# siyi-wind/MDViT

Hardware: AMD Instinct MI355X
Metric: 512x512 images/sec MDViT train step (fwd+bwd, two-sweep, AdamW) (higher is better)
Workload: dtype bf16x3 (fp32 storage; GEMM operands split hi+lo bf16, fp32 accumulate); 1 GPU; MDViT Sup+MLPFM train step, 4 domain(s) x bs=4 per GPU, 512x512, drop_rate=0.1 drop_path=0.1, bf16x3 GEMMs, data-parallel x1

## Files before the change

### include/mdvit_hip.h

```cpp
#ifndef MDVIT_HIP_H
#define MDVIT_HIP_H

#include <stddef.h>
#include <stdint.h>

#ifdef __cplusplus
extern "C" {
#endif

#define MDVIT_ABI_VERSION 1

enum {
    MDVIT_OK = 0,
    MDVIT_E_SHAPE = 1,
    MDVIT_E_DTYPE = 2,
    MDVIT_E_ALIGN = 3,
    MDVIT_E_WORKSPACE = 4,
    MDVIT_E_HIP = 5
};

enum { MDVIT_EPI_NONE = 0, MDVIT_EPI_GELU_DUAL = 1, MDVIT_EPI_DGELU = 2 };
enum { MDVIT_ACT_NONE = 0, MDVIT_ACT_HSWISH = 1, MDVIT_ACT_RELU = 2 };

const char* mdvit_last_error(void);
// ... 159 lines not shown
    int32_t ln_accumulate;
    float* e_out;
} MdvitBlockGrads;
typedef struct MdvitBlockStreams {
    void* main; void* side;
    void** events; int32_t n_events; int32_t* next_event;
} MdvitBlockStreams;
size_t mdvit_block_save_bytes(const MdvitBlockDesc* d);
size_t mdvit_block_fwd_ws_bytes(const MdvitBlockDesc* d);
int mdvit_block_fwd(const MdvitBlockDesc* d, const float* x, float* y, void* save, size_t save_bytes, void* ws, size_t ws_bytes, void* stream);
size_t mdvit_block_bwd_ws_bytes(const MdvitBlockDesc* d, const MdvitBlockGrads* g, int32_t with_side_stream, size_t* side_bytes);
int mdvit_block_bwd(const MdvitBlockDesc* d, const MdvitBlockGrads* g, const MdvitBlockStreams* st, const float* x, const void* save, size_t save_bytes,
                    const float* dy, float* dx , void* ws, size_t ws_bytes, void* ws_side, size_t ws_side_bytes);

int mdvit_rowdot_fwd(const float* x, int64_t ldx, const float* w, const float* b, float* y,
                     int32_t M, int32_t K, int32_t accumulate, void* stream);
int mdvit_rowdot_bwd(const float* x, int64_t ldx, const float* w, const float* dy, float* dx, int64_t lddx,
                     float* dw, float* db, void* ws , size_t ws_bytes, int32_t M, int32_t K, void* stream);

int mdvit_colsum_f32(const float* A, int64_t lda, float* out, float* masked, void* ws , size_t ws_bytes, int32_t M, int32_t N,
                     float drop_p, uint32_t key0, uint32_t key1, const float* rowscale, int32_t rows_per_scale,
                     int32_t accumulate, const uint32_t* drop_seed, void* stream);

int mdvit_layernorm_fwd(const float* x, const float* gamma, const float* beta, float* y, float* mean, float* rstd,
                        int32_t M, int32_t C, int32_t groups, float eps, void* stream);
int mdvit_layernorm_bwd(const float* dy, const float* x, const float* gamma, const float* mean, const float* rstd,
                        const float* add, float* dx, float* dgamma, float* dbeta, void* ws , size_t ws_bytes,
                        int32_t M, int32_t C, int32_t groups, void* stream);
int mdvit_layernorm_bwd_masked(const float* dy, const float* x, const float* gamma, const float* mean, const float* rstd, const float* add, float* dx,
                               float* dx_masked, float* dgamma, float* dbeta, void* ws, size_t ws_bytes, int32_t M, int32_t C, int32_t groups,
                               float drop_p, uint32_t key0, uint32_t key1, const float* rowscale, int32_t rows_per_scale, const uint32_t* seed, void* stream);

int mdvit_dwconv3x3_fwd(const float* x, const float* w, const float* bias, float* y,
                        int32_t B, int32_t Hi, int32_t Wi, int32_t C, int32_t stride, int32_t add_input, void* stream);
int mdvit_dwconv3x3_bwd(const float* dy, const float* x, const float* w, float* dx, float* dw, float* dbias,
                        void* ws , size_t ws_bytes,
                        int32_t B, int32_t Hi, int32_t Wi, int32_t C, int32_t stride, int32_t add_input,
                        int32_t accumulate , void* stream);
int mdvit_gconv2_3x3_fwd(const float* skip, const float* up, const float* w, float* y,
                         int32_t B, int32_t H, int32_t W, int32_t C, void* stream);
int mdvit_gconv2_3x3_bwd(const float* dy, const float* skip, const float* up, const float* w,
                         float* dskip, float* dup, float* dw, void* ws , size_t ws_bytes,
                         int32_t B, int32_t H, int32_t W, int32_t C, int32_t accumulate , void* stream);
int mdvit_im2col3x3(const float* x, float* col, int32_t B, int32_t Hi, int32_t Wi, int32_t Cin, int32_t stride, int32_t dilation, void* stream);
int mdvit_col2im3x3(const float* dcol, float* dx, int32_t B, int32_t Hi, int32_t Wi, int32_t Cin, int32_t stride, int32_t dilation, void* stream);
int mdvit_dropout_f32(const float* x, float* y, int64_t n, float p, uint32_t key0, uint32_t key1, const uint32_t* drop_seed, void* stream);
int mdvit_stemconv_fwd(const float* img, const float* w, float* y, int32_t B, int32_t H, int32_t W, int32_t Cin, int32_t Cout, void* stream);
int mdvit_stemconv_wgrad(const float* img, const float* dy, float* dw, void* ws , size_t ws_bytes,
                         int32_t B, int32_t H, int32_t W, int32_t Cin, int32_t Cout, int32_t accumulate , void* stream);

size_t mdvit_bn_ws_bytes(int32_t M, int32_t C, int32_t groups);
int mdvit_bn_stats(const float* y, void* ws, size_t ws_bytes, float* mean, float* rstd, float* running_mean, float* running_var,
                   int64_t* num_batches_tracked, int32_t M, int32_t C, int32_t groups, int32_t per_group_affine, float eps,
                   float momentum, void* stream);
int mdvit_bn_eval_prep(const float* running_mean, const float* running_var, float* mean, float* rstd, int32_t C, float eps, void* stream);
int mdvit_bn_apply(const float* y, const float* mean, const float* rstd, const float* gamma, const float* beta, float* z,
                   int32_t M, int32_t C, int32_t groups, int32_t per_group_affine, int32_t act, float drop2d_p, uint32_t key0,
                   uint32_t key1, const uint32_t* drop_seed, int32_t rows_per_sample, void* stream);
int mdvit_bn_bwd(const float* dz, const float* y, const float* mean, const float* rstd, const float* gamma, const float* beta,
                 float* dy, float* dgamma, float* dbeta, void* ws, size_t ws_bytes, int32_t M, int32_t C, int32_t groups,
                 int32_t per_group_affine, int32_t act, int32_t training, float drop2d_p, uint32_t key0, uint32_t key1, const uint32_t* drop_seed, int32_t rows_per_sample,
                 void* stream);

size_t mdvit_bn_rowdot_ws_bytes(int32_t M, int32_t C);
int mdvit_bn_rowdot_fwd(const float* y, const float* mean, const float* rstd, const float* gamma, const float* beta, const float* w, const float* b ,
                        float* low, int32_t M, int32_t C, int32_t act, float drop2d_p, uint32_t key0, uint32_t key1, const uint32_t* drop_seed,
                        int32_t rows_per_sample, void* stream);
int mdvit_bn_rowdot_bwd(const float* g, const float* y, const float* mean, const float* rstd, const float* gamma, const float* beta, const float* w,
                        float* dy, float* dgamma, float* dbeta, float* dw, float* db , void* ws, size_t ws_bytes, int32_t M, int32_t C, int32_t act,
                        int32_t training, float drop2d_p, uint32_t key0, uint32_t key1, const uint32_t* drop_seed, int32_t rows_per_sample, void* stream);

int mdvit_upsample_fwd(const float* x, const float* base , float* y,
                       int32_t B, int32_t Hi, int32_t Wi, int32_t Ho, int32_t Wo, int32_t C, void* stream);
size_t mdvit_upsample_bwd_ws_bytes(int32_t B, int32_t Hi, int32_t Wi, int32_t Ho, int32_t Wo, int32_t C);
int mdvit_upsample_bwd(const float* dy, float* dx, void* ws, size_t ws_bytes, int32_t B, int32_t Hi, int32_t Wi, int32_t Ho, int32_t Wo,
                       int32_t C, void* stream);

int mdvit_upsample_multi_fwd(const float* const* xs, const int32_t* Hi, const int32_t* Wi, int32_t n, const float* base, float* y, int32_t B, int32_t Ho,
                             int32_t Wo, int32_t C, void* stream);
size_t mdvit_upsample_multi_bwd_ws_bytes(const int32_t* Wi, int32_t n, int32_t B, int32_t Ho, int32_t C);
int mdvit_upsample_multi_bwd(const float* dy, float* const* dxs, const int32_t* Hi, const int32_t* Wi, int32_t n, void* ws, size_t ws_bytes, int32_t B,
                             int32_t Ho, int32_t Wo, int32_t C, void* stream);

int mdvit_da_fwd(const float* label, const float* W1, const float* b1, const float* W2, const float* b2, float* a,
                 int32_t B, int32_t D, int32_t hid, int32_t C, int32_t heads, void* stream);
#define MDVIT_DA_MANY_MAX 32
typedef struct MdvitDaMany {
    int32_t n;
    int32_t hid[MDVIT_DA_MANY_MAX], C[MDVIT_DA_MANY_MAX], heads[MDVIT_DA_MANY_MAX];
    const float* W1[MDVIT_DA_MANY_MAX]; const float* b1[MDVIT_DA_MANY_MAX]; const float* W2[MDVIT_DA_MANY_MAX]; const float* b2[MDVIT_DA_MANY_MAX];
    float* a[MDVIT_DA_MANY_MAX];
} MdvitDaMany;
int mdvit_da_fwd_many(const MdvitDaMany* m, const float* label, int32_t B, int32_t D, void* stream);
typedef struct MdvitDaManyGrads {
    const float* e[MDVIT_DA_MANY_MAX];
    float* dW1[MDVIT_DA_MANY_MAX]; float* db1[MDVIT_DA_MANY_MAX]; float* dW2[MDVIT_DA_MANY_MAX]; float* db2[MDVIT_DA_MANY_MAX];
} MdvitDaManyGrads;
size_t mdvit_da_many_ws_bytes(const MdvitDaMany* m, int32_t B);
int mdvit_da_bwd_many(const MdvitDaMany* m, const MdvitDaManyGrads* g, const float* label, float scale, void* ws, size_t ws_bytes, int32_t B, int32_t D, void* stream);
size_t mdvit_da_ws_bytes(int32_t B, int32_t hid, int32_t C);
int mdvit_da_bwd(const float* label, const float* W1, const float* b1, const float* W2, const float* b2, const float* a,
                 const float* e, float scale, float* dW1, float* db1, float* dW2, float* db2, void* ws, size_t ws_bytes,
                 int32_t B, int32_t D, int32_t hid, int32_t C, int32_t heads, void* stream);

size_t mdvit_factoratt_ws_bytes(int32_t B, int32_t N, int32_t C, int32_t heads);
int mdvit_factoratt_fwd(const float* qkv, const float* w3, const float* b3, const float* w5, const float* b5,
                        const float* w7, const float* b7, const float* a, float* out, float* U, float* kmax, float* ksum, float* Mmat,
                        void* ws, size_t ws_bytes, int32_t B, int32_t H, int32_t W, int32_t C, int32_t heads,
                        int32_t s3, int32_t s5, int32_t s7, void* stream);
int mdvit_factoratt_bwd(const float* dout, const float* qkv, const float* out, const float* U,
                        const float* w3, const float* b3, const float* w5, const float* b5, const float* w7, const float* b7,
                        const float* a, const float* kmax, const float* ksum, const float* Mmat,
                        float* dqkv, float* e, float* dw3, float* db3, float* dw5, float* db5, float* dw7, float* db7,
                        void* ws, size_t ws_bytes, int32_t B, int32_t H, int32_t W, int32_t C, int32_t heads,
                        int32_t s3, int32_t s5, int32_t s7, void* stream);
int mdvit_factoratt_wgrad(const float* qkv, void* ws, size_t ws_bytes, float* dw3, float* db3, float* dw5, float* db5,
                          float* dw7, float* db7, int32_t B, int32_t H, int32_t W, int32_t C, int32_t heads,
                          int32_t s3, int32_t s5, int32_t s7, int32_t accumulate, void* stream);

int mdvit_seg_losses_fwd(const float* out, const float* aux, const float* label, double* sums, float* losses, int64_t n, void* stream);
int mdvit_seg_losses_sums(const float* out, const float* aux, const float* label, double* sums, int64_t n, void* stream);
int mdvit_seg_losses_final(const double* sums, float* losses, int64_t n_total, int32_t has_aux, void* stream);
int mdvit_seg_losses_bwd(const float* out, const float* aux, const float* label, const double* sums, const float* g,
                         float* dout, float* daux, int64_t n, float dice_gain, void* stream);
int mdvit_seg_losses_bwd3(const float* out, const float* aux, const float* label, const double* sums, const float* g0, const float* g1, const float* g2,
                          float* dout, float* daux, int64_t n, float dice_gain, void* stream);
int mdvit_seg_losses_groups_sums(const float* out, const float* aux, const float* label, double* sums, int64_t n, int32_t G, void* stream);
int mdvit_seg_losses_groups_final(const double* sums, float* losses, float* per_group, int64_t n_total, int32_t has_aux, int32_t G, void* stream);
int mdvit_seg_losses_groups_bwd(const float* out, const float* aux, const float* label, const double* sums, const float* g0, const float* g1, const float* g2,
                                float* dout, float* daux, int64_t n, int32_t G, float dice_gain, void* stream);

int mdvit_seg_metrics(const float* out, const float* aux, const float* label, uint64_t* counts, float* metrics, int64_t n, void* stream);
int mdvit_image_normalize_u8(const uint8_t* img_nhwc, float* out_nchw, int32_t B, int32_t H, int32_t W, void* stream);
int mdvit_augment_normalize_u8(const uint8_t* img_nhwc, const uint8_t* mask, const float* params, const uint32_t* keys, float* out_nchw, float* label,
                               int32_t B, int32_t H, int32_t W, void* stream);
int mdvit_augment_probe_taps(float xs, float ys, int32_t H, int32_t W, int32_t* idx5, float* w4);

int mdvit_adamw_step(const void* table_dev, int32_t n_tensors, int32_t blocks_per_tensor, const float* lr_dev, float* step_dev,
                     float beta1, float beta2, float eps, float weight_decay, int32_t zero_grad, void* stream);

int mdvit_imgconv_fwd(const float* img, const float* w, float* y, int32_t B, int32_t H, int32_t W, int32_t in_chans, int32_t Cout, int32_t ksize, void* stream);
int mdvit_imgconv_wgrad(const float* img, const float* dy, float* dw, void* ws, size_t ws_bytes, int32_t B, int32_t H, int32_t W, int32_t in_chans,
                        int32_t Cout, int32_t ksize, int32_t accumulate, void* stream);
int mdvit_imgconv_im2col(const float* img, float* col, int32_t B, int32_t H, int32_t W, int32_t in_chans, int32_t ksize, int32_t ldc, void* stream);
int mdvit_maxpool3x3s2_fwd(const float* x, float* y, void* idx, int32_t B, int32_t H, int32_t W, int32_t C, void* stream);
int mdvit_maxpool3x3s2_bwd(const float* dy, const void* idx, float* dx, int32_t B, int32_t H, int32_t W, int32_t C, void* stream);
int mdvit_resize_ac_fwd(const float* x, float* y, int32_t B, int32_t Hi, int32_t Wi, int32_t Ho, int32_t Wo, int32_t C, void* stream);
int mdvit_resize_ac_bwd(const float* dy, float* dx, int32_t B, int32_t Hi, int32_t Wi, int32_t Ho, int32_t Wo, int32_t C, void* stream);
int mdvit_ew(const float* a, const float* b, float* y, int64_t n, int32_t mode, void* stream);
int mdvit_add3(const float* a, const float* b, const float* c, float* y, int64_t n, void* stream);
int mdvit_add_parts(const float* a, const float* b, const void* const* parts, int32_t G, int64_t part_elems, float* y, void* stream);
int mdvit_add_bcast(const float* x, const float* pe, float* y, int32_t B, int64_t R, void* stream);
int mdvit_sum_batch(const float* g, float* out, int32_t B, int64_t R, void* stream);
int mdvit_gate_fwd(const float* x, const float* s, float* y, int32_t B, int64_t P, int32_t C, int32_t mode, void* stream);
size_t mdvit_gate_bwd_ws_bytes(int32_t B, int64_t P, int32_t C, int32_t mode);
int mdvit_gate_bwd(const float* g, const float* x, const float* s, float* dx, float* ds, void* ws, size_t ws_bytes, int32_t B, int64_t P, int32_t C, int32_t mode,
                   void* stream);
int mdvit_chanpool_fwd(const float* x, float* y, int32_t* idx, int64_t M, int32_t C, void* stream);
int mdvit_chanpool_bwd(const float* dy, const int32_t* idx, float* dx, int64_t M, int32_t C, void* stream);
int mdvit_conv7x7_2to1_fwd(const float* x, const float* w, float* y, int32_t B, int32_t H, int32_t W, void* stream);
int mdvit_conv7x7_2to1_bwd(const float* dy, const float* x, const float* w, float* dx , float* dw , int32_t B, int32_t H,
                           int32_t W, void* stream);
int mdvit_bn1_fwd(const float* x, const float* gamma, const float* beta, float* running_mean, float* running_var, void* num_batches_tracked, float* y,
                  float* stat, int64_t M, int32_t groups, int32_t training, float eps, float momentum, void* stream);
int mdvit_bn1_bwd(const float* g, const float* x, const float* gamma, const float* stat, float* dx, float* dgamma_dbeta, int64_t M, int32_t groups, int32_t training,
                  void* stream);
// ... 32 lines not shown
```

### mdvit_amd/_lib.py

```python
from __future__ import annotations

import ctypes as C
import os
import re
from typing import List

_HERE = os.path.dirname(os.path.abspath(__file__))
LIB_PATH = os.environ.get("MDVIT_HIP_LIB") or os.path.join(_HERE, "lib", "libmdvit_hip.so")
HEADER_PATH = os.path.join(_HERE, "..", "include", "mdvit_hip.h")

EPI_NONE, EPI_GELU_DUAL, EPI_DGELU = 0, 1, 2
ACT_NONE, ACT_HSWISH, ACT_RELU = 0, 1, 2

f32p = C.c_void_p
vp = C.c_void_p
i32 = C.c_int32
i64 = C.c_int64
u32 = C.c_uint32
f32 = C.c_float


class GemmDesc(C.Structure):
    _fields_ = [
        ("A", vp), ("B", vp), ("C", vp), ("C2", vp),
# ... 113 lines not shown
    "mdvit_linear_rc": [vp, i64, vp, i64, vp, vp, i64, i32, i32, i32, f32, u32, u32, vp, i32, vp, i64, vp, vp],
    "mdvit_linear_rc_ln": [vp, vp, vp, i32, f32, vp, vp, vp, vp, i64, vp, vp, i64, i32, i32, i32, vp],
    "mdvit_mlp_rc_fwd_ln": [vp, vp, vp, i32, f32, vp, vp, vp, vp, vp, vp, vp, vp, i32, vp, vp, i32, i32, i32, f32, u32, u32, u32, u32, vp, vp],
    "mdvit_mlp_rc16_fwd": [vp, vp, vp, vp, vp, vp, vp, i32, vp, vp, i32, i32, i32, f32, u32, u32, u32, u32, vp, vp],
    "mdvit_mlp_rc_dgrad": [vp, vp, vp, vp, vp, vp, vp, i32, i32, i32, f32, u32, u32, vp, vp],
    "mdvit_mlp_rc16_dgrad": [vp, vp, vp, vp, vp, vp, vp, vp, i32, i32, i32, f32, u32, u32, vp, vp],
    "mdvit_mlp_rc_fwd_ln_hbf16": [vp, vp, vp, i32, f32, vp, vp, vp, vp, vp, vp, vp, vp, i32, vp, vp, i32, i32, i32, f32, u32, u32, u32, u32, vp, vp],
    "mdvit_mlp_rc16_fwd_hbf16": [vp, vp, vp, vp, vp, vp, vp, i32, vp, vp, i32, i32, i32, f32, u32, u32, u32, u32, vp, vp],
    "mdvit_mlp_rc16_dgrad_hbf16": [vp, vp, vp, vp, vp, vp, vp, vp, i32, i32, i32, f32, u32, u32, vp, vp],
    "mdvit_mlp_rc_wgrad": [vp, vp, vp, vp, vp, vp, vp, vp, vp, C.c_size_t, i32, i32, i32, f32, u32, u32, vp, i32, vp],
    "mdvit_mlp_rc_bwd": [vp, vp, vp, vp, vp, vp, vp, vp, vp, vp, vp, C.c_size_t, i32, i32, i32, f32, u32, u32, vp, i32, vp],
    "mdvit_imgconv_fwd": [vp, vp, vp, i32, i32, i32, i32, i32, i32, vp],
    "mdvit_imgconv_wgrad": [vp, vp, vp, vp, C.c_size_t, i32, i32, i32, i32, i32, i32, i32, vp],
    "mdvit_maxpool3x3s2_fwd": [vp, vp, vp, i32, i32, i32, i32, vp],
    "mdvit_maxpool3x3s2_bwd": [vp, vp, vp, i32, i32, i32, i32, vp],
    "mdvit_resize_ac_fwd": [vp, vp, i32, i32, i32, i32, i32, i32, vp],
    "mdvit_resize_ac_bwd": [vp, vp, i32, i32, i32, i32, i32, i32, vp],
    "mdvit_ew": [vp, vp, vp, i64, i32, vp],
    "mdvit_add3": [vp, vp, vp, vp, i64, vp],
    "mdvit_add_parts": [vp, vp, C.POINTER(vp), i32, i64, vp, vp],
    "mdvit_add_bcast": [vp, vp, vp, i32, i64, vp],
    "mdvit_sum_batch": [vp, vp, i32, i64, vp],
    "mdvit_gate_fwd": [vp, vp, vp, i32, i64, i32, i32, vp],
    "mdvit_gate_bwd": [vp, vp, vp, vp, vp, vp, C.c_size_t, i32, i64, i32, i32, vp],
    "mdvit_imgconv_im2col": [vp, vp, i32, i32, i32, i32, i32, i32, vp],
    "mdvit_chanpool_fwd": [vp, vp, vp, i64, i32, vp],
    "mdvit_chanpool_bwd": [vp, vp, vp, i64, i32, vp],
    "mdvit_conv7x7_2to1_fwd": [vp, vp, vp, i32, i32, i32, vp],
    "mdvit_conv7x7_2to1_bwd": [vp, vp, vp, vp, vp, i32, i32, i32, vp],
    "mdvit_bn1_fwd": [vp, vp, vp, vp, vp, vp, vp, vp, i64, i32, i32, f32, f32, vp],
    "mdvit_bn1_bwd": [vp, vp, vp, vp, vp, vp, i64, i32, i32, vp],
    "mdvit_subsample2": [vp, vp, i32, i32, i32, i32, i32, vp],
    "mdvit_patchify": [vp, vp, i32, i32, i32, i32, i32, vp],
    "mdvit_dropout2d": [vp, vp, i32, i64, i32, f32, u32, u32, vp, vp],
    "mdvit_sdpa_fwd": [vp, vp, vp, vp, i32, i32, i32, i32, vp],
    "mdvit_sdpa_bwd": [vp, vp, vp, vp, vp, vp, vp, vp, i32, i32, i32, i32, vp],
    "mdvit_sdpa_mfma_fwd": [vp, vp, vp, vp, i32, i32, i32, i32, vp],
    "mdvit_sdpa_mfma_bwd": [vp, vp, vp, vp, vp, vp, vp, vp, i32, i32, i32, i32, vp],
    "mdvit_structure_weight": [vp, vp, vp, i32, i32, i32, vp],
    "mdvit_structure_loss_fwd": [vp, vp, vp, vp, vp, i32, i64, vp],
    "mdvit_structure_loss_bwd": [vp, vp, vp, vp, vp, vp, i32, i64, vp],
    "mdvit_split_planes": [vp, i64, vp, i64, i64, i64, i32, i32, vp],
    "mdvit_split_planes_many": [vp, i32, i32, i32, vp],
    "mdvit_split_planes_t": [vp, i64, vp, i64, i64, i32, i32, i32, i32, vp],
    "mdvit_event_create": [C.POINTER(vp)],
    "mdvit_event_destroy": [vp],
    "mdvit_event_elapsed_ms": [vp, vp, C.POINTER(f32)],
    "mdvit_timing_arm": [vp, vp],
    "mdvit_gemm_f32": [C.POINTER(GemmDesc), vp],
    "mdvit_gemm_plan": [C.POINTER(GemmDesc), C.POINTER(i32), C.POINTER(i32), C.POINTER(i32)],
    "mdvit_gemm_force_plan": [i32, i32],
    "mdvit_conv_weight_relayout": [vp, vp, i32, i32, i32, vp],
    "mdvit_conv_weight_relayout_many": [vp, i32, i32, vp],
    "mdvit_gemm_kernel_name": [vp, C.c_char_p, i32],
    "mdvit_gemm_tn_config": [i32, i32, i32],
    "mdvit_gemm_tn_grid_order": [i32],
    "mdvit_transpose_f32": [vp, i64, vp, i32, i32, vp],
    "mdvit_mlp_bwd_dgrad_f32": [vp, vp, vp, vp, vp, vp, vp, vp, i32, i32, i32, f32, u32, u32, vp, vp],
    "mdvit_mlp_fwd_f32": [vp, vp, vp, vp, vp, vp, vp, i32, vp, vp, i32, i32, i32, f32, u32, u32, u32, u32, vp, vp],
    "mdvit_transpose_many": [vp, i32, i32, vp],
    "mdvit_rowdot_fwd": [vp, i64, vp, vp, vp, i32, i32, i32, vp],
    "mdvit_rowdot_bwd": [vp, i64, vp, vp, vp, i64, vp, vp, vp, C.c_size_t, i32, i32, vp],
    "mdvit_colsum_f32": [vp, i64, vp, vp, vp, C.c_size_t, i32, i32, f32, u32, u32, vp, i32, i32, vp, vp],
    "mdvit_layernorm_fwd": [vp, vp, vp, vp, vp, vp, i32, i32, i32, f32, vp],
    "mdvit_layernorm_bwd": [vp, vp, vp, vp, vp, vp, vp, vp, vp, vp, C.c_size_t, i32, i32, i32, vp],
    "mdvit_layernorm_bwd_masked": [vp, vp, vp, vp, vp, vp, vp, vp, vp, vp, vp, C.c_size_t, i32, i32, i32, f32, u32, u32, vp, i32, vp, vp],
    "mdvit_dwconv3x3_fwd": [vp, vp, vp, vp, i32, i32, i32, i32, i32, i32, vp],
    "mdvit_dwconv3x3_bwd": [vp, vp, vp, vp, vp, vp, vp, C.c_size_t, i32, i32, i32, i32, i32, i32, i32, vp],
    "mdvit_gconv2_3x3_fwd": [vp, vp, vp, vp, i32, i32, i32, i32, vp],
    "mdvit_gconv2_3x3_bwd": [vp, vp, vp, vp, vp, vp, vp, vp, C.c_size_t, i32, i32, i32, i32, i32, vp],
    "mdvit_im2col3x3": [vp, vp, i32, i32, i32, i32, i32, i32, vp],
    "mdvit_col2im3x3": [vp, vp, i32, i32, i32, i32, i32, i32, vp],
    "mdvit_dropout_f32": [vp, vp, i64, f32, u32, u32, vp, vp],
    "mdvit_stemconv_fwd": [vp, vp, vp, i32, i32, i32, i32, i32, vp],
    "mdvit_stemconv_wgrad": [vp, vp, vp, vp, C.c_size_t, i32, i32, i32, i32, i32, i32, vp],
    "mdvit_bn_rowdot_fwd": [vp, vp, vp, vp, vp, vp, vp, vp, i32, i32, i32, f32, u32, u32, vp, i32, vp],
    "mdvit_bn_rowdot_bwd": [vp, vp, vp, vp, vp, vp, vp, vp, vp, vp, vp, vp, vp, C.c_size_t, i32, i32, i32, i32, f32, u32, u32, vp, i32, vp],
    "mdvit_bn_stats": [vp, vp, C.c_size_t, vp, vp, vp, vp, vp, i32, i32, i32, i32, f32, f32, vp],
    "mdvit_bn_eval_prep": [vp, vp, vp, vp, i32, f32, vp],
    "mdvit_bn_apply": [vp, vp, vp, vp, vp, vp, i32, i32, i32, i32, i32, f32, u32, u32, vp, i32, vp],
    "mdvit_bn_bwd": [vp, vp, vp, vp, vp, vp, vp, vp, vp, vp, C.c_size_t, i32, i32, i32, i32, i32, i32, f32, u32, u32, vp, i32, vp],
    "mdvit_upsample_multi_fwd": [vp, vp, vp, i32, vp, vp, i32, i32, i32, i32, vp],
    "mdvit_upsample_multi_bwd": [vp, vp, vp, vp, i32, vp, C.c_size_t, i32, i32, i32, i32, vp],
    "mdvit_upsample_fwd": [vp, vp, vp, i32, i32, i32, i32, i32, i32, vp],
    "mdvit_upsample_bwd": [vp, vp, vp, C.c_size_t, i32, i32, i32, i32, i32, i32, vp],
    "mdvit_da_fwd": [vp, vp, vp, vp, vp, vp, i32, i32, i32, i32, i32, vp],
    "mdvit_da_bwd": [vp] * 7 + [f32] + [vp] * 4 + [vp, C.c_size_t] + [i32] * 5 + [vp],
    "mdvit_factoratt_fwd": [vp] * 13 + [vp, C.c_size_t] + [i32] * 8 + [vp],
    "mdvit_factoratt_wgrad": [vp, vp, C.c_size_t] + [vp] * 6 + [i32] * 9 + [vp],
    "mdvit_factoratt_bwd": [vp] * 22 + [vp, C.c_size_t] + [i32] * 8 + [vp],
    "mdvit_seg_losses_fwd": [vp, vp, vp, vp, vp, i64, vp],
    "mdvit_adamw_step": [vp, i32, i32, vp, vp, f32, f32, f32, f32, i32, vp],
    "mdvit_seg_metrics": [vp, vp, vp, vp, vp, i64, vp],
    "mdvit_image_normalize_u8": [vp, vp, i32, i32, i32, vp],
    "mdvit_augment_normalize_u8": [vp, vp, vp, vp, vp, vp, i32, i32, i32, vp],
    "mdvit_augment_probe_taps": [f32, f32, i32, i32, C.POINTER(i32), C.POINTER(f32)],
    "mdvit_seg_losses_sums": [vp, vp, vp, vp, i64, vp],
    "mdvit_seg_losses_final": [vp, vp, i64, i32, vp],
    "mdvit_seg_losses_bwd": [vp, vp, vp, vp, vp, vp, vp, i64, f32, vp],
    "mdvit_seg_losses_bwd3": [vp, vp, vp, vp, vp, vp, vp, vp, vp, i64, f32, vp],
    "mdvit_seg_losses_groups_sums": [vp, vp, vp, vp, i64, i32, vp],
    "mdvit_seg_losses_groups_final": [vp, vp, vp, i64, i32, i32, vp],
    "mdvit_seg_losses_groups_bwd": [vp, vp, vp, vp, vp, vp, vp, vp, vp, i64, i32, f32, vp],
    "mdvit_se_adapter_fwd": [C.POINTER(SeAdapterDesc), vp, vp, vp, vp, C.c_size_t, vp],
    "mdvit_se_adapter_bwd": [C.POINTER(SeAdapterDesc)] + [vp] * 10 + [vp, C.c_size_t, vp],
}

_lib = None


class MdvitHipError(RuntimeError):
    pass


def declared_symbols() -> List[str]:
    with open(HEADER_PATH) as f:
        text = f.read()
    text = re.sub(r"/\*.*?\*/", "", text, flags=re.S)
    return sorted(set(re.findall(r"\b(mdvit_[a-z0-9_]+)\s*\(", text)))


_on_load = []


def on_load(fn):
    if _lib is not None:
        fn(_lib)
    else:
        _on_load.append(fn)


def load():
    global _lib
    if _lib is not None:
        return _lib
    if not os.path.exists(LIB_PATH):
        raise MdvitHipError(
            f"{LIB_PATH} is missing: build it with `python -m mdvit_amd.build` (hipcc, gfx950). "
            "mdvit_amd has no CPU or PyTorch fallback.")
    lib = C.CDLL(LIB_PATH)
    try:
        _attach_prototypes(lib)
    except AttributeError as e:
        raise MdvitHipError(f"{LIB_PATH} is stale ({e}): rebuild it with `python -m mdvit_amd.build`.") from None
    _lib = lib
    while _on_load:
        _on_load.pop(0)(lib)
    return lib


def _attach_prototypes(lib):
    lib.mdvit_last_error.restype = C.c_char_p
    lib.mdvit_last_error.argtypes = []
    lib.mdvit_version.restype = C.c_int
    lib.mdvit_version.argtypes = []
    lib.mdvit_factoratt_ws_bytes.restype = C.c_size_t
    lib.mdvit_factoratt_ws_bytes.argtypes = [i32, i32, i32, i32]
    lib.mdvit_gemm_ws_bytes.restype = C.c_size_t
    lib.mdvit_gemm_ws_bytes.argtypes = [C.POINTER(GemmDesc)]
    lib.mdvit_gate_bwd_ws_bytes.restype = C.c_size_t
    lib.mdvit_gate_bwd_ws_bytes.argtypes = [i32, i64, i32, i32]
    lib.mdvit_gemm_planes_ws_bytes.restype = C.c_size_t
    lib.mdvit_gemm_planes_ws_bytes.argtypes = [C.POINTER(PlaneGemmDesc)]
    lib.mdvit_bn_rowdot_ws_bytes.restype = C.c_size_t
    lib.mdvit_bn_rowdot_ws_bytes.argtypes = [i32, i32]
    lib.mdvit_bn_ws_bytes.restype = C.c_size_t
    lib.mdvit_bn_ws_bytes.argtypes = [i32, i32, i32]
    lib.mdvit_upsample_multi_bwd_ws_bytes.restype = C.c_size_t
    lib.mdvit_upsample_multi_bwd_ws_bytes.argtypes = [vp, i32, i32, i32, i32]
    lib.mdvit_upsample_bwd_ws_bytes.restype = C.c_size_t
    lib.mdvit_upsample_bwd_ws_bytes.argtypes = [i32] * 6
    lib.mdvit_partials_ws_bytes.restype = C.c_size_t
    lib.mdvit_partials_ws_bytes.argtypes = [i32]
    lib.mdvit_mlp_rc_wgrad_ws_bytes.restype = C.c_size_t
    lib.mdvit_mlp_rc_wgrad_ws_bytes.argtypes = [i32, i32, i32]
    lib.mdvit_block_save_bytes.restype = C.c_size_t
    lib.mdvit_block_save_bytes.argtypes = [C.POINTER(BlockDesc)]
    lib.mdvit_block_fwd_ws_bytes.restype = C.c_size_t
    lib.mdvit_block_fwd_ws_bytes.argtypes = [C.POINTER(BlockDesc)]
    lib.mdvit_block_bwd_ws_bytes.restype = C.c_size_t
    lib.mdvit_block_bwd_ws_bytes.argtypes = [C.POINTER(BlockDesc), C.POINTER(BlockGrads), i32, C.POINTER(C.c_size_t)]
    lib.mdvit_da_ws_bytes.restype = C.c_size_t
    lib.mdvit_da_ws_bytes.argtypes = [i32, i32, i32]
    lib.mdvit_da_many_ws_bytes.restype = C.c_size_t
    lib.mdvit_da_many_ws_bytes.argtypes = [C.POINTER(DaMany), i32]
    lib.mdvit_se_adapter_save_bytes.restype = C.c_size_t
    lib.mdvit_se_adapter_save_bytes.argtypes = [C.POINTER(SeAdapterDesc)]
    lib.mdvit_se_adapter_ws_bytes.restype = C.c_size_t
    lib.mdvit_se_adapter_ws_bytes.argtypes = [C.POINTER(SeAdapterDesc)]
    for name, sig in _SIGS.items():
        try:
            fn = getattr(lib, name)
        except AttributeError:
            raise MdvitHipError(f"{LIB_PATH} is stale: it does not export `{name}` (built from an earlier tree). "
                                "Rebuild it with `python -m mdvit_amd.build`.") from None
        fn.restype = C.c_int
        fn.argtypes = sig


def check(code: int, what: str):
    if code != 0:
        msg = load().mdvit_last_error().decode(errors="replace")
        raise MdvitHipError(f"{what} failed (code {code}): {msg}")


def call(name: str, *args):
    lib = load()
    check(getattr(lib, name)(*args), name)
```

### mdvit_amd/build.py

```python
from __future__ import annotations

import concurrent.futures as cf
import hashlib
import os
import subprocess
import sys

HERE = os.path.dirname(os.path.abspath(__file__))
CSRC = os.path.join(HERE, "csrc")
OBJ = os.path.join(HERE, "build")
LIB_DIR = os.path.join(HERE, "lib")
LIB = os.path.join(LIB_DIR, "libmdvit_hip.so")
SOURCES = ["abi.hip", "gemm.hip", "gemm_tn.hip", "gemm_bp.hip", "gemm_ph.hip", "gemm_pm.hip", "mlp.hip", "mlp_rc.hip", "block.hip", "norm.hip", "conv.hip", "attn.hip", "loss.hip", "optim.hip", "transfuse.hip", "sdpa.hip", "se_adapter.hip", "augment.hip"]
FLAGS = ["--offload-arch=gfx950", "-O3", "-std=c++17", "-fPIC", "-Wno-unused-result"]
EXTRA_FLAGS = {"mlp_rc.hip": ["-fno-slp-vectorize"], "gemm.hip": ["-fno-slp-vectorize"], "gemm_tn.hip": ["-fno-slp-vectorize"], "gemm_bp.hip": ["-fno-slp-vectorize"], "gemm_ph.hip": ["-fno-slp-vectorize"], "gemm_pm.hip": ["-fno-slp-vectorize"]}


def _hipcc() -> str:
    for c in (os.environ.get("HIPCC"), "/opt/rocm/bin/hipcc", "hipcc"):
        if c and (os.path.isabs(c) and os.path.exists(c) or not os.path.isabs(c)):
            return c
    raise RuntimeError("hipcc not found")


def _digest(paths) -> str:
    h = hashlib.sha256()
    for p in paths:
        with open(p, "rb") as f:
            h.update(f.read())
    h.update(" ".join(FLAGS).encode())
    return h.hexdigest()


def _compile(src: str) -> str:
    obj = os.path.join(OBJ, os.path.splitext(src)[0] + ".o")
    stamp = obj + ".sha"
    deps = [os.path.join(CSRC, src), os.path.join(CSRC, "common.h"), os.path.join(CSRC, "conv_tile.h"), os.path.join(CSRC, "gemm_body.inc"), os.path.join(CSRC, "gemm_bp.h"), os.path.join(CSRC, "augment_taps.h"),
            os.path.join(HERE, "..", "include", "mdvit_hip.h")]
    extra = EXTRA_FLAGS.get(src, [])
    dig = _digest(deps) + " ".join(extra)
    if os.path.exists(obj) and os.path.exists(stamp) and open(stamp).read() == dig:
        return obj
    cmd = [_hipcc(), *FLAGS, *extra, "-c", os.path.join(CSRC, src), "-o", obj]
    r = subprocess.run(cmd, capture_output=True, text=True)
    if r.returncode != 0:
        raise RuntimeError(f"hipcc failed on {src}:\n{r.stderr}")
    with open(stamp, "w") as f:
        f.write(dig)
    return obj


def build(verbose: bool = True) -> str:
    os.makedirs(OBJ, exist_ok=True)
    os.makedirs(LIB_DIR, exist_ok=True)
    with cf.ThreadPoolExecutor(max_workers=min(6, os.cpu_count() or 2)) as ex:
        objs = list(ex.map(_compile, SOURCES))
    newest = max(os.path.getmtime(o) for o in objs)
    if not os.path.exists(LIB) or os.path.getmtime(LIB) < newest:
        cmd = [_hipcc(), "--offload-arch=gfx950", "-shared", "-fPIC", *objs, "-o", LIB]
        r = subprocess.run(cmd, capture_output=True, text=True)
        if r.returncode != 0:
            raise RuntimeError(f"link failed:\n{r.stderr}")
    if verbose:
        print(f"built {LIB} ({os.path.getsize(LIB) / 1e6:.1f} MB)")
    return LIB


if __name__ == "__main__":
    build()
    sys.exit(0)
```

### mdvit_amd/csrc/conv.hip

```cpp
#include "common.h"
#include "conv_tile.h"

namespace {

__device__ __forceinline__ float4 f4_fma(float4 a, float4 w, float4 acc) {
    acc.x = fmaf(a.x, w.x, acc.x); acc.y = fmaf(a.y, w.y, acc.y); acc.z = fmaf(a.z, w.z, acc.z); acc.w = fmaf(a.w, w.w, acc.w);
    return acc;
}
__device__ __forceinline__ float4 f4_add(float4 a, float4 b) { return make_float4(a.x + b.x, a.y + b.y, a.z + b.z, a.w + b.w); }

__global__ __launch_bounds__(256) void dwconv3x3_fwd_kernel(const float* __restrict__ x, const float* __restrict__ w,
                                                            const float* __restrict__ bias, float* __restrict__ y,
                                                            int B, int Hi, int Wi, int C, int stride, int add_input) {
    extern __shared__ float s_w[];
    for (int i = threadIdx.x; i < 9 * C; i += blockDim.x) { const int c = i / 9, t = i % 9; s_w[t * C + c] = w[i]; }
    __syncthreads();
    const int Ho = (Hi - 1) / stride + 1, Wo = (Wi - 1) / stride + 1, QC = C >> 2;
    const long total = (long)B * Ho * Wo * QC;
    for (long e = (long)blockIdx.x * blockDim.x + threadIdx.x; e < total; e += (long)gridDim.x * blockDim.x) {
        const int c = (int)(e % QC) * 4;
        long tkn = e / QC;
        const int wo = (int)(tkn % Wo); tkn /= Wo;
        const int ho = (int)(tkn % Ho);
        const int b = (int)(tkn / Ho);
        float4 acc = bias ? *reinterpret_cast<const float4*>(bias + c) : make_float4(0.f, 0.f, 0.f, 0.f);
#pragma unroll
        for (int kh = 0; kh < 3; ++kh) {
            const int hi = ho * stride + kh - 1, hc = min(max(hi, 0), Hi - 1);
#pragma unroll
            for (int kw = 0; kw < 3; ++kw) {
                const int wi = wo * stride + kw - 1, wc = min(max(wi, 0), Wi - 1);
                const float m = (hi == hc && wi == wc) ? 1.f : 0.f;
                const float4 xv = *reinterpret_cast<const float4*>(x + (((long)b * Hi + hc) * Wi + wc) * C + c);
                const float4 wv = *reinterpret_cast<const float4*>(&s_w[(kh * 3 + kw) * C + c]);
                acc = f4_fma(xv, make_float4(wv.x * m, wv.y * m, wv.z * m, wv.w * m), acc);
            }
        }
        if (add_input) acc = f4_add(acc, *reinterpret_cast<const float4*>(x + (((long)b * Hi + ho) * Wi + wo) * C + c));
        *reinterpret_cast<float4*>(y + (((long)b * Ho + ho) * Wo + wo) * C + c) = acc;
    }
}

__global__ __launch_bounds__(256) void dwconv3x3_dgrad_kernel(const float* __restrict__ dy, const float* __restrict__ w,
                                                              float* __restrict__ dx, int B, int Hi, int Wi, int C, int stride, int add_input) {
    extern __shared__ float s_w[];
    for (int i = threadIdx.x; i < 9 * C; i += blockDim.x) { const int c = i / 9, t = i % 9; s_w[t * C + c] = w[i]; }
    __syncthreads();
    const int Ho = (Hi - 1) / stride + 1, Wo = (Wi - 1) / stride + 1, QC = C >> 2;
    const long total = (long)B * Hi * Wi * QC;
    for (long e = (long)blockIdx.x * blockDim.x + threadIdx.x; e < total; e += (long)gridDim.x * blockDim.x) {
        const int c = (int)(e % QC) * 4;
        long tkn = e / QC;
        const int wi = (int)(tkn % Wi); tkn /= Wi;
        const int hi = (int)(tkn % Hi);
        const int b = (int)(tkn / Hi);
        float4 acc = make_float4(0.f, 0.f, 0.f, 0.f);
#pragma unroll
        for (int kh = 0; kh < 3; ++kh) {
            const int hn = hi - kh + 1;
            if (hn < 0 || (hn % stride) != 0) continue;
            const int ho = hn / stride;
            if (ho >= Ho) continue;
#pragma unroll
            for (int kw = 0; kw < 3; ++kw) {
                const int wn = wi - kw + 1;
                if (wn < 0 || (wn % stride) != 0) continue;
                const int wo = wn / stride;
                if (wo >= Wo) continue;
                const float4 g = *reinterpret_cast<const float4*>(dy + (((long)b * Ho + ho) * Wo + wo) * C + c);
                const float4 wv = *reinterpret_cast<const float4*>(&s_w[(kh * 3 + kw) * C + c]);
                acc = f4_fma(g, wv, acc);
            }
        }
        if (add_input) acc = f4_add(acc, *reinterpret_cast<const float4*>(dy + (((long)b * Hi + hi) * Wi + wi) * C + c));
        *reinterpret_cast<float4*>(dx + (((long)b * Hi + hi) * Wi + wi) * C + c) = acc;
    }
}

__global__ __launch_bounds__(256) void dwconv3x3_wgrad_kernel(const float* __restrict__ dy, const float* __restrict__ x,
                                                              float* __restrict__ part,
                                                              int B, int Hi, int Wi, int C, int stride, int tokens_per_block) {
    extern __shared__ float s_acc[];
    for (int i = threadIdx.x; i < C * 10; i += blockDim.x) s_acc[i] = 0.f;
    __syncthreads();
// ... 334 lines not shown
    for (int co = threadIdx.x % nco; co < Cout; co += nco) {
        float acc[KK];
#pragma unroll
        for (int k = 0; k < KK; ++k) acc[k] = 0.f;
        if (pl < npl) {
            for (long px = p_beg + pl; px < p_end; px += npl) {
                long r = px;
                const int wo = (int)(r % Wo); r /= Wo;
                const int ho = (int)(r % Ho);
                const int b = (int)(r / Ho);
                const float g = dy[px * Cout + co];
#pragma unroll
                for (int ci = 0; ci < CIN; ++ci)
#pragma unroll
                    for (int kh = 0; kh < 3; ++kh) {
                        const int hi = 2 * ho + kh - 1;
#pragma unroll
                        for (int kw = 0; kw < 3; ++kw) {
                            const int wi = 2 * wo + kw - 1;
                            const bool ok = hi >= 0 && hi < H && wi >= 0 && wi < W;
                            const float xv = ok ? img[(((long)b * CIN + ci) * H + hi) * W + wi] : 0.f;
                            acc[ci * 9 + kh * 3 + kw] = fmaf(g, xv, acc[ci * 9 + kh * 3 + kw]);
                        }
                    }
            }
        }
#pragma unroll
        for (int k = 0; k < KK; ++k) atomicAdd(&s_acc[co * KK + k], acc[k]);
    }
    __syncthreads();
    for (int i = threadIdx.x; i < Cout * KK; i += blockDim.x) part[(long)blockIdx.x * Cout * KK + i] = s_acc[i];
}

template <int CIN>
__global__ __launch_bounds__(256) void stemconv_wgrad_mfma_kernel(const float* __restrict__ img, const float* __restrict__ dy,
                                                                  float* __restrict__ part, int B, int H, int W, int Cout, int pix_per_block) {
    typedef float f32x16 __attribute__((ext_vector_type(16)));
    constexpr int KK = CIN * 9;
    static_assert(KK <= 32, "one 32-wide tap block");
    __shared__ float s_acc[4][32 * 33];
    const int Ho = (H - 1) / 2 + 1, Wo = (W - 1) / 2 + 1;
    const long npix = (long)B * Ho * Wo;
    const long p_beg = (long)blockIdx.x * pix_per_block, p_end = min(npix, p_beg + pix_per_block);
    const int lane = threadIdx.x & 63, wave = threadIdx.x >> 6, l31 = lane & 31, lhi = lane >> 5;
    const int tap = min(l31, KK - 1), ci = tap / 9, kh = (tap % 9) / 3, kw = tap % 3;
    const bool tap_ok = l31 < KK;
    constexpr int UN = 8;
    for (int cb = 0; cb < Cout; cb += 32) {
        f32x16 acc;
#pragma unroll
        for (int r = 0; r < 16; ++r) acc[r] = 0.f;
        for (long p0 = p_beg + wave * 2 * UN; p0 < p_end; p0 += 4 * 2 * UN) {
            float a[UN], x[UN];
            const long p0s = ((long)__builtin_amdgcn_readfirstlane((int)(p0 >> 32)) << 32) | (unsigned)__builtin_amdgcn_readfirstlane((int)p0);
            const int wo0 = (int)(p0s % Wo), ho0 = (int)((p0s / Wo) % Ho), b0 = (int)(p0s / Wo / Ho);
#pragma unroll
            for (int u = 0; u < UN; ++u) {
                const long px = p0 + 2 * u + lhi;
                const bool pok = px < p_end;
                const long pc = pok ? px : p_end - 1;
                int wo = wo0 + 2 * u + lhi - (int)(px - pc), ho = ho0, b = b0;
                while (wo >= Wo) { wo -= Wo; ++ho; }
                while (ho >= Ho) { ho -= Ho; ++b; }
                const int hi = 2 * ho + kh - 1, wi = 2 * wo + kw - 1;
                const bool ok = pok && tap_ok && hi >= 0 && hi < H && wi >= 0 && wi < W;
                const float g = dy[pc * Cout + cb + l31];
                const float v = img[(((long)b * CIN + ci) * H + min(max(hi, 0), H - 1)) * W + min(max(wi, 0), W - 1)];
                a[u] = pok ? g : 0.f;
                x[u] = ok ? v : 0.f;
            }
#pragma unroll
            for (int u = 0; u < UN; ++u) acc = __builtin_amdgcn_mfma_f32_32x32x2f32(a[u], x[u], acc, 0, 0, 0);
        }
        __syncthreads();
#pragma unroll
        for (int r = 0; r < 16; ++r) s_acc[wave][((r & 3) + 8 * (r >> 2) + 4 * lhi) * 33 + l31] = acc[r];
        __syncthreads();
        for (int i = threadIdx.x; i < 32 * KK; i += 256) {
            const int co = i / KK, k = i % KK;
            const float t = ((s_acc[0][co * 33 + k] + s_acc[1][co * 33 + k]) + s_acc[2][co * 33 + k]) + s_acc[3][co * 33 + k];
            part[(long)blockIdx.x * Cout * KK + (cb + co) * KK + k] = t;
        }
    }
}

__device__ __forceinline__ void bilin_src(int o, int in_size, float scale, int& i0, int& i1, float& l1) {
    float src = scale * ((float)o + 0.5f) - 0.5f;
    if (src < 0.f) src = 0.f;
    i0 = (int)src;
    if (i0 > in_size - 1) i0 = in_size - 1;
    i1 = i0 + (i0 < in_size - 1 ? 1 : 0);
    l1 = src - (float)i0;
}

__global__ __launch_bounds__(256) void upsample_fwd_kernel(const float* __restrict__ x, const float* base_, float* y,
                                                           int B, int Hi, int Wi, int Ho, int Wo, int C) {
    const float sh = (float)Hi / (float)Ho, sw = (float)Wi / (float)Wo;
    const bool vec = (C & 3) == 0;
    const int QC = vec ? C >> 2 : C;
    const long total = (long)B * Ho * Wo * QC;
    for (long e = (long)mdvit_xcd_logical_block() * blockDim.x + threadIdx.x; e < total; e += (long)gridDim.x * blockDim.x) {
        const int q = (int)(e % QC);
        long r = e / QC;
        const int wo = (int)(r % Wo); r /= Wo;
        const int ho = (int)(r % Ho);
        const int b = (int)(r / Ho);
        int h0, h1, w0, w1; float lh, lw;
        bilin_src(ho, Hi, sh, h0, h1, lh);
        bilin_src(wo, Wi, sw, w0, w1, lw);
        const float c00 = (1.f - lh) * (1.f - lw), c01 = (1.f - lh) * lw, c10 = lh * (1.f - lw), c11 = lh * lw;
        const long base = (long)b * Hi * Wi;
        if (vec) {
            const int c = q * 4;
            const float4 v00 = *reinterpret_cast<const float4*>(x + (base + (long)h0 * Wi + w0) * C + c);
            const float4 v01 = *reinterpret_cast<const float4*>(x + (base + (long)h0 * Wi + w1) * C + c);
            const float4 v10 = *reinterpret_cast<const float4*>(x + (base + (long)h1 * Wi + w0) * C + c);
            const float4 v11 = *reinterpret_cast<const float4*>(x + (base + (long)h1 * Wi + w1) * C + c);
            float4 o;
            o.x = c00 * v00.x + c01 * v01.x + c10 * v10.x + c11 * v11.x;
            o.y = c00 * v00.y + c01 * v01.y + c10 * v10.y + c11 * v11.y;
            o.z = c00 * v00.z + c01 * v01.z + c10 * v10.z + c11 * v11.z;
            o.w = c00 * v00.w + c01 * v01.w + c10 * v10.w + c11 * v11.w;
            const long oi = (((long)b * Ho + ho) * Wo + wo) * C + c;
            if (base_) o = f4_add(o, *reinterpret_cast<const float4*>(base_ + oi));
            *reinterpret_cast<float4*>(y + oi) = o;
        } else {
            const float v = c00 * x[(base + (long)h0 * Wi + w0) * C + q] + c01 * x[(base + (long)h0 * Wi + w1) * C + q] +
                            c10 * x[(base + (long)h1 * Wi + w0) * C + q] + c11 * x[(base + (long)h1 * Wi + w1) * C + q];
            const long oi = (((long)b * Ho + ho) * Wo + wo) * C + q;
            y[oi] = base_ ? base_[oi] + v : v;
        }
    }
}

__device__ __forceinline__ void out_range(int i, int in_size, int out_size, int& lo, int& hi) {
    if (out_size % in_size == 0 && ((out_size / in_size) & 1) == 0) {
        const int s = out_size / in_size;
        lo = s * i - s / 2; hi = s * i + 3 * s / 2;
        if (lo < 0) lo = 0;
        if (hi > out_size) hi = out_size;
        return;
    }
    const float inv = (float)out_size / (float)in_size;
    lo = (int)floorf(((float)i - 1.0f) * inv) - 1;
    hi = (int)ceilf(((float)i + 2.0f) * inv) + 1;
    if (lo < 0) lo = 0;
    if (hi > out_size) hi = out_size;
}

template <bool ALONG_W>
__global__ __launch_bounds__(256) void upsample_bwd_pass_kernel(const float* __restrict__ src, float* __restrict__ dst,
                                                                long outer, int n_in, int n_out, long inner_q, int vec) {
    const float sc = (float)n_in / (float)n_out;
    const long total = outer * n_in * inner_q;
    for (long e = (long)blockIdx.x * blockDim.x + threadIdx.x; e < total; e += (long)gridDim.x * blockDim.x) {
        const long q = e % inner_q;
        long r = e / inner_q;
        const int i = (int)(r % n_in);
        const long o = r / n_in;
        int lo, hi;
        out_range(i, n_in, n_out, lo, hi);
        float4 acc = make_float4(0.f, 0.f, 0.f, 0.f);
        const long inner = vec ? inner_q * 4 : inner_q;
        const float* base = src + o * n_out * inner + (vec ? q * 4 : q);
#pragma unroll 4
        for (int t = lo; t < hi; ++t) {
            int i0, i1; float l;
            bilin_src(t, n_in, sc, i0, i1, l);
            const float wgt = (i0 == i ? 1.f - l : 0.f) + (i1 == i ? l : 0.f);
            if (vec) {
                const float4 g = *reinterpret_cast<const float4*>(base + (long)t * inner);
                acc.x = fmaf(wgt, g.x, acc.x); acc.y = fmaf(wgt, g.y, acc.y); acc.z = fmaf(wgt, g.z, acc.z); acc.w = fmaf(wgt, g.w, acc.w);
            } else {
                acc.x = fmaf(wgt, base[(long)t * inner], acc.x);
            }
        }
        float* d = dst + (o * n_in + i) * inner + (vec ? q * 4 : q);
        if (vec) *reinterpret_cast<float4*>(d) = acc;
        else *d = acc.x;
    }
}

struct UpMulti {
    const float* x[3]; float* d[3];
    int Hi[3], Wi[3];
    int n;
};

__global__ __launch_bounds__(256) void upsample_multi_fwd_kernel(UpMulti p, const float* base_, float* __restrict__ y, int B, int Ho, int Wo, int C) {
    const int QC = C >> 2;
    const int row_items = Wo * QC;
    const int cpr = (row_items + 1023) >> 10;
    const long nunits = (long)B * Ho * cpr;
    for (long u = mdvit_xcd_logical_block(); u < nunits; u += gridDim.x) {
        const long row = u / cpr;
        const int k = (int)(u - row * cpr);
        const int ho = (int)(row % Ho), b = (int)(row / Ho);
        int h0[3], h1[3]; float lh[3];
#pragma unroll
        for (int i = 0; i < 3; ++i) {
            h0[i] = h1[i] = 0; lh[i] = 0.f;
            if (i < p.n) bilin_src(ho, p.Hi[i], (float)p.Hi[i] / (float)Ho, h0[i], h1[i], lh[i]);
        }
#pragma unroll
        for (int it = 0; it < 4; ++it) {
            const int e = (k << 10) + it * 256 + (int)threadIdx.x;
            if (e >= row_items) break;
            const int wo = e / QC, c = (e - wo * QC) * 4;
            const long oi = ((row * Wo) + wo) * C + c;
            float4 o = base_ ? *reinterpret_cast<const float4*>(base_ + oi) : make_float4(0.f, 0.f, 0.f, 0.f);
#pragma unroll
            for (int i = 0; i < 3; ++i) {
                if (i >= p.n) break;
                const int Hi = p.Hi[i], Wi = p.Wi[i];
                int w0, w1; float lw;
                bilin_src(wo, Wi, (float)Wi / (float)Wo, w0, w1, lw);
                const float c00 = (1.f - lh[i]) * (1.f - lw), c01 = (1.f - lh[i]) * lw, c10 = lh[i] * (1.f - lw), c11 = lh[i] * lw;
                const float* x = p.x[i] + (long)b * Hi * Wi * C + c;
                const float4 v00 = *reinterpret_cast<const float4*>(x + ((long)h0[i] * Wi + w0) * C), v01 = *reinterpret_cast<const float4*>(x + ((long)h0[i] * Wi + w1) * C);
                const float4 v10 = *reinterpret_cast<const float4*>(x + ((long)h1[i] * Wi + w0) * C), v11 = *reinterpret_cast<const float4*>(x + ((long)h1[i] * Wi + w1) * C);
                float4 uu;
                uu.x = c00 * v00.x + c01 * v01.x + c10 * v10.x + c11 * v11.x;
                uu.y = c00 * v00.y + c01 * v01.y + c10 * v10.y + c11 * v11.y;
                uu.z = c00 * v00.z + c01 * v01.z + c10 * v10.z + c11 * v11.z;
                uu.w = c00 * v00.w + c01 * v01.w + c10 * v10.w + c11 * v11.w;
                o = (i == 0 && !base_) ? uu : f4_add(uu, o);
            }
            *reinterpret_cast<float4*>(y + oi) = o;
        }
    }
}

constexpr int UT_H = 8, UT_W = 16, UT_C = 128, UT_POOL = 96;
__global__ __launch_bounds__(256) void upsample_multi_tile_kernel(UpMulti p, const float* __restrict__ base_, float* __restrict__ y, int Ho, int Wo, int C) {
    __shared__ __attribute__((aligned(16))) float s_src[UT_POOL * UT_C];
    const int tiles_w = Wo / UT_W;
    const int ty = blockIdx.x / tiles_w, tx = blockIdx.x - ty * tiles_w;
    const int ho0 = ty * UT_H, wo0 = tx * UT_W, c0 = blockIdx.y * UT_C, b = blockIdx.z;
    int r0[3], q0[3], pw[3], off[3];
    {
        int used = 0;
#pragma unroll
        for (int i = 0; i < 3; ++i) {
            r0[i] = q0[i] = pw[i] = off[i] = 0;
            if (i >= p.n) continue;
            const int Hi = p.Hi[i], Wi = p.Wi[i];
            int a0, a1, b0, b1; float l;
            bilin_src(ho0, Hi, (float)Hi / (float)Ho, a0, b0, l);
            bilin_src(ho0 + UT_H - 1, Hi, (float)Hi / (float)Ho, a1, b1, l);
            const int ph = b1 - a0 + 1;
            r0[i] = a0;
            bilin_src(wo0, Wi, (float)Wi / (float)Wo, a0, b0, l);
            bilin_src(wo0 + UT_W - 1, Wi, (float)Wi / (float)Wo, a1, b1, l);
            pw[i] = b1 - a0 + 1;
            q0[i] = a0;
            off[i] = used * UT_C;
            const float* x = p.x[i] + (long)b * Hi * Wi * C + c0;
            const int items = ph * pw[i] * (UT_C / 4);
            for (int e = threadIdx.x; e < items; e += 256) {
                const int cq = e & (UT_C / 4 - 1), px = e >> 5, pr = px / pw[i], pc = px - pr * pw[i];
                *reinterpret_cast<float4*>(s_src + off[i] + px * UT_C + 4 * cq) =
                    *reinterpret_cast<const float4*>(x + ((long)(r0[i] + pr) * Wi + (q0[i] + pc)) * C + 4 * cq);
            }
            used += ph * pw[i];
        }
    }
    __syncthreads();
    const int cq = threadIdx.x & 31, colh = threadIdx.x >> 5;
#pragma unroll 2
    for (int it = 0; it < UT_H * 2; ++it) {
        const int ho = ho0 + (it >> 1), wo = wo0 + (it & 1) * 8 + colh;
        const long oi = ((((long)b * Ho + ho) * Wo) + wo) * C + c0 + 4 * cq;
        float4 o = base_ ? *reinterpret_cast<const float4*>(base_ + oi) : make_float4(0.f, 0.f, 0.f, 0.f);
#pragma unroll
        for (int i = 0; i < 3; ++i) {
            if (i >= p.n) break;
            const int Hi = p.Hi[i], Wi = p.Wi[i];
            int h0, h1, w0, w1; float lh, lw;
            bilin_src(ho, Hi, (float)Hi / (float)Ho, h0, h1, lh);
            bilin_src(wo, Wi, (float)Wi / (float)Wo, w0, w1, lw);
            const float c00 = (1.f - lh) * (1.f - lw), c01 = (1.f - lh) * lw, c10 = lh * (1.f - lw), c11 = lh * lw;
            const float* sp = s_src + off[i] + 4 * cq;
            const float4 v00 = *reinterpret_cast<const float4*>(sp + ((h0 - r0[i]) * pw[i] + (w0 - q0[i])) * UT_C), v01 = *reinterpret_cast<const float4*>(sp + ((h0 - r0[i]) * pw[i] + (w1 - q0[i])) * UT_C);
            const float4 v10 = *reinterpret_cast<const float4*>(sp + ((h1 - r0[i]) * pw[i] + (w0 - q0[i])) * UT_C), v11 = *reinterpret_cast<const float4*>(sp + ((h1 - r0[i]) * pw[i] + (w1 - q0[i])) * UT_C);
            float4 uu;
            uu.x = c00 * v00.x + c01 * v01.x + c10 * v10.x + c11 * v11.x;
            uu.y = c00 * v00.y + c01 * v01.y + c10 * v10.y + c11 * v11.y;
            uu.z = c00 * v00.z + c01 * v01.z + c10 * v10.z + c11 * v11.z;
            uu.w = c00 * v00.w + c01 * v01.w + c10 * v10.w + c11 * v11.w;
            o = (i == 0 && !base_) ? uu : f4_add(uu, o);
        }
        *reinterpret_cast<float4*>(y + oi) = o;
    }
}

__global__ __launch_bounds__(256) void upsample_multi_bwd_w_kernel(UpMulti p, const float* __restrict__ dy, long outer, int Wo, int C, int bpr) {
    const int QC = C >> 2;
    const int Wsum = p.Wi[0] + (p.n > 1 ? p.Wi[1] : 0) + (p.n > 2 ? p.Wi[2] : 0);
    const int nwg = (int)gridDim.x, qx = nwg >> 3, rx = nwg & 7, xcd = blockIdx.x & 7, ix = blockIdx.x >> 3;
    const int lb = (xcd < rx ? xcd * (qx + 1) : rx * (qx + 1) + (xcd - rx) * qx) + ix;
    const long o = lb / bpr;
    {
        const long e = (long)(lb % bpr) * blockDim.x + threadIdx.x;
        if (e >= (long)Wsum * QC) return;
        const int c = (int)(e % QC) * 4;
        int j = (int)(e / QC);
        int src = 0;
        if (j >= p.Wi[0]) { j -= p.Wi[0]; src = 1; if (j >= p.Wi[1]) { j -= p.Wi[1]; src = 2; } }
        const int Wi = p.Wi[src];
        const float sc = (float)Wi / (float)Wo;
        int lo, hi;
        out_range(j, Wi, Wo, lo, hi);
        float4 acc = make_float4(0.f, 0.f, 0.f, 0.f);
        const float* base = dy + o * Wo * C + c;
#pragma unroll 4
        for (int t = lo; t < hi; ++t) {
            int i0, i1; float l;
            bilin_src(t, Wi, sc, i0, i1, l);
            const float wgt = (i0 == j ? 1.f - l : 0.f) + (i1 == j ? l : 0.f);
            const float4 g = *reinterpret_cast<const float4*>(base + (long)t * C);
            acc.x = fmaf(wgt, g.x, acc.x); acc.y = fmaf(wgt, g.y, acc.y); acc.z = fmaf(wgt, g.z, acc.z); acc.w = fmaf(wgt, g.w, acc.w);
        }
        float* dsts[3] = {p.d[0], p.d[1], p.d[2]};
        *reinterpret_cast<float4*>(dsts[src] + (o * Wi + j) * C + c) = acc;
    }
}

__global__ __launch_bounds__(256) void upsample_multi_bwd_w_lds_kernel(UpMulti p, const float* __restrict__ dy, int Wo, int C) {
    extern __shared__ __attribute__((aligned(16))) float s_row[];
    const long o = blockIdx.x;
    const int c0 = blockIdx.y * 32;
    const float* src = dy + o * Wo * C + c0;
    for (int e = threadIdx.x; e < Wo * 8; e += 256) {
        const int t = e >> 3, q = e & 7;
        *reinterpret_cast<float4*>(s_row + t * 32 + 4 * q) = *reinterpret_cast<const float4*>(src + (long)t * C + 4 * q);
    }
    __syncthreads();
    const int Wsum = p.Wi[0] + (p.n > 1 ? p.Wi[1] : 0) + (p.n > 2 ? p.Wi[2] : 0);
    float* dsts[3] = {p.d[0], p.d[1], p.d[2]};
    for (int e = threadIdx.x; e < Wsum * 8; e += 256) {
        const int q = e & 7;
        int j = e >> 3, sidx = 0;
        if (j >= p.Wi[0]) { j -= p.Wi[0]; sidx = 1; if (j >= p.Wi[1]) { j -= p.Wi[1]; sidx = 2; } }
        const int Wi = p.Wi[sidx];
        const float sc = (float)Wi / (float)Wo;
        int lo, hi;
        out_range(j, Wi, Wo, lo, hi);
        float4 acc = make_float4(0.f, 0.f, 0.f, 0.f);
#pragma unroll 4
        for (int t = lo; t < hi; ++t) {
            int i0, i1; float l;
            bilin_src(t, Wi, sc, i0, i1, l);
            const float wgt = (i0 == j ? 1.f - l : 0.f) + (i1 == j ? l : 0.f);
            const float4 g = *reinterpret_cast<const float4*>(s_row + t * 32 + 4 * q);
            acc.x = fmaf(wgt, g.x, acc.x); acc.y = fmaf(wgt, g.y, acc.y); acc.z = fmaf(wgt, g.z, acc.z); acc.w = fmaf(wgt, g.w, acc.w);
        }
        *reinterpret_cast<float4*>(dsts[sidx] + (o * Wi + j) * C + c0 + 4 * q) = acc;
    }
}

__global__ __launch_bounds__(256) void dropout_kernel(const float* __restrict__ x, float* __restrict__ y, long n4, uint32_t k0, uint32_t k1,
                                                      const uint32_t* __restrict__ seed, uint32_t thresh, float inv_keep) {
    const uint32_t k0e = k0 ^ (seed ? seed[0] : 0u), k1e = k1 + (seed ? seed[1] : 0u);
    for (long i = (long)blockIdx.x * blockDim.x + threadIdx.x; i < n4; i += (long)gridDim.x * blockDim.x) {
        const float4 v = *reinterpret_cast<const float4*>(x + 4 * i);
        const float4 d = mdvit_drop_scale4(k0e, k1e, (uint32_t)(4 * i), thresh, inv_keep);
        *reinterpret_cast<float4*>(y + 4 * i) = make_float4(v.x * d.x, v.y * d.y, v.z * d.z, v.w * d.w);
    }
}

inline int ew_grid(long total) { return (int)min((total + 255) / 256, 16384L); }

}

extern "C" int mdvit_dwconv3x3_fwd(const float* x, const float* w, const float* bias, float* y, int32_t B, int32_t Hi, int32_t Wi,
                                   int32_t C, int32_t stride, int32_t add_input, void* stream) {
    MDVIT_CHECK_ARG(B > 0 && Hi > 0 && Wi > 0 && C > 0 && C % 4 == 0 && C <= 4096, MDVIT_E_SHAPE, "dwconv3x3_fwd: bad shape B=%d H=%d W=%d C=%d", B, Hi, Wi, C);
    MDVIT_CHECK_ARG(stride == 1 || stride == 2, MDVIT_E_SHAPE, "dwconv3x3_fwd: stride must be 1 or 2");
    MDVIT_CHECK_ARG(!(add_input && stride != 1), MDVIT_E_SHAPE, "dwconv3x3_fwd: add_input needs stride 1");
    const int Ho = (Hi - 1) / stride + 1, Wo = (Wi - 1) / stride + 1;
    if (stride == 1) {
        launch_conv_tile<3, false>(x, (long)C, 0, w, bias, y, (long)C, 0, CtGeom{B, Hi, Wi}, C, (hipStream_t)stream, add_input);
        MDVIT_LAUNCH_CHECK();
        return MDVIT_OK;
    }
    const long total = (long)B * Ho * Wo * C / 4;
    hipLaunchKernelGGL(dwconv3x3_fwd_kernel, dim3(ew_grid(total)), dim3(256), sizeof(float) * 9 * C, (hipStream_t)stream,
                       x, w, bias, y, B, Hi, Wi, C, stride, add_input);
    MDVIT_LAUNCH_CHECK();
    return MDVIT_OK;
}

extern "C" int mdvit_dwconv3x3_bwd(const float* dy, const float* x, const float* w, float* dx, float* dw, float* dbias, void* ws, size_t ws_bytes,
                                   int32_t B, int32_t Hi, int32_t Wi, int32_t C, int32_t stride, int32_t add_input, int32_t accumulate,
                                   void* stream) {
    hipStream_t s = (hipStream_t)stream;
    MDVIT_CHECK_ARG(B > 0 && Hi > 0 && Wi > 0 && C > 0 && C % 4 == 0 && C <= 1024, MDVIT_E_SHAPE, "dwconv3x3_bwd: bad shape B=%d H=%d W=%d C=%d", B, Hi, Wi, C);
    MDVIT_CHECK_ARG(stride == 1 || stride == 2, MDVIT_E_SHAPE, "dwconv3x3_bwd: stride must be 1 or 2");
    const int Ho = (Hi - 1) / stride + 1, Wo = (Wi - 1) / stride + 1;
    if (stride == 1) {
        const CtGeom cg{B, Hi, Wi};
        if (dx) launch_conv_tile<3, true>(dy, (long)C, 0, w, nullptr, dx, (long)C, 0, cg, C, s, add_input);
        if (dw) {
            int tpb; long nblk;
            conv_wgrad_plan(cg, C, tpb, nblk);
            MDVIT_CHECK_PARTIALS_WS(ws, ws_bytes, nblk, CT_CL * 10, "dwconv3x3_bwd");
            const int rc = launch_conv_tile_wgrad<3>(dy, (long)C, 0, x, (long)C, 0, dw, dbias, (float*)ws, cg, C, s, accumulate);
            if (rc != MDVIT_OK) return rc;
        }
        MDVIT_LAUNCH_CHECK();
        return MDVIT_OK;
    }
    if (dx) {
        const long total = (long)B * Hi * Wi * C / 4;
        hipLaunchKernelGGL(dwconv3x3_dgrad_kernel, dim3(ew_grid(total)), dim3(256), sizeof(float) * 9 * C, s, dy, w, dx, B, Hi, Wi, C, stride, add_input);
    }
    if (dw) {
        const long ntok = (long)B * Ho * Wo;
        int tpb = (int)max(64L, (ntok + 1023) / 1024);
        const int nblk = cdiv(ntok, tpb);
        MDVIT_CHECK_PARTIALS_WS(ws, ws_bytes, nblk, 10 * C, "dwconv3x3_bwd");
        hipLaunchKernelGGL(dwconv3x3_wgrad_kernel, dim3(nblk), dim3(256), sizeof(float) * 10 * C, s, dy, x, (float*)ws, B, Hi, Wi, C, stride, tpb);
        const int rc = mdvit_reduce_partials((const float*)ws, nblk, 10L * C, 9 * C, dw, C, dbias, accumulate, s);
        if (rc != MDVIT_OK) return rc;
    }
    MDVIT_LAUNCH_CHECK();
    return MDVIT_OK;
}

extern "C" int mdvit_gconv2_3x3_fwd(const float* skip, const float* up, const float* w, float* y, int32_t B, int32_t H, int32_t W, int32_t C, void* stream) {
    MDVIT_CHECK_ARG(B > 0 && H > 0 && W > 0 && C > 0 && C % 4 == 0 && C <= 2048, MDVIT_E_SHAPE, "gconv2_fwd: bad shape B=%d H=%d W=%d C=%d", B, H, W, C);
    const long total = (long)B * H * W * C / 2;
    const int tiles_w = cdiv(W, CT_TW), tiles = tiles_w * cdiv(H, CT_TH);
    if (C % 32 == 0 && aligned16(skip) && aligned16(up) && B <= 65535)
        hipLaunchKernelGGL((gconv2_tile_kernel<false>), dim3(tiles, 2 * C / CT_CL, B), dim3(256), 0, (hipStream_t)stream, skip, up, w, y, (float*)nullptr, H, W, C, tiles_w);
    else
        hipLaunchKernelGGL(gconv2_fwd_kernel, dim3(ew_grid(total)), dim3(256), sizeof(float) * 18 * C, (hipStream_t)stream, skip, up, w, y, B, H, W, C);
    MDVIT_LAUNCH_CHECK();
    return MDVIT_OK;
}

// ... 46 lines not shown
    return MDVIT_OK;
}

extern "C" int mdvit_dropout_f32(const float* x, float* y, int64_t n, float p, uint32_t key0, uint32_t key1, const uint32_t* drop_seed, void* stream) {
    MDVIT_CHECK_ARG(n > 0 && n % 4 == 0 && n < (1L << 32) && p >= 0.f && p < 1.f, MDVIT_E_SHAPE, "dropout: need 0 < n < 2^32, n %% 4 == 0, 0 <= p < 1 (n=%ld p=%g)", (long)n, p);
    MDVIT_CHECK_ARG(aligned16(x) && aligned16(y), MDVIT_E_ALIGN, "dropout: 16-byte aligned buffers");
    hipLaunchKernelGGL(dropout_kernel, dim3(ew_grid(n / 4)), dim3(256), 0, (hipStream_t)stream, x, y, (long)(n / 4), key0, key1, drop_seed,
                       mdvit_drop_thresh(p), 1.f / (1.f - p));
    MDVIT_LAUNCH_CHECK();
    return MDVIT_OK;
}

extern "C" int mdvit_stemconv_fwd(const float* img, const float* w, float* y, int32_t B, int32_t H, int32_t W, int32_t Cin, int32_t Cout, void* stream) {
    MDVIT_CHECK_ARG(Cin == 3, MDVIT_E_SHAPE, "stemconv_fwd: only in_chans == 3 is built (got %d)", Cin);
    MDVIT_CHECK_ARG(B > 0 && H > 0 && W > 0 && Cout > 0 && Cout % 4 == 0 && Cout <= 256, MDVIT_E_SHAPE, "stemconv_fwd: bad shape");
    const int Ho = (H - 1) / 2 + 1, Wo = (W - 1) / 2 + 1;
    static const bool px32 = [] { const char* e = getenv("MDVIT_STEM_FWD32"); return !(e && e[0] == '0'); }();
    if (px32 && Cout == 32)
        hipLaunchKernelGGL((stemconv_fwd32_kernel<3>), dim3((int)min(((long)B * Ho * Wo + 127) / 128, 8192L)), dim3(256), 0, (hipStream_t)stream, img, w, y, B, H, W);
    else
        hipLaunchKernelGGL((stemconv_fwd_kernel<3>), dim3(ew_grid((long)B * Ho * Wo * Cout / 4)), dim3(256), sizeof(float) * 27 * Cout, (hipStream_t)stream,
                           img, w, y, B, H, W, Cout);
    MDVIT_LAUNCH_CHECK();
    return MDVIT_OK;
}

extern "C" int mdvit_stemconv_wgrad(const float* img, const float* dy, float* dw, void* ws, size_t ws_bytes, int32_t B, int32_t H, int32_t W,
                                    int32_t Cin, int32_t Cout, int32_t accumulate, void* stream) {
    hipStream_t s = (hipStream_t)stream;
    MDVIT_CHECK_ARG(Cin == 3, MDVIT_E_SHAPE, "stemconv_wgrad: only in_chans == 3 is built (got %d)", Cin);
    MDVIT_CHECK_ARG(B > 0 && H > 0 && W > 0 && Cout > 0 && Cout <= 256, MDVIT_E_SHAPE, "stemconv_wgrad: bad shape");
    const int Ho = (H - 1) / 2 + 1, Wo = (W - 1) / 2 + 1;
    const long npix = (long)B * Ho * Wo;
    int ppb = (int)max(64L, (npix + 2047) / 2048);
    const int nblk = cdiv(npix, ppb);
    MDVIT_CHECK_PARTIALS_WS(ws, ws_bytes, nblk, 27 * Cout, "stemconv_wgrad");
    static const bool mfma = [] { const char* e = getenv("MDVIT_STEM_WGRAD_MFMA"); return !(e && e[0] == '0'); }();
    if (mfma && Cout % 32 == 0) {
        ppb = (int)max(128L, (npix + 1023) / 1024);
        const int nb2 = cdiv(npix, ppb);
        hipLaunchKernelGGL((stemconv_wgrad_mfma_kernel<3>), dim3(nb2), dim3(256), 0, s, img, dy, (float*)ws, B, H, W, Cout, ppb);
        MDVIT_LAUNCH_CHECK();
        return mdvit_reduce_partials((const float*)ws, nb2, 27L * Cout, 27 * Cout, dw, 0, nullptr, accumulate, s);
    }
    hipLaunchKernelGGL((stemconv_wgrad_kernel<3>), dim3(nblk), dim3(256), sizeof(float) * 27 * Cout, s, img, dy, (float*)ws, B, H, W, Cout, ppb);
    MDVIT_LAUNCH_CHECK();
    return mdvit_reduce_partials((const float*)ws, nblk, 27L * Cout, 27 * Cout, dw, 0, nullptr, accumulate, s);
}

extern "C" int mdvit_upsample_fwd(const float* x, const float* base, float* y, int32_t B, int32_t Hi, int32_t Wi, int32_t Ho, int32_t Wo, int32_t C, void* stream) {
    MDVIT_CHECK_ARG(B > 0 && Hi > 0 && Wi > 0 && Ho > 0 && Wo > 0 && C > 0, MDVIT_E_SHAPE, "upsample_fwd: bad shape");
    const long total = (long)B * Ho * Wo * ((C & 3) == 0 ? C / 4 : C);
    hipLaunchKernelGGL(upsample_fwd_kernel, dim3(ew_grid(total)), dim3(256), 0, (hipStream_t)stream, x, base, y, B, Hi, Wi, Ho, Wo, C);
    MDVIT_LAUNCH_CHECK();
    return MDVIT_OK;
}

extern "C" size_t mdvit_upsample_bwd_ws_bytes(int32_t B, int32_t Hi, int32_t Wi, int32_t Ho, int32_t Wo, int32_t C) {
    if (B <= 0 || Hi <= 0 || Wi <= 0 || Ho <= 0 || Wo <= 0 || C <= 0) return 0;
    return sizeof(float) * (size_t)B * Ho * Wi * C;
}

extern "C" int mdvit_upsample_bwd(const float* dy, float* dx, void* ws, size_t ws_bytes, int32_t B, int32_t Hi, int32_t Wi, int32_t Ho, int32_t Wo,
                                  int32_t C, void* stream) {
    hipStream_t s = (hipStream_t)stream;
    MDVIT_CHECK_ARG(B > 0 && Hi > 0 && Wi > 0 && Ho > 0 && Wo > 0 && C > 0, MDVIT_E_SHAPE, "upsample_bwd: bad shape");
    MDVIT_CHECK_ARG(ws != nullptr && ws_bytes >= mdvit_upsample_bwd_ws_bytes(B, Hi, Wi, Ho, Wo, C), MDVIT_E_WORKSPACE,
                    "upsample_bwd: workspace too small (mdvit_upsample_bwd_ws_bytes)");
    float* tmp = (float*)ws;
    const int vec = (C & 3) == 0 && aligned16(dy) && aligned16(dx) && aligned16(tmp);
    const long cq = vec ? C / 4 : C;
    {
        const long total = (long)B * Ho * Wi * cq;
        hipLaunchKernelGGL((upsample_bwd_pass_kernel<true>), dim3(ew_grid(total)), dim3(256), 0, s, dy, tmp, (long)B * Ho, Wi, Wo, cq, vec);
    }
    {
        const long total = (long)B * Hi * Wi * cq;
        hipLaunchKernelGGL((upsample_bwd_pass_kernel<false>), dim3(ew_grid(total)), dim3(256), 0, s, tmp, dx, (long)B, Hi, Ho, (long)Wi * cq, vec);
    }
    MDVIT_LAUNCH_CHECK();
    return MDVIT_OK;
}

extern "C" int mdvit_upsample_multi_fwd(const float* const* xs, const int32_t* Hi, const int32_t* Wi, int32_t n, const float* base, float* y, int32_t B, int32_t Ho,
                                        int32_t Wo, int32_t C, void* stream) {
    MDVIT_CHECK_ARG(n >= 1 && n <= 3 && B > 0 && Ho > 0 && Wo > 0 && C > 0 && C % 4 == 0, MDVIT_E_SHAPE, "upsample_multi_fwd: 1..3 sources, C %% 4 == 0 (n=%d C=%d)", n, C);
    UpMulti p; memset(&p, 0, sizeof(p));
    p.n = n;
    for (int i = 0; i < n; ++i) {
        MDVIT_CHECK_ARG(xs[i] && Hi[i] > 0 && Wi[i] > 0 && aligned16(xs[i]), MDVIT_E_SHAPE, "upsample_multi_fwd: bad source %d", i);
        p.x[i] = xs[i]; p.Hi[i] = Hi[i]; p.Wi[i] = Wi[i];
    }
    MDVIT_CHECK_ARG(aligned16(y) && (!base || aligned16(base)), MDVIT_E_ALIGN, "upsample_multi_fwd: y / base must be 16-byte aligned");
    {
        bool ok = Ho % UT_H == 0 && Wo % UT_W == 0 && C % UT_C == 0 && (long)(Ho / UT_H) * (Wo / UT_W) < (1L << 30) && C / UT_C < 65536 && B < 65536;
        int pool = 0;
        for (int i = 0; i < n && ok; ++i) {
            const int fh = Ho / Hi[i], fw = Wo / Wi[i];
            ok = Ho % Hi[i] == 0 && Wo % Wi[i] == 0 && fh >= 2 && fw >= 2 && fh <= 16 && fw <= 16 && (fh & (fh - 1)) == 0 && (fw & (fw - 1)) == 0;
            if (ok) pool += (UT_H / fh + 2) * (UT_W / fw + 2);
        }
        if (ok && pool <= UT_POOL) {
            hipLaunchKernelGGL(upsample_multi_tile_kernel, dim3((Ho / UT_H) * (Wo / UT_W), C / UT_C, B), dim3(256), 0, (hipStream_t)stream, p, base, y, Ho, Wo, C);
            MDVIT_LAUNCH_CHECK();
            return MDVIT_OK;
        }
    }
    MDVIT_CHECK_ARG((long)Wo * (C / 4) < (1L << 30), MDVIT_E_SHAPE, "upsample_multi_fwd: output row too long");
    const long nunits = (long)B * Ho * (((long)Wo * (C / 4) + 1023) >> 10);
    hipLaunchKernelGGL(upsample_multi_fwd_kernel, dim3((unsigned)min(nunits, 16384L)), dim3(256), 0, (hipStream_t)stream, p, base, y, B, Ho, Wo, C);
    MDVIT_LAUNCH_CHECK();
    return MDVIT_OK;
}

extern "C" size_t mdvit_upsample_multi_bwd_ws_bytes(const int32_t* Wi, int32_t n, int32_t B, int32_t Ho, int32_t C) {
    size_t t = 0;
    for (int i = 0; i < n && i < 3; ++i) t += (size_t)B * Ho * Wi[i] * C;
    return sizeof(float) * t;
}

extern "C" int mdvit_upsample_multi_bwd(const float* dy, float* const* dxs, const int32_t* Hi, const int32_t* Wi, int32_t n, void* ws, size_t ws_bytes, int32_t B,
                                        int32_t Ho, int32_t Wo, int32_t C, void* stream) {
    hipStream_t s = (hipStream_t)stream;
    MDVIT_CHECK_ARG(n >= 1 && n <= 3 && B > 0 && Ho > 0 && Wo > 0 && C > 0 && C % 4 == 0, MDVIT_E_SHAPE, "upsample_multi_bwd: 1..3 sources, C %% 4 == 0 (n=%d C=%d)", n, C);
    MDVIT_CHECK_ARG(ws && ws_bytes >= mdvit_upsample_multi_bwd_ws_bytes(Wi, n, B, Ho, C) && aligned16(ws) && aligned16(dy), MDVIT_E_WORKSPACE,
                    "upsample_multi_bwd: workspace too small (mdvit_upsample_multi_bwd_ws_bytes)");
    UpMulti p; memset(&p, 0, sizeof(p));
    p.n = n;
    float* t = (float*)ws;
    int wsum = 0;
    for (int i = 0; i < n; ++i) {
        MDVIT_CHECK_ARG(dxs[i] && Hi[i] > 0 && Wi[i] > 0 && aligned16(dxs[i]), MDVIT_E_SHAPE, "upsample_multi_bwd: bad source %d", i);
        p.Hi[i] = Hi[i]; p.Wi[i] = Wi[i]; p.d[i] = t;
        t += (size_t)B * Ho * Wi[i] * C;
        wsum += Wi[i];
    }
    const long cq = C / 4;
    const int bpr = (int)cdiv((long)wsum * cq, 256L);
    MDVIT_CHECK_ARG((long)B * Ho * bpr < (1L << 31), MDVIT_E_SHAPE, "upsample_multi_bwd: too many workgroups");
    if (C % 32 == 0 && Wo <= 384 && (long)B * Ho < (1L << 31) && C / 32 <= 65535)
        hipLaunchKernelGGL(upsample_multi_bwd_w_lds_kernel, dim3((unsigned)((long)B * Ho), C / 32), dim3(256), sizeof(float) * Wo * 32, s, p, dy, Wo, C);
    else
        hipLaunchKernelGGL(upsample_multi_bwd_w_kernel, dim3((unsigned)((long)B * Ho * bpr)), dim3(256), 0, s, p, dy, (long)B * Ho, Wo, C, bpr);
    for (int i = 0; i < n; ++i)
        hipLaunchKernelGGL((upsample_bwd_pass_kernel<false>), dim3(ew_grid((long)B * Hi[i] * Wi[i] * cq)), dim3(256), 0, s, p.d[i], dxs[i], (long)B, Hi[i], Ho,
                           (long)Wi[i] * cq, 1);
    MDVIT_LAUNCH_CHECK();
    return MDVIT_OK;
}
```

### mdvit_amd/csrc/norm.hip

```cpp
#include "common.h"

namespace {

#define LN_GROUP_FWD(C_)                                                                                   \
    { const long g_ = blockIdx.y; x += g_ * M * (C_); y += g_ * M * (C_); mean += g_ * M; rstd += g_ * M;   \
      gamma += g_ * (C_); beta += g_ * (C_); }
#define LN_GROUP_BWD(C_)                                                                                   \
    { const long g_ = blockIdx.y; dy += g_ * M * (C_); x += g_ * M * (C_); dx += g_ * M * (C_);             \
      if (add) add += g_ * M * (C_);                                                                       \
      mean += g_ * M; rstd += g_ * M; gamma += g_ * (C_); part += g_ * gridDim.x * 2 * (C_); }

template <int VPT>
__global__ __launch_bounds__(256) void ln_fwd_kernel(const float* __restrict__ x, const float* __restrict__ gamma,
                                                     const float* __restrict__ beta, float* __restrict__ y,
                                                     float* __restrict__ mean, float* __restrict__ rstd, int M, int C, float eps) {
    LN_GROUP_FWD(C);
    const int lane = threadIdx.x & 63;
    const int nw = (gridDim.x * blockDim.x) >> 6;
    for (int row = (blockIdx.x * blockDim.x + threadIdx.x) >> 6; row < M; row += nw) {
        const float* xr = x + (long)row * C;
        float v[VPT];
        float s = 0.f;
#pragma unroll
        for (int j = 0; j < VPT; ++j) {
            const int c = lane + 64 * j;
            v[j] = c < C ? xr[c] : 0.f;
            s += v[j];
        }
        const float mu = wave_sum(s) / (float)C;
        float q = 0.f;
#pragma unroll
        for (int j = 0; j < VPT; ++j) {
            const int c = lane + 64 * j;
            const float d = c < C ? v[j] - mu : 0.f;
            q += d * d;
        }
        const float rs = 1.0f / sqrtf(wave_sum(q) / (float)C + eps);
        float* yr = y + (long)row * C;
#pragma unroll
        for (int j = 0; j < VPT; ++j) {
            const int c = lane + 64 * j;
            if (c < C) yr[c] = (v[j] - mu) * rs * gamma[c] + beta[c];
        }
        if (lane == 0) { mean[row] = mu; rstd[row] = rs; }
    }
}

template <int VPT>
__global__ __launch_bounds__(256) void ln_bwd_kernel(const float* __restrict__ dy, const float* __restrict__ x,
                                                     const float* __restrict__ gamma, const float* __restrict__ mean,
                                                     const float* __restrict__ rstd, const float* __restrict__ add, float* __restrict__ dx,
                                                     float* __restrict__ part, int M, int C) {
    LN_GROUP_BWD(C);
    __shared__ float s_dg[4][64 * VPT];
    __shared__ float s_db[4][64 * VPT];
    const int lane = threadIdx.x & 63, wave = threadIdx.x >> 6;
    const int nw = (gridDim.x * blockDim.x) >> 6;
    float adg[VPT], adb[VPT], g[VPT];
#pragma unroll
    for (int j = 0; j < VPT; ++j) {
        adg[j] = 0.f; adb[j] = 0.f;
        const int c = lane + 64 * j;
        g[j] = c < C ? gamma[c] : 0.f;
    }
    for (int row = (blockIdx.x * blockDim.x + threadIdx.x) >> 6; row < M; row += nw) {
        const float mu = mean[row], rs = rstd[row];
        float xh[VPT], d[VPT];
        float c1 = 0.f, c2 = 0.f;
#pragma unroll
        for (int j = 0; j < VPT; ++j) {
            const int c = lane + 64 * j;
            const bool ok = c < C;
            const float dv = ok ? dy[(long)row * C + c] : 0.f;
            xh[j] = ok ? (x[(long)row * C + c] - mu) * rs : 0.f;
            d[j] = dv * g[j];
            c1 += d[j];
            c2 += d[j] * xh[j];
            adg[j] += dv * xh[j];
            adb[j] += dv;
        }
        c1 = wave_sum(c1) / (float)C;
        c2 = wave_sum(c2) / (float)C;
#pragma unroll
// ... 492 lines not shown
            const int c = (lane + 64 * v) * 4 + j;
            const float rs = p.rstd[c] * p.gamma[c];
            sc[v][j] = rs; sh[v][j] = p.beta[c] - p.mean[c] * rs; wv[v][j] = w[c];
        }
    const float b0 = bias ? bias[0] : 0.f;
    for (long row = ((long)blockIdx.x * blockDim.x + threadIdx.x) >> 6; row < p.M; row += nw) {
        float4 yv[VPL];
#pragma unroll
        for (int v = 0; v < VPL; ++v) yv[v] = *reinterpret_cast<const float4*>(p.a + row * p.C + (lane + 64 * v) * 4);
        float s = 0.f;
#pragma unroll
        for (int v = 0; v < VPL; ++v) {
            const float y4[4] = {yv[v].x, yv[v].y, yv[v].z, yv[v].w};
            float ds[4] = {1.f, 1.f, 1.f, 1.f};
            if (p.drop_p > 0.f) {
                const float4 d4 = mdvit_drop_scale4(k0e, k1e, (uint32_t)((row / p.rows_per_sample) * p.C + (lane + 64 * v) * 4), p.thresh, p.inv_keep);
                ds[0] = d4.x; ds[1] = d4.y; ds[2] = d4.z; ds[3] = d4.w;
            }
#pragma unroll
            for (int j = 0; j < 4; ++j) s += wv[v][j] * (act_fwd(p.act, fmaf(y4[j], sc[v][j], sh[v][j])) * ds[j]);
        }
        s = wave_sum(s);
        if (lane == 0) low[row] = s + b0;
    }
}

__global__ __launch_bounds__(256) void bn_rowdot_reduce_kernel(ChanArgs p, const float* __restrict__ g, const float* __restrict__ w, int want_w) {
    extern __shared__ float s_part[];
    const uint32_t k0e = p.k0 ^ (p.seed ? p.seed[0] : 0u), k1e = p.k1 + (p.seed ? p.seed[1] : 0u);
    const int QC = p.C >> 2;
    const long T = (long)gridDim.x * blockDim.x, t0 = (long)blockIdx.x * blockDim.x + threadIdx.x;
    const int q = (int)(t0 % QC), c = q * 4;
    const long total = (long)p.M * QC;
    float mu[4], rs[4], ga[4], be[4], wv[4];
#pragma unroll
    for (int j = 0; j < 4; ++j) { mu[j] = p.mean[c + j]; rs[j] = p.rstd[c + j]; ga[j] = p.gamma[c + j]; be[j] = p.beta[c + j]; wv[j] = w[c + j]; }
    float s1[4] = {0.f, 0.f, 0.f, 0.f}, s2[4] = {0.f, 0.f, 0.f, 0.f}, s3[4] = {0.f, 0.f, 0.f, 0.f}, s4 = 0.f;
    (void)total;
    const long rstep = T / QC;
    auto one_row = [&](long row, const float gr, const float4 yv) __attribute__((always_inline)) {
        const float y4[4] = {yv.x, yv.y, yv.z, yv.w};
        float ds[4] = {1.f, 1.f, 1.f, 1.f};
        if (p.drop_p > 0.f) {
            const float4 d4 = mdvit_drop_scale4(k0e, k1e, (uint32_t)((row / p.rows_per_sample) * p.C + c), p.thresh, p.inv_keep);
            ds[0] = d4.x; ds[1] = d4.y; ds[2] = d4.z; ds[3] = d4.w;
        }
        if (q == 0) s4 += gr;
#pragma unroll
        for (int j = 0; j < 4; ++j) {
            const float xh = (y4[j] - mu[j]) * rs[j], pre = xh * ga[j] + be[j];
            const float G = gr * wv[j] * act_grad(p.act, pre) * ds[j];
            s1[j] += G; s2[j] += G * xh;
            if (want_w) s3[j] += gr * (act_fwd(p.act, pre) * ds[j]);
        }
    };
    long r = t0 / QC;
    for (; r + 3 * rstep < p.M; r += 4 * rstep) {
        float gr[4]; float4 yv[4];
#pragma unroll
        for (int k = 0; k < 4; ++k) { gr[k] = g[r + k * rstep]; yv[k] = *reinterpret_cast<const float4*>(p.a + (r + k * rstep) * p.C + c); }
#pragma unroll
        for (int k = 0; k < 4; ++k) one_row(r + k * rstep, gr[k], yv[k]);
    }
    for (; r < p.M; r += rstep) one_row(r, g[r], *reinterpret_cast<const float4*>(p.a + r * p.C + c));
#pragma unroll
    for (int j = 0; j < 4; ++j) { s_part[threadIdx.x * 13 + j] = s1[j]; s_part[threadIdx.x * 13 + 4 + j] = s2[j]; s_part[threadIdx.x * 13 + 8 + j] = s3[j]; }
    s_part[threadIdx.x * 13 + 12] = s4;
    __syncthreads();
    const int blk_q0 = (int)(((long)blockIdx.x * blockDim.x) % QC);
    float* dst = p.part + (long)blockIdx.x * (3 * p.C + 4);
    for (int qq = threadIdx.x; qq < QC; qq += blockDim.x) {
        float a1[4] = {0.f, 0.f, 0.f, 0.f}, a2[4] = {0.f, 0.f, 0.f, 0.f}, a3[4] = {0.f, 0.f, 0.f, 0.f}, a4 = 0.f;
        for (int tt = (qq - blk_q0 + QC) % QC; tt < (int)blockDim.x; tt += QC) {
#pragma unroll
            for (int j = 0; j < 4; ++j) { a1[j] += s_part[tt * 13 + j]; a2[j] += s_part[tt * 13 + 4 + j]; a3[j] += s_part[tt * 13 + 8 + j]; }
            a4 += s_part[tt * 13 + 12];
        }
#pragma unroll
        for (int j = 0; j < 4; ++j) { dst[qq * 4 + j] = a1[j]; dst[p.C + qq * 4 + j] = a2[j]; dst[2 * p.C + qq * 4 + j] = a3[j]; }
        if (qq == 0) { dst[3 * p.C] = a4; dst[3 * p.C + 1] = 0.f; dst[3 * p.C + 2] = 0.f; dst[3 * p.C + 3] = 0.f; }
    }
}

__global__ __launch_bounds__(256) void bn_rowdot_bwd_apply_kernel(ChanArgs p, const float* __restrict__ g, const float* __restrict__ w, float* __restrict__ dy,
                                                                 float* dgamma, float* dbeta, float* dw, float* db, int training) {
    const uint32_t k0e = p.k0 ^ (p.seed ? p.seed[0] : 0u), k1e = p.k1 + (p.seed ? p.seed[1] : 0u);
    const int QC = p.C >> 2;
    const long T = (long)gridDim.x * blockDim.x, t0 = (long)blockIdx.x * blockDim.x + threadIdx.x;
    const int c = (int)(t0 % QC) * 4;
    const long rstep = T / QC;
    const double invM = 1.0 / (double)p.M;
    float mu[4], rs[4], ga[4], be[4], wv[4], sg[4], sgx[4];
#pragma unroll
    for (int j = 0; j < 4; ++j) {
        mu[j] = p.mean[c + j]; rs[j] = p.rstd[c + j]; ga[j] = p.gamma[c + j]; be[j] = p.beta[c + j]; wv[j] = w[c + j];
        sg[j] = training ? (float)(p.ws[c + j] * invM) : 0.f;
        sgx[j] = training ? (float)(p.ws[p.C + c + j] * invM) : 0.f;
    }
    for (long row = t0 / QC; row < p.M; row += rstep) {
        const float gr = g[row];
        const float4 yv = *reinterpret_cast<const float4*>(p.a + row * p.C + c);
        const float y4[4] = {yv.x, yv.y, yv.z, yv.w};
        float ds[4] = {1.f, 1.f, 1.f, 1.f};
        if (p.drop_p > 0.f) {
            const float4 q4 = mdvit_drop_scale4(k0e, k1e, (uint32_t)((row / p.rows_per_sample) * p.C + c), p.thresh, p.inv_keep);
            ds[0] = q4.x; ds[1] = q4.y; ds[2] = q4.z; ds[3] = q4.w;
        }
        float o[4];
#pragma unroll
        for (int j = 0; j < 4; ++j) {
            const float xh = (y4[j] - mu[j]) * rs[j];
            const float G = gr * wv[j] * act_grad(p.act, xh * ga[j] + be[j]) * ds[j];
            o[j] = ga[j] * rs[j] * (G - sg[j] - xh * sgx[j]);
        }
        *reinterpret_cast<float4*>(dy + row * p.C + c) = make_float4(o[0], o[1], o[2], o[3]);
    }
    if (blockIdx.x == 0 && dgamma) {
        for (int cc = threadIdx.x; cc < p.C; cc += blockDim.x) { dbeta[cc] = (float)p.ws[cc]; dgamma[cc] = (float)p.ws[p.C + cc]; dw[cc] = (float)p.ws[2 * p.C + cc]; }
        if (threadIdx.x == 0 && db) db[0] = (float)p.ws[3 * p.C];
    }
}

int chan_grid(long M, int C, int max_blocks) {
    const int QC = C / 4;
    int g = 1;
    {
        int a = QC, b = 256;
        while (b) { int t = a % b; a = b; b = t; }
        g = QC / a;
    }
    long want = ((long)M * QC + 256L * 8 - 1) / (256L * 8);
    if (want > max_blocks) want = max_blocks;
    if (want < 1) want = 1;
    long grid = (want + g - 1) / g * g;
    return (int)grid;
}

void fill_drop(ChanArgs& a, float p, uint32_t k0, uint32_t k1, int rows_per_sample) {
    a.drop_p = p; a.k0 = k0; a.k1 = k1;
    a.thresh = mdvit_drop_thresh(p);
    a.inv_keep = p > 0.f ? 1.f / (1.f - p) : 1.f;
    a.rows_per_sample = rows_per_sample > 0 ? rows_per_sample : 1;
}

}

#define LN_DISPATCH(KERN, C, ...)                                                                    \
    do {                                                                                             \
        if (C <= 64) hipLaunchKernelGGL((KERN<1>), grid, dim3(256), 0, s, __VA_ARGS__);              \
        else if (C <= 128) hipLaunchKernelGGL((KERN<2>), grid, dim3(256), 0, s, __VA_ARGS__);        \
        else if (C <= 256) hipLaunchKernelGGL((KERN<4>), grid, dim3(256), 0, s, __VA_ARGS__);        \
        else if (C <= 512) hipLaunchKernelGGL((KERN<8>), grid, dim3(256), 0, s, __VA_ARGS__);        \
        else hipLaunchKernelGGL((KERN<16>), grid, dim3(256), 0, s, __VA_ARGS__);                     \
    } while (0)

extern "C" int mdvit_layernorm_fwd(const float* x, const float* gamma, const float* beta, float* y, float* mean, float* rstd,
                                   int32_t M, int32_t C, int32_t groups, float eps, void* stream) {
    hipStream_t s = (hipStream_t)stream;
    MDVIT_CHECK_ARG(M > 0 && C > 0 && C <= 1024, MDVIT_E_SHAPE, "layernorm_fwd: need 0 < C <= 1024 (M=%d C=%d)", M, C);
    MDVIT_CHECK_ARG(groups > 0 && M % groups == 0, MDVIT_E_SHAPE, "layernorm_fwd: M=%d is not a multiple of groups=%d", M, groups);
    const int Mg = M / groups;
    if (C == 64 || C == 128 || C == 320 || C == 512) {
        dim3 grid16(min(cdiv(Mg, 16), max(1, 4096 / groups)), groups);
        if (C == 64) hipLaunchKernelGGL((ln_fwd16_kernel<1>), grid16, dim3(256), 0, s, x, gamma, beta, y, mean, rstd, Mg, eps);
        else if (C == 128) hipLaunchKernelGGL((ln_fwd16_kernel<2>), grid16, dim3(256), 0, s, x, gamma, beta, y, mean, rstd, Mg, eps);
        else if (C == 320) hipLaunchKernelGGL((ln_fwd16_kernel<5>), grid16, dim3(256), 0, s, x, gamma, beta, y, mean, rstd, Mg, eps);
        else hipLaunchKernelGGL((ln_fwd16_kernel<8>), grid16, dim3(256), 0, s, x, gamma, beta, y, mean, rstd, Mg, eps);
        MDVIT_LAUNCH_CHECK();
        return MDVIT_OK;
    }
    dim3 grid(min(cdiv(Mg, 4), max(1, 4096 / groups)), groups);
    LN_DISPATCH(ln_fwd_kernel, C, x, gamma, beta, y, mean, rstd, Mg, C, eps);
    MDVIT_LAUNCH_CHECK();
    return MDVIT_OK;
}

static thread_local const float* g_ln_dy2 = nullptr;
void mdvit_layernorm_bwd_next_dy2(const float* dy2) { g_ln_dy2 = dy2; }
static inline const float* ln_take_dy2() { const float* p = g_ln_dy2; g_ln_dy2 = nullptr; return p; }

static int layernorm_bwd_impl(const float* dy, const float* dy2, const float* x, const float* gamma, const float* mean, const float* rstd,
                              const float* add, float* dx, float* dgamma, float* dbeta, void* ws, size_t ws_bytes,
                              int32_t M, int32_t C, int32_t groups, const LnMasked& mk, void* stream, int* defer_nblk = nullptr);

extern "C" int mdvit_layernorm_bwd(const float* dy, const float* x, const float* gamma, const float* mean, const float* rstd,
                                   const float* add, float* dx, float* dgamma, float* dbeta, void* ws, size_t ws_bytes,
                                   int32_t M, int32_t C, int32_t groups, void* stream) {
    const float* dy2 = ln_take_dy2();
    LnMasked mk; memset(&mk, 0, sizeof(mk));
    return layernorm_bwd_impl(dy, dy2, x, gamma, mean, rstd, add, dx, dgamma, dbeta, ws, ws_bytes, M, C, groups, mk, stream);
}

extern "C" int mdvit_layernorm_bwd_masked(const float* dy, const float* x, const float* gamma, const float* mean, const float* rstd,
                                          const float* add, float* dx, float* dx_masked, float* dgamma, float* dbeta, void* ws, size_t ws_bytes,
                                          int32_t M, int32_t C, int32_t groups, float drop_p, uint32_t key0, uint32_t key1, const float* rowscale,
                                          int32_t rows_per_scale, const uint32_t* seed, void* stream) {
    const float* dy2 = ln_take_dy2();
    MDVIT_CHECK_ARG(C == 64 || C == 128 || C == 320 || C == 512, MDVIT_E_SHAPE, "layernorm_bwd_masked: C=%d not built (64/128/320/512)", C);
    MDVIT_CHECK_ARG(dx_masked != nullptr && drop_p >= 0.f && drop_p < 1.f && (rowscale == nullptr || rows_per_scale > 0), MDVIT_E_SHAPE,
                    "layernorm_bwd_masked: bad mask arguments");
    MDVIT_CHECK_ARG((long)M * C < (1L << 32), MDVIT_E_SHAPE, "layernorm_bwd_masked: dropout index space exceeds 2^32");
    LnMasked mk; memset(&mk, 0, sizeof(mk));
    mk.out = dx_masked; mk.drop_p = drop_p; mk.k0 = key0; mk.k1 = key1; mk.thresh = mdvit_drop_thresh(drop_p);
// ... 2 lines not shown
}

int mdvit_layernorm_bwd_parts(const float* dy, const float* x, const float* gamma, const float* mean, const float* rstd, const float* add, float* dx,
                              float* dx_masked, void* ws, size_t ws_bytes, int M, int C, int groups, float drop_p, uint32_t key0, uint32_t key1,
                              const float* rowscale, int rows_per_scale, const uint32_t* seed, hipStream_t stream, int* nblk) {
    const float* dy2 = ln_take_dy2();
    MDVIT_CHECK_ARG(C == 64 || C == 128 || C == 320 || C == 512, MDVIT_E_SHAPE, "layernorm_bwd_parts: C=%d not built (64/128/320/512)", C);
    MDVIT_CHECK_ARG(nblk != nullptr && ws != nullptr, MDVIT_E_SHAPE, "layernorm_bwd_parts: null argument");
    LnMasked mk; memset(&mk, 0, sizeof(mk));
    if (dx_masked) {
        MDVIT_CHECK_ARG((long)M * C < (1L << 32), MDVIT_E_SHAPE, "layernorm_bwd_parts: dropout index space exceeds 2^32");
        mk.out = dx_masked; mk.drop_p = drop_p; mk.k0 = key0; mk.k1 = key1; mk.thresh = mdvit_drop_thresh(drop_p);
        mk.inv_keep = drop_p > 0.f ? 1.f / (1.f - drop_p) : 1.f; mk.rowscale = rowscale; mk.rows_per_scale = rows_per_scale > 0 ? rows_per_scale : 1; mk.seed = seed;
    }
    float dummy;
    return layernorm_bwd_impl(dy, dy2, x, gamma, mean, rstd, add, dx, &dummy, &dummy, ws, ws_bytes, M, C, groups, mk, stream, nblk);
}

static int layernorm_bwd_impl(const float* dy, const float* dy2, const float* x, const float* gamma, const float* mean, const float* rstd,
                              const float* add, float* dx, float* dgamma, float* dbeta, void* ws, size_t ws_bytes,
                              int32_t M, int32_t C, int32_t groups, const LnMasked& mk_in, void* stream, int* defer_nblk) {
    hipStream_t s = (hipStream_t)stream;
    LnMasked mk = mk_in;
    mk.dy2 = dy2;
    MDVIT_CHECK_ARG(mk.dy2 == nullptr || ((C == 64 || C == 128 || C == 320 || C == 512) && aligned16(mk.dy2)), MDVIT_E_SHAPE, "layernorm_bwd: a second dy partial needs C in 64/128/320/512");
    MDVIT_CHECK_ARG(M > 0 && C > 0 && C <= 1024, MDVIT_E_SHAPE, "layernorm_bwd: need 0 < C <= 1024 (M=%d C=%d)", M, C);
    MDVIT_CHECK_ARG(groups > 0 && groups <= 64 && M % groups == 0, MDVIT_E_SHAPE, "layernorm_bwd: M=%d is not a multiple of groups=%d", M, groups);
    const int Mg = M / groups;
    const bool want_params = dgamma != nullptr || dbeta != nullptr;
    float* part = want_params ? (float*)ws : nullptr;
    int nblk;
    if (C == 64 || C == 128 || C == 320 || C == 512) {
        static const int rows_env = [] { const char* e = getenv("MDVIT_LN_BWD_ROWS"); return e ? atoi(e) : 0; }();
        const int rows_wg = rows_env > 0 ? rows_env : ((C >= 320 && (long)M * C <= (16384L * 512)) ? 16 : 64);
        nblk = min(cdiv(Mg, rows_wg), 1024 / groups);
        if (want_params) MDVIT_CHECK_PARTIALS_WS(ws, ws_bytes, nblk * groups, 2 * C, "layernorm_bwd");
        dim3 grid16(nblk, groups);
        if (C == 64) hipLaunchKernelGGL((ln_bwd16_kernel<1>), grid16, dim3(256), 0, s, dy, x, gamma, mean, rstd, add, dx, part, Mg, mk);
        else if (C == 128) hipLaunchKernelGGL((ln_bwd16_kernel<2>), grid16, dim3(256), 0, s, dy, x, gamma, mean, rstd, add, dx, part, Mg, mk);
        else if (C == 320) hipLaunchKernelGGL((ln_bwd16_kernel<5>), grid16, dim3(256), 0, s, dy, x, gamma, mean, rstd, add, dx, part, Mg, mk);
        else hipLaunchKernelGGL((ln_bwd16_kernel<8>), grid16, dim3(256), 0, s, dy, x, gamma, mean, rstd, add, dx, part, Mg, mk);
    } else {
        nblk = min(cdiv(Mg, 16), 1024 / groups);
        MDVIT_CHECK_PARTIALS_WS(ws, ws_bytes, nblk * groups, 2 * C, "layernorm_bwd");
        part = (float*)ws;
        dim3 grid(nblk, groups);
        LN_DISPATCH(ln_bwd_kernel, C, dy, x, gamma, mean, rstd, add, dx, part, Mg, C);
    }
    MDVIT_LAUNCH_CHECK();
    if (!want_params) return MDVIT_OK;
    if (defer_nblk) { *defer_nblk = nblk; return MDVIT_OK; }
    return mdvit_reduce_partials_batched2(part, groups, nblk, C, dgamma, C, dbeta, s);
}

constexpr int CHAN_MAX_BLOCKS = 512;

static size_t bn_ws_bytes(int M, int C, int groups) {
    return (size_t)groups * (sizeof(double) * 2 * (size_t)C + sizeof(float) * 2 * (size_t)C * (size_t)chan_grid(M, C, CHAN_MAX_BLOCKS));
}

extern "C" size_t mdvit_bn_ws_bytes(int32_t M, int32_t C, int32_t groups) {
    if (M <= 0 || C <= 0 || C % 4 || groups <= 0 || M % groups) return 0;
    return bn_ws_bytes(M / groups, C, groups);
}

extern "C" int mdvit_bn_stats(const float* y, void* ws, size_t ws_bytes, float* mean, float* rstd, float* running_mean, float* running_var,
                              int64_t* nbt, int32_t M, int32_t C, int32_t groups, int32_t per_group_affine, float eps, float momentum, void* stream) {
    hipStream_t s = (hipStream_t)stream;
    MDVIT_CHECK_ARG(M > 0 && C > 0 && C % 4 == 0 && C <= 4096, MDVIT_E_SHAPE, "bn_stats: need C %% 4 == 0, C <= 4096 (M=%d C=%d)", M, C);
    MDVIT_CHECK_ARG(groups > 0 && M % groups == 0, MDVIT_E_SHAPE, "bn_stats: M=%d is not a multiple of groups=%d", M, groups);
    const int Mg = M / groups;
    MDVIT_CHECK_ARG(ws_bytes >= bn_ws_bytes(Mg, C, groups), MDVIT_E_WORKSPACE, "bn_stats: workspace too small");
    ChanArgs a; memset(&a, 0, sizeof(a));
    a.a = y; a.lda = C; a.M = Mg; a.C = C; a.groups = groups; a.rows_per_group = Mg;
    a.ws = (double*)ws; a.part = (float*)((double*)ws + 2 * (size_t)C * groups);
    const int grid = chan_grid(Mg, C, CHAN_MAX_BLOCKS);
    hipLaunchKernelGGL((chan_reduce_kernel<0>), dim3(grid, groups), dim3(256), sizeof(float) * (2 * C + 256 * 8), s, a);
    hipLaunchKernelGGL(bn_stats_finalize_kernel, dim3(cdiv(C, 16)), dim3(1024), 0, s, a.part, a.ws, grid, mean, rstd, running_mean, running_var, nbt, Mg, C, eps, momentum,
                       groups, per_group_affine);
    MDVIT_LAUNCH_CHECK();
    return MDVIT_OK;
}

extern "C" int mdvit_bn_eval_prep(const float* rm, const float* rv, float* mean, float* rstd, int32_t C, float eps, void* stream) {
    hipLaunchKernelGGL(bn_eval_prep_kernel, dim3(cdiv(C, 256)), dim3(256), 0, (hipStream_t)stream, rm, rv, mean, rstd, C, eps);
    MDVIT_LAUNCH_CHECK();
    return MDVIT_OK;
}

extern "C" int mdvit_bn_apply(const float* y, const float* mean, const float* rstd, const float* gamma, const float* beta, float* z,
                              int32_t M, int32_t C, int32_t groups, int32_t per_group_affine, int32_t act, float drop2d_p, uint32_t key0, uint32_t key1,
                              const uint32_t* seed, int32_t rows_per_sample, void* stream) {
    MDVIT_CHECK_ARG(M > 0 && C > 0 && C % 4 == 0, MDVIT_E_SHAPE, "bn_apply: need C %% 4 == 0 (M=%d C=%d)", M, C);
    MDVIT_CHECK_ARG(groups > 0 && M % groups == 0, MDVIT_E_SHAPE, "bn_apply: M=%d is not a multiple of groups=%d", M, groups);
    ChanArgs a; memset(&a, 0, sizeof(a));
    a.a = y; a.mean = mean; a.rstd = rstd; a.gamma = gamma; a.beta = beta; a.M = M; a.C = C; a.act = act;
    a.groups = groups; a.rows_per_group = M / groups; a.affine_stride = per_group_affine ? C : 0;
    a.M = M / groups;
    fill_drop(a, drop2d_p, key0, key1, rows_per_sample);
    a.seed = seed;
    hipLaunchKernelGGL(bn_apply_kernel, dim3(chan_grid(a.M, C, max(1, 4096 / groups)), groups), dim3(256), 0, (hipStream_t)stream, a, z);
    MDVIT_LAUNCH_CHECK();
    return MDVIT_OK;
}

extern "C" int mdvit_bn_bwd(const float* dz, const float* y, const float* mean, const float* rstd, const float* gamma, const float* beta,
                            float* dy, float* dgamma, float* dbeta, void* ws, size_t ws_bytes, int32_t M, int32_t C, int32_t groups,
                            int32_t per_group_affine, int32_t act, int32_t training, float drop2d_p, uint32_t key0, uint32_t key1, const uint32_t* seed, int32_t rows_per_sample,
                            void* stream) {
    hipStream_t s = (hipStream_t)stream;
    MDVIT_CHECK_ARG(M > 0 && C > 0 && C % 4 == 0 && C <= 4096, MDVIT_E_SHAPE, "bn_bwd: need C %% 4 == 0, C <= 4096 (M=%d C=%d)", M, C);
    MDVIT_CHECK_ARG(groups > 0 && M % groups == 0, MDVIT_E_SHAPE, "bn_bwd: M=%d is not a multiple of groups=%d", M, groups);
    const int Mg = M / groups;
    MDVIT_CHECK_ARG(ws_bytes >= bn_ws_bytes(Mg, C, groups), MDVIT_E_WORKSPACE, "bn_bwd: workspace too small");
    ChanArgs a; memset(&a, 0, sizeof(a));
    a.a = dz; a.b = y; a.lda = C; a.mean = mean; a.rstd = rstd; a.gamma = gamma; a.beta = beta; a.M = Mg; a.C = C; a.act = act;
    a.groups = groups; a.rows_per_group = Mg; a.affine_stride = per_group_affine ? C : 0;
    a.ws = (double*)ws; a.part = (float*)((double*)ws + 2 * (size_t)C * groups);
    fill_drop(a, drop2d_p, key0, key1, rows_per_sample);
    a.seed = seed;
    const int grid = chan_grid(Mg, C, CHAN_MAX_BLOCKS);
    hipLaunchKernelGGL((chan_reduce_kernel<1>), dim3(grid, groups), dim3(256), sizeof(float) * (2 * C + 256 * 8), s, a);
    hipLaunchKernelGGL(chan_finalize_kernel, dim3(cdiv(2 * C, 32), groups), dim3(256), 0, s, a.part, a.ws, grid, 2 * C);
    hipLaunchKernelGGL(bn_bwd_apply_kernel, dim3(chan_grid(Mg, C, max(1, 4096 / groups)), groups), dim3(256), 0, s, a, dy, dgamma, dbeta, training);
    MDVIT_LAUNCH_CHECK();
    return MDVIT_OK;
}

extern "C" size_t mdvit_bn_rowdot_ws_bytes(int32_t M, int32_t C) {
    if (M <= 0 || C <= 0 || C % 4) return 0;
    return sizeof(double) * (3 * (size_t)C + 4) + sizeof(float) * (3 * (size_t)C + 4) * (size_t)chan_grid(M, C, CHAN_MAX_BLOCKS);
}

extern "C" int mdvit_bn_rowdot_fwd(const float* y, const float* mean, const float* rstd, const float* gamma, const float* beta, const float* w, const float* b,
                                   float* low, int32_t M, int32_t C, int32_t act, float drop2d_p, uint32_t key0, uint32_t key1, const uint32_t* seed,
                                   int32_t rows_per_sample, void* stream) {
    MDVIT_CHECK_ARG(M > 0 && (C == 256 || C == 512 || C == 1024), MDVIT_E_SHAPE, "bn_rowdot_fwd: built for C = 256 / 512 / 1024 (M=%d C=%d)", M, C);
    MDVIT_CHECK_ARG(y && mean && rstd && gamma && beta && w && low && aligned16(y), MDVIT_E_SHAPE, "bn_rowdot_fwd: null or misaligned operand");
    ChanArgs a; memset(&a, 0, sizeof(a));
    a.a = y; a.mean = mean; a.rstd = rstd; a.gamma = gamma; a.beta = beta; a.M = M; a.C = C; a.act = act;
    fill_drop(a, drop2d_p, key0, key1, rows_per_sample);
    a.seed = seed;
    const dim3 grid(min(cdiv(M, 4), 8192));
    if (C == 256) hipLaunchKernelGGL((bn_rowdot_fwd_kernel<1>), grid, dim3(256), 0, (hipStream_t)stream, a, w, b, low);
    else if (C == 512) hipLaunchKernelGGL((bn_rowdot_fwd_kernel<2>), grid, dim3(256), 0, (hipStream_t)stream, a, w, b, low);
    else hipLaunchKernelGGL((bn_rowdot_fwd_kernel<4>), grid, dim3(256), 0, (hipStream_t)stream, a, w, b, low);
    MDVIT_LAUNCH_CHECK();
    return MDVIT_OK;
}

extern "C" int mdvit_bn_rowdot_bwd(const float* g, const float* y, const float* mean, const float* rstd, const float* gamma, const float* beta, const float* w,
                                   float* dy, float* dgamma, float* dbeta, float* dw, float* db, void* ws, size_t ws_bytes, int32_t M, int32_t C, int32_t act,
                                   int32_t training, float drop2d_p, uint32_t key0, uint32_t key1, const uint32_t* seed, int32_t rows_per_sample, void* stream) {
    hipStream_t s = (hipStream_t)stream;
    MDVIT_CHECK_ARG(M > 0 && C > 0 && C % 4 == 0 && C <= 4096, MDVIT_E_SHAPE, "bn_rowdot_bwd: need C %% 4 == 0, C <= 4096 (M=%d C=%d)", M, C);
    MDVIT_CHECK_ARG(g && y && mean && rstd && gamma && beta && w && dy && aligned16(y) && aligned16(dy), MDVIT_E_SHAPE, "bn_rowdot_bwd: null or misaligned operand");
    MDVIT_CHECK_ARG((dgamma == nullptr) == (dbeta == nullptr) && (dgamma == nullptr) == (dw == nullptr), MDVIT_E_SHAPE,
                    "bn_rowdot_bwd: dgamma, dbeta and dw must be all given or all NULL (data gradient only)");
    MDVIT_CHECK_ARG(ws && ws_bytes >= mdvit_bn_rowdot_ws_bytes(M, C), MDVIT_E_WORKSPACE, "bn_rowdot_bwd: workspace too small (mdvit_bn_rowdot_ws_bytes)");
    ChanArgs a; memset(&a, 0, sizeof(a));
    a.a = y; a.mean = mean; a.rstd = rstd; a.gamma = gamma; a.beta = beta; a.M = M; a.C = C; a.act = act;
    a.ws = (double*)ws; a.part = (float*)((double*)ws + 3 * (size_t)C + 4);
    fill_drop(a, drop2d_p, key0, key1, rows_per_sample);
    a.seed = seed;
    const int C2 = 3 * C + 4;
    if (training || dgamma) {
        const int grid = chan_grid(M, C, CHAN_MAX_BLOCKS);
        hipLaunchKernelGGL(bn_rowdot_reduce_kernel, dim3(grid), dim3(256), sizeof(float) * 256 * 13, s, a, g, w, dgamma != nullptr);
        hipLaunchKernelGGL(chan_finalize_kernel, dim3(cdiv(C2, 32), 1), dim3(256), 0, s, a.part, a.ws, grid, C2);
    }
    hipLaunchKernelGGL(bn_rowdot_bwd_apply_kernel, dim3(chan_grid(M, C, 4096)), dim3(256), 0, s, a, g, w, dy, dgamma, dbeta, dw, db, training);
    MDVIT_LAUNCH_CHECK();
    return MDVIT_OK;
}

static int colsum_impl(const float* A, int64_t lda, float* out, float* masked, void* ws, size_t ws_bytes, int32_t M, int32_t N, float drop_p,
                       uint32_t key0, uint32_t key1, const float* rowscale, int32_t rows_per_scale, int32_t accumulate, const uint32_t* seed, void* stream, int* defer_nblk);

int mdvit_colsum_parts(const float* A, long lda, float* masked, void* ws, size_t ws_bytes, int M, int N, float drop_p, uint32_t key0, uint32_t key1,
                       const float* rowscale, int rows_per_scale, const uint32_t* seed, hipStream_t stream, int* nblk) {
    float dummy;
    return colsum_impl(A, lda, &dummy, masked, ws, ws_bytes, M, N, drop_p, key0, key1, rowscale, rows_per_scale, 0, seed, stream, nblk);
}

extern "C" int mdvit_colsum_f32(const float* A, int64_t lda, float* out, float* masked, void* ws, size_t ws_bytes, int32_t M, int32_t N, float drop_p,
                                uint32_t key0, uint32_t key1, const float* rowscale, int32_t rows_per_scale, int32_t accumulate,
                                const uint32_t* seed, void* stream) {
    return colsum_impl(A, lda, out, masked, ws, ws_bytes, M, N, drop_p, key0, key1, rowscale, rows_per_scale, accumulate, seed, stream, nullptr);
}

static int colsum_impl(const float* A, int64_t lda, float* out, float* masked, void* ws, size_t ws_bytes, int32_t M, int32_t N, float drop_p,
                       uint32_t key0, uint32_t key1, const float* rowscale, int32_t rows_per_scale, int32_t accumulate, const uint32_t* seed, void* stream,
                       int* defer_nblk) {
    hipStream_t s = (hipStream_t)stream;
    MDVIT_CHECK_ARG(M > 0 && N > 0 && N % 4 == 0 && N <= 8192 && lda % 4 == 0, MDVIT_E_SHAPE, "colsum: need N %% 4 == 0 (M=%d N=%d)", M, N);
    MDVIT_CHECK_ARG(out || masked, MDVIT_E_SHAPE, "colsum: nothing to produce (out and masked are both NULL)");
    MDVIT_CHECK_ARG((long)M * N < (1L << 32), MDVIT_E_SHAPE, "colsum: dropout index space exceeds 2^32");
    const int nblk = chan_grid(M, N, out ? 1024 : 4096);
    if (out) MDVIT_CHECK_PARTIALS_WS(ws, ws_bytes, nblk, N, "colsum");
    ChanArgs a; memset(&a, 0, sizeof(a));
    a.a = A; a.lda = lda; a.M = M; a.C = N; a.out = out; a.masked = masked; a.part = (float*)ws;
    fill_drop(a, drop_p, key0, key1, 1);
    a.seed = seed;
    a.rowscale = rowscale; a.rows_per_scale = rows_per_scale > 0 ? rows_per_scale : 1;
    hipLaunchKernelGGL((chan_reduce_kernel<2>), dim3(nblk), dim3(256), sizeof(float) * (2 * N + 256 * 4), s, a);
    MDVIT_LAUNCH_CHECK();
    if (defer_nblk) { *defer_nblk = nblk; return MDVIT_OK; }
    return out ? mdvit_reduce_partials((const float*)ws, nblk, (long)N, N, out, 0, nullptr, accumulate, s) : MDVIT_OK;
}

extern "C" int mdvit_rowdot_fwd(const float* x, int64_t ldx, const float* w, const float* b, float* y, int32_t M, int32_t K,
                                int32_t accumulate, void* stream) {
    MDVIT_CHECK_ARG(M > 0 && K > 0, MDVIT_E_SHAPE, "rowdot_fwd: bad shape M=%d K=%d", M, K);
    hipLaunchKernelGGL(rowdot_fwd_kernel, dim3(min(cdiv(M, 4), 8192)), dim3(256), 0, (hipStream_t)stream, x, (long)ldx, w, b, y, M, K, accumulate);
    MDVIT_LAUNCH_CHECK();
    return MDVIT_OK;
}

extern "C" int mdvit_rowdot_bwd(const float* x, int64_t ldx, const float* w, const float* dy, float* dx, int64_t lddx, float* dw, float* db,
                                void* ws, size_t ws_bytes, int32_t M, int32_t K, void* stream) {
    hipStream_t s = (hipStream_t)stream;
    MDVIT_CHECK_ARG(M > 0 && K > 0 && K <= 1024, MDVIT_E_SHAPE, "rowdot_bwd: need K <= 1024 (M=%d K=%d)", M, K);
    const int nblk = min(cdiv(M, 4), 1024);
    const bool want_w = dw != nullptr || db != nullptr;
    MDVIT_CHECK_ARG(want_w || dx != nullptr, MDVIT_E_SHAPE, "rowdot_bwd: nothing to produce");
    if (want_w) MDVIT_CHECK_PARTIALS_WS(ws, ws_bytes, nblk, K + 1, "rowdot_bwd");
    dim3 grid(nblk);
    const int C = K;
    float* part = want_w ? (float*)ws : nullptr;
    LN_DISPATCH(rowdot_bwd_kernel, C, x, (long)ldx, w, dy, dx, (long)lddx, part, db != nullptr, M, K);
    MDVIT_LAUNCH_CHECK();
    if (!want_w) return MDVIT_OK;
    return mdvit_reduce_partials(part, nblk, (long)K + 1, K, dw, 1, db, 0, s);
}
```

### mdvit_amd/decode.py

```python
from __future__ import annotations

import os

import torch
from torch import nn

from . import ops
from ._lib import ACT_RELU
from .blocks import BatchNormAct, ConvParams, DecoderDWConv2d_BN, _NoParams, _check_norm


class UnetDecodingBlockTransformer(nn.Module):
    def __init__(self, in_channel, out_channel, mhsa_block, use_res=False, conv_norm=nn.BatchNorm2d, dsn=0):
        super().__init__()
        if use_res:
            raise NotImplementedError("use_res=True is never used by the reference's models")
        self.use_res = use_res
        self.conv_before = ConvParams(out_channel, in_channel, 1, 1, bias=True)
        self.conv_after = DecoderDWConv2d_BN(out_channel * 2, out_channel, norm_layer=conv_norm, dsn=dsn)
        self.mhsa_block = mhsa_block

    def forward(self, input, skip, domain_label=None):
        B, H, W, Cout = skip.shape
        low = ops.linear(input, self.conv_before.weight, self.conv_before.bias)
        up = ops.upsample_bilinear(low, H, W)
        z = self.conv_after(skip, up)
        t = self.mhsa_block(z.view(B, H * W, Cout), H, W, domain_label)
        return t.view(B, H, W, Cout)


_COMPOSE_GROUPED = os.environ.get("MDVIT_COMPOSE_GROUPED", "1") != "0"
_LOWS_GROUPED = os.environ.get("MDVIT_LOWS_GROUPED", "1") != "0"
_WT_BATCH = os.environ.get("MDVIT_WT_BATCH", "1") != "0"
_HEAD_CAT = os.environ.get("MDVIT_HEAD_CAT", "1") != "0"


class MLPDecoderFM(nn.Module):
    def __init__(self, in_channels, out_channel, hidden_channel=256, outfeature_channel=64, dropout_ratio=0.1, conv_norm=nn.BatchNorm2d):
        super().__init__()
        _check_norm(conv_norm)
        assert out_channel == 1
        self.linear1 = ConvParams(hidden_channel, in_channels[0], 1, 1)
        self.linear2 = ConvParams(hidden_channel, in_channels[1], 1, 1)
        self.linear3 = ConvParams(hidden_channel, in_channels[2], 1, 1)
        self.linear4 = ConvParams(hidden_channel, in_channels[3], 1, 1)
        self.linear_fuse = nn.Sequential(ConvParams(hidden_channel, hidden_channel * 4 + outfeature_channel, 1, 1),
                                         BatchNormAct(hidden_channel, ACT_RELU), _NoParams())
        self.dropout = nn.Dropout2d(dropout_ratio)
        self.linear_out = ConvParams(out_channel, hidden_channel, 1, 1)
        self.hidden = hidden_channel
        self.with_fm = outfeature_channel > 0

    def fuse_blocks(self):
        hid = self.hidden
        Wf = self.linear_fuse[0].weight.view(hid, -1)
        if not self.with_fm:
            return Wf, None
        return ops.split_cols(Wf, [4 * hid, Wf.shape[1] - 4 * hid])

    @staticmethod
    def compose_many(heads):
        blocks = [h.fuse_blocks() for h in heads]
        lins = [(h.linear1, h.linear2, h.linear3, h.linear4) for h in heads]
        if not _COMPOSE_GROUPED:
            hid = heads[0].hidden
            return [(blocks[g][1], [(ops.matmul(blocks[g][0][:, q * hid:(q + 1) * hid], l.weight.view(hid, -1)), ops.rowdot(blocks[g][0][:, q * hid:(q + 1) * hid], l.bias))
                                    for q, l in enumerate(lins[g])]) for g in range(len(heads))]
        comp = ops.compose_heads([b[0] for b in blocks], [[l.weight for l in ls] for ls in lins], [[l.bias for l in ls] for ls in lins])
        cat = _HEAD_CAT and all(h.with_fm for h in heads)
        if cat:
            for g, h in enumerate(heads):
                comp[g].append((torch.cat([comp[g][0][0], blocks[g][1]], 1), comp[g][0][1] + h.linear_fuse[0].bias))
        if _WT_BATCH and ops._gemm_precision >= 1 and torch.is_grad_enabled():
            ops.transpose_weights_batch([w for g in range(len(heads)) for (w, _) in (comp[g][1:] if cat else comp[g])] + ([] if cat else [blocks[g][1] for g in range(len(heads))]))
        return [(blocks[g][1], comp[g]) for g in range(len(heads))]

    @staticmethod
    def grouped_lows(composed, feats_per_head):
        G = len(composed)
        if G < 2 or not _LOWS_GROUPED or any(c is None for c in composed):
            return composed
        h, w = feats_per_head[0][0].shape[1:3]
        out = [dict() for _ in range(G)]
        for q in range(4):
            f0 = feats_per_head[0][q]
            if (f0.shape[1] == h and f0.shape[2] == w) or f0.shape[-1] in (64, 128) or not f0.is_cuda:
                continue
            ys = ops.linear_grouped([feats_per_head[g][q] for g in range(G)], [composed[g][1][q][0] for g in range(G)], [composed[g][1][q][1] for g in range(G)])
            for g in range(G):
                out[g][q] = ys[g]
        return [(composed[g][0], composed[g][1], out[g]) for g in range(G)]

    def forward(self, features, img_size, out_feat=False, composed=None):
        if out_feat:
            raise NotImplementedError("out_feat=True of the aux head is unused by the train path")
        x1 = features[0]
        B, h, w, _ = x1.shape
        hid = self.hidden
        bias = self.linear_fuse[0].bias
        W5, comp = (composed if composed is not None else MLPDecoderFM.compose_many([self])[0])[:2]
        pre = composed[2] if (composed is not None and len(composed) > 2) else {}
        lows = []
        q0 = 0
        if self.with_fm and len(comp) > 4 and features[0].shape[1:3] == features[4].shape[1:3]:
            Wcat, bcat = comp[4]
            acc = ops.linear(ops.cat_channels(features[0], features[4]), Wcat, bcat)
            q0 = 1
        else:
            acc = ops.linear(features[4], W5, bias) if self.with_fm else None
        for q in range(q0, 4):
            Wc, bc = comp[q]
            fq = features[q]
            if acc is None:
                assert fq.shape[1] == h and fq.shape[2] == w
                acc = ops.linear(fq, Wc, bc + bias)
            elif fq.shape[1] == h and fq.shape[2] == w:
                acc = ops.linear(fq, Wc, bc, residual=acc)
            elif q in pre:
                lows.append(pre[q])
            else:
                lows.append(ops.linear(fq, Wc, bc))
        if lows:
            acc = ops.upsample_sum(acc, lows, h, w)
        p = self.dropout.p if self.training else 0.0
        bn = self.linear_fuse[1]
        low = ops.bn_act_rowdot(acc, bn.weight, bn.bias, bn.running_mean, bn.running_var, bn.num_batches_tracked, bn.training, bn.act,
                                self.linear_out.weight, self.linear_out.bias, bn.eps, bn.momentum, p)
        out = ops.upsample_bilinear(low.view(B, h, w, 1), int(img_size[0]), int(img_size[1]))
        return out.view(B, 1, int(img_size[0]), int(img_size[1]))


class MLPDecoder(MLPDecoderFM):

    def __init__(self, in_channels, out_channel, hidden_channel=256, dropout_ratio=0.1, conv_norm=nn.BatchNorm2d):
        super().__init__(in_channels, out_channel, hidden_channel, outfeature_channel=0, dropout_ratio=dropout_ratio, conv_norm=conv_norm)


class _ASPP(nn.Module):

    def __init__(self, in_channels, atrous_rates, out_channels=256):
        super().__init__()
        mods = [nn.Sequential(ConvParams(out_channels, in_channels, 1, 1, bias=False), BatchNormAct(out_channels, ACT_RELU), _NoParams())]
        for _ in atrous_rates:
            mods.append(nn.Sequential(ConvParams(out_channels, in_channels, 3, 3, bias=False), BatchNormAct(out_channels, ACT_RELU), _NoParams()))
        mods.append(nn.Sequential(_NoParams(), ConvParams(out_channels, in_channels, 1, 1, bias=False), BatchNormAct(out_channels, ACT_RELU), _NoParams()))
        self.convs = nn.ModuleList(mods)
        self.project = nn.Sequential(ConvParams(out_channels, (len(atrous_rates) + 2) * out_channels, 1, 1, bias=False),
                                     BatchNormAct(out_channels, ACT_RELU), _NoParams(), nn.Dropout(0.1))
        self.rates = tuple(atrous_rates)
        self.out_channels = out_channels

    def forward(self, x):
        B, h, w, _ = x.shape
        oc = self.out_channels
        xs = ops.fork(x, len(self.rates) + 2)
        res = [self.convs[0][1](ops.linear(xs[0], self.convs[0][0].weight.view(oc, -1)))]
        for i, r in enumerate(self.rates, start=1):
            res.append(self.convs[i][1](ops.conv3x3_dense(xs[i], self.convs[i][0].weight, None, 1, dilation=r)))
        pool = self.convs[-1]
        pooled = ops.linear(ops.global_avg_pool(xs[-1]), pool[1].weight.view(oc, -1)).view(B, 1, 1, oc)
        res.append(ops.upsample_bilinear(pool[2](pooled), h, w))
        y = self.project[1](ops.linear(torch.cat(res, dim=-1), self.project[0].weight.view(oc, -1)))
        return ops.dropout(y, self.project[3].p, self.training)


class DeepLabV3Decoder(nn.Module):

    def __init__(self, in_channel, out_channel, aspp_dilate=(6, 12, 18), conv_norm=nn.BatchNorm2d):
        super().__init__()
        _check_norm(conv_norm)
        assert out_channel == 1
        self.classifier = nn.Sequential(_ASPP(in_channel, aspp_dilate), ConvParams(256, 256, 3, 3, bias=False), BatchNormAct(256, ACT_RELU),
                                        _NoParams(), ConvParams(out_channel, 256, 1, 1))

    def forward(self, features, img_size, out_feat=False):
        x = features[3] if isinstance(features, (list, tuple)) else features
        c = self.classifier
        y = ops.conv3x3_dense(c[0](x), c[1].weight, None, 1)
        B, h, w, _ = y.shape
        bn = c[2]
        low = ops.bn_act_rowdot(y, bn.weight, bn.bias, bn.running_mean, bn.running_var, bn.num_batches_tracked, bn.training, bn.act, c[4].weight, c[4].bias,
                                bn.eps, bn.momentum, 0.0)
        out = ops.upsample_bilinear(low.view(B, h, w, 1), int(img_size[0]), int(img_size[1]))
        return out.view(B, 1, int(img_size[0]), int(img_size[1]))
```

### mdvit_amd/ops.py

```python
from __future__ import annotations

import ctypes as C
import itertools
import os
import weakref
from typing import Optional, Tuple

import torch

from . import _lib
from ._lib import GemmDesc, call

_key_counter = itertools.count(1)
_POISON = os.environ.get("MDVIT_POISON", "0") == "1"


def _empty(*a, **k):
    t = torch.empty(*a, **k)
    if _POISON and t.is_floating_point():
        t.fill_(float("nan"))
    return t


def _empty_like(x):
# ... 1977 lines not shown
    groups = _bn_groups if (training or gamma.dim() == 2) else 1
    if groups > 1 and y.shape[0] % groups:
        raise ValueError(f"bn_groups({groups}) needs a batch that is a multiple of it, got {y.shape[0]}")
    return _BNAct.apply(_c(y), _c(gamma), _c(beta), running_mean, running_var, nbt, bool(training), float(eps), float(momentum),
                        int(act), float(drop2d_p), int(rows_per_sample), int(groups))


class _Upsample(torch.autograd.Function):
    @staticmethod
    def forward(ctx, x, Ho, Wo, base):
        ctx.set_materialize_grads(False)
        _chk(x, base)
        B, H, W_, Cn = x.shape
        y = _empty((B, Ho, Wo, Cn), device=x.device, dtype=torch.float32)
        call("mdvit_upsample_fwd", _p(x), _p(base), _p(y), B, H, W_, Ho, Wo, Cn, _stream())
        ctx.meta = (B, H, W_, Ho, Wo, Cn, base is not None)
        return y

    @staticmethod
    def backward(ctx, g):
        if g is None:
            return (None,) * 4
        B, H, W_, Ho, Wo, Cn, has_base = ctx.meta
        g = _c(g)
        dx = _empty((B, H, W_, Cn), device=g.device, dtype=torch.float32)
        wsb = _lib.load().mdvit_upsample_bwd_ws_bytes(B, H, W_, Ho, Wo, Cn)
        ws = _empty((wsb // 4,), device=g.device, dtype=torch.float32)
        call("mdvit_upsample_bwd", _p(g), _p(dx), _p(ws), wsb, B, H, W_, Ho, Wo, Cn, _stream())
        return dx, None, None, (g if has_base else None)


def upsample_bilinear(x, Ho, Wo, base=None):
    if base is None and x.shape[1] == Ho and x.shape[2] == Wo:
        return x
    return _Upsample.apply(_c(x), int(Ho), int(Wo), None if base is None else _c(base))


class _UpsampleSum(torch.autograd.Function):

    @staticmethod
    def forward(ctx, base, Ho, Wo, *xs):
        ctx.set_materialize_grads(False)
        _chk(base, *xs)
        B, _, _, Cn = xs[0].shape
        n = len(xs)
        y = _empty((B, Ho, Wo, Cn), device=xs[0].device, dtype=torch.float32)
        ptrs = (C.c_void_p * n)(*[x.data_ptr() for x in xs])
        Hi = (C.c_int32 * n)(*[x.shape[1] for x in xs])
        Wi = (C.c_int32 * n)(*[x.shape[2] for x in xs])
        call("mdvit_upsample_multi_fwd", ptrs, Hi, Wi, n, _p(base), _p(y), B, Ho, Wo, Cn, _stream())
        ctx.meta = (B, Ho, Wo, Cn, [(x.shape[1], x.shape[2]) for x in xs], base is not None)
        return y

    @staticmethod
    def backward(ctx, g):
        B, Ho, Wo, Cn, dims, has_base = ctx.meta
        if g is None:
            return (None,) * (3 + len(dims))
        g = _c(g)
        n = len(dims)
        dxs = [_empty((B, h, w, Cn), device=g.device, dtype=torch.float32) for h, w in dims]
        ptrs = (C.c_void_p * n)(*[t.data_ptr() for t in dxs])
        Hi = (C.c_int32 * n)(*[h for h, _ in dims])
        Wi = (C.c_int32 * n)(*[w for _, w in dims])
        wsb = _lib.load().mdvit_upsample_multi_bwd_ws_bytes(Wi, n, B, Ho, Cn)
        ws = _empty((wsb // 4,), device=g.device, dtype=torch.float32)
        call("mdvit_upsample_multi_bwd", _p(g), ptrs, Hi, Wi, n, _p(ws), wsb, B, Ho, Wo, Cn, _stream())
        return (g if has_base else None, None, None, *dxs)


def upsample_sum(base, xs, Ho, Wo):
    xs = [_c(x) for x in xs]
    out = base
    while xs:
        chunk, xs = xs[:3], xs[3:]
        if chunk[0].shape[-1] % 4 or not chunk[0].is_cuda:
            for x in chunk:
                out = upsample_bilinear(x, Ho, Wo, base=out)
            continue
        out = _UpsampleSum.apply(None if out is None else _c(out), int(Ho), int(Wo), *chunk)
    return out


class _RowDot(torch.autograd.Function):
    @staticmethod
    def forward(ctx, x, w, b):
        ctx.set_materialize_grads(False)
        _chk(w, b)
        M, K, ldx = _ld_view(x)
        y = _empty((M,), device=x.device, dtype=torch.float32)
        call("mdvit_rowdot_fwd", _p(x), ldx, _p(w), _p(b), _p(y), M, K, 0, _stream())
        ctx.save_for_backward(x, w)
        ctx.has_b = b is not None
        return y

    @staticmethod
    def backward(ctx, g):
        if g is None:
            return (None,) * 3
        x, w = ctx.saved_tensors
        g = _c(g)
        M, K, ldx = _ld_view(x)
        dx = _empty((M, K), device=x.device, dtype=torch.float32) if ctx.needs_input_grad[0] else None
        if _dgrad_only:
            if dx is not None:
                call("mdvit_rowdot_bwd", _p(x), ldx, _p(w), _p(g), _p(dx), K, None, None, None, 0, M, K, _stream())
            return dx, None, None
        dw, db = _flat_like(w.reshape(-1), (1,) if ctx.has_b else None)
        wsp, wsb, _keep = _partials_ws(K + 1, g.device)
        call("mdvit_rowdot_bwd", _p(x), ldx, _p(w), _p(g), _p(dx), K, _p(dw), _p(db), wsp, wsb, M, K, _stream())
        return dx, dw.view_as(w), db


def rowdot(x, w, b=None):
    if x.dim() == 2:
        return _RowDot.apply(x, w, b)
    shp = x.shape
    return _RowDot.apply(_c(x).view(-1, shp[-1]), w, b).view(shp[:-1])


SE_KINDS = {"dase": _lib.SE_DASE, "use": _lib.SE_USE}


def _se_desc(kind, B, N, Cn, r, W1, b1, W2, b2, Wg, bg):
    d = _lib.SeAdapterDesc()
    d.kind, d.B, d.N, d.C, d.r = kind, B, N, Cn, r
    d.W1, d.b1, d.W2, d.b2, d.Wg, d.bg = _p(W1), _p(b1), _p(W2), _p(b2), _p(Wg), _p(bg)
    return d


def _se_sizes(d):
    lib = _lib.load()
    save, ws = lib.mdvit_se_adapter_save_bytes(C.byref(d)), lib.mdvit_se_adapter_ws_bytes(C.byref(d))
    if not save or not ws:
        raise _lib.MdvitHipError("se_adapter: " + lib.mdvit_last_error().decode(errors="replace"))
    return save, ws


class _SeAdapter(torch.autograd.Function):

    @staticmethod
    def forward(ctx, x, kind, *params):
        ctx.set_materialize_grads(False)
        _chk(x, *params)
        if x.dim() != 3:
            raise _lib.MdvitHipError("se_adapter: x must be [B, N, C] tokens")
        B, N, Cn = x.shape
        if kind == _lib.SE_DASE:
            if len(params) != 18:
                raise _lib.MdvitHipError("se_adapter: DASE takes (Wg, bg) and four (W1, b1, W2, b2) branches")
            Wg, bg = params[0], params[1]
            with torch.no_grad():
                W1, b1, W2, b2 = (torch.stack([params[2 + 4 * k + i] for k in range(4)]) for i in range(4))
        elif kind == _lib.SE_USE:
            if len(params) != 4:
                raise _lib.MdvitHipError("se_adapter: USE takes (W1, b1, W2, b2)")
            (W1, b1, W2, b2), Wg, bg = params, None, None
        else:
            raise _lib.MdvitHipError(f"se_adapter: unknown kind {kind!r}")
        r = W1.shape[-2]
        d = _se_desc(kind, B, N, Cn, r, W1, b1, W2, b2, Wg, bg)
        save_b, ws_b = _se_sizes(d)
        y = _empty_like(x)
        save = _empty((save_b // 4,), device=x.device, dtype=torch.float32)
        ws = torch.empty((ws_b // 4,), device=x.device, dtype=torch.float32)
        call("mdvit_se_adapter_fwd", C.byref(d), _p(x), _p(y), _p(save), _p(ws), ws_b, _stream())
# ... 711 lines not shown
```

Measured before the change: 512.6 images/s.

## Fuse decoder upsample-sum with BN statistics and fold upsample backward into BN-rowdot backward

In training, the decoder head's multi-source upsample-sum tile kernel now also accumulates per-block channel sums and squares. A small finalize kernel reduces these into BN mean/rstd and running stats, so the separate BN stats pass over the full-resolution feature map is no longer needed. The backward pass gets a combined bn_rowdot+upsample backward entry that folds the width-direction upsample gradient into the BN backward. This cuts passes over a large activation tensor, at the cost of new workspace, a narrower set of supported shapes, and a different summation order for the statistics.

```diff
diff --git a/include/mdvit_hip.h b/include/mdvit_hip.h
--- a/include/mdvit_hip.h
+++ b/include/mdvit_hip.h
@@ -265,6 +265,16 @@
 int mdvit_upsample_multi_bwd(const float* dy, float* const* dxs, const int32_t* Hi, const int32_t* Wi, int32_t n, void* ws, size_t ws_bytes, int32_t B,
                              int32_t Ho, int32_t Wo, int32_t C, void* stream);
 
+size_t mdvit_upsample_multi_stats_ws_bytes(const int32_t* Hi, const int32_t* Wi, int32_t n, int32_t B, int32_t Ho, int32_t Wo, int32_t C);
+int mdvit_upsample_multi_fwd_stats(const float* const* xs, const int32_t* Hi, const int32_t* Wi, int32_t n, const float* base, float* y, void* ws, size_t ws_bytes,
+                                   int32_t B, int32_t Ho, int32_t Wo, int32_t C, void* stream);
+int mdvit_bn_stats_finalize(void* ws, size_t ws_bytes, int32_t nblk, float* mean, float* rstd, float* running_mean, float* running_var,
+                            int64_t* num_batches_tracked, int32_t M, int32_t C, float eps, float momentum, void* stream);
+int mdvit_bn_rowdot_upsample_bwd(const float* g, const float* y, const float* mean, const float* rstd, const float* gamma, const float* beta, const float* w,
+                                 float* dy, float* dgamma, float* dbeta, float* dw, float* db , void* ws, size_t ws_bytes, float* const* dxs,
+                                 const int32_t* Hi, const int32_t* Wi, int32_t n, void* up_ws, size_t up_ws_bytes, int32_t B, int32_t Ho, int32_t Wo, int32_t C,
+                                 int32_t act, int32_t training, float drop2d_p, uint32_t key0, uint32_t key1, const uint32_t* drop_seed, void* stream);
+
 int mdvit_da_fwd(const float* label, const float* W1, const float* b1, const float* W2, const float* b2, float* a,
                  int32_t B, int32_t D, int32_t hid, int32_t C, int32_t heads, void* stream);
 #define MDVIT_DA_MANY_MAX 32
diff --git a/mdvit_amd/_lib.py b/mdvit_amd/_lib.py
--- a/mdvit_amd/_lib.py
+++ b/mdvit_amd/_lib.py
@@ -219,6 +219,10 @@
     "mdvit_bn_bwd": [vp, vp, vp, vp, vp, vp, vp, vp, vp, vp, C.c_size_t, i32, i32, i32, i32, i32, i32, f32, u32, u32, vp, i32, vp],
     "mdvit_upsample_multi_fwd": [vp, vp, vp, i32, vp, vp, i32, i32, i32, i32, vp],
     "mdvit_upsample_multi_bwd": [vp, vp, vp, vp, i32, vp, C.c_size_t, i32, i32, i32, i32, vp],
+    "mdvit_upsample_multi_fwd_stats": [vp, vp, vp, i32, vp, vp, vp, C.c_size_t, i32, i32, i32, i32, vp],
+    "mdvit_bn_stats_finalize": [vp, C.c_size_t, i32, vp, vp, vp, vp, vp, i32, i32, f32, f32, vp],
+    "mdvit_bn_rowdot_upsample_bwd": [vp, vp, vp, vp, vp, vp, vp, vp, vp, vp, vp, vp, vp, C.c_size_t, vp, vp, vp, i32, vp, C.c_size_t, i32, i32, i32, i32, i32, i32, f32, u32, u32,
+                                     vp, vp],
     "mdvit_upsample_fwd": [vp, vp, vp, i32, i32, i32, i32, i32, i32, vp],
     "mdvit_upsample_bwd": [vp, vp, vp, C.c_size_t, i32, i32, i32, i32, i32, i32, vp],
     "mdvit_da_fwd": [vp, vp, vp, vp, vp, vp, i32, i32, i32, i32, i32, vp],
@@ -305,6 +309,8 @@
     lib.mdvit_bn_ws_bytes.argtypes = [i32, i32, i32]
     lib.mdvit_upsample_multi_bwd_ws_bytes.restype = C.c_size_t
     lib.mdvit_upsample_multi_bwd_ws_bytes.argtypes = [vp, i32, i32, i32, i32]
+    lib.mdvit_upsample_multi_stats_ws_bytes.restype = C.c_size_t
+    lib.mdvit_upsample_multi_stats_ws_bytes.argtypes = [vp, vp, i32, i32, i32, i32, i32]
     lib.mdvit_upsample_bwd_ws_bytes.restype = C.c_size_t
     lib.mdvit_upsample_bwd_ws_bytes.argtypes = [i32] * 6
     lib.mdvit_partials_ws_bytes.restype = C.c_size_t
diff --git a/mdvit_amd/build.py b/mdvit_amd/build.py
--- a/mdvit_amd/build.py
+++ b/mdvit_amd/build.py
@@ -35,7 +35,7 @@
 def _compile(src: str) -> str:
     obj = os.path.join(OBJ, os.path.splitext(src)[0] + ".o")
     stamp = obj + ".sha"
-    deps = [os.path.join(CSRC, src), os.path.join(CSRC, "common.h"), os.path.join(CSRC, "conv_tile.h"), os.path.join(CSRC, "gemm_body.inc"), os.path.join(CSRC, "gemm_bp.h"), os.path.join(CSRC, "augment_taps.h"),
+    deps = [os.path.join(CSRC, src), os.path.join(CSRC, "common.h"), os.path.join(CSRC, "conv_tile.h"), os.path.join(CSRC, "gemm_body.inc"), os.path.join(CSRC, "gemm_bp.h"), os.path.join(CSRC, "augment_taps.h"), os.path.join(CSRC, "upsample_fold.h"),
             os.path.join(HERE, "..", "include", "mdvit_hip.h")]
     extra = EXTRA_FLAGS.get(src, [])
     dig = _digest(deps) + " ".join(extra)
diff --git a/mdvit_amd/csrc/conv.hip b/mdvit_amd/csrc/conv.hip
--- a/mdvit_amd/csrc/conv.hip
+++ b/mdvit_amd/csrc/conv.hip
@@ -1,5 +1,6 @@
 #include "common.h"
 #include "conv_tile.h"
+#include "upsample_fold.h"
 
 namespace {
 
@@ -500,15 +501,6 @@
             part[(long)blockIdx.x * Cout * KK + (cb + co) * KK + k] = t;
         }
     }
-}
-
-__device__ __forceinline__ void bilin_src(int o, int in_size, float scale, int& i0, int& i1, float& l1) {
-    float src = scale * ((float)o + 0.5f) - 0.5f;
-    if (src < 0.f) src = 0.f;
-    i0 = (int)src;
-    if (i0 > in_size - 1) i0 = in_size - 1;
-    i1 = i0 + (i0 < in_size - 1 ? 1 : 0);
-    l1 = src - (float)i0;
 }
 
 __global__ __launch_bounds__(256) void upsample_fwd_kernel(const float* __restrict__ x, const float* base_, float* y,
@@ -551,21 +543,6 @@
     }
 }
 
-__device__ __forceinline__ void out_range(int i, int in_size, int out_size, int& lo, int& hi) {
-    if (out_size % in_size == 0 && ((out_size / in_size) & 1) == 0) {
-        const int s = out_size / in_size;
-        lo = s * i - s / 2; hi = s * i + 3 * s / 2;
-        if (lo < 0) lo = 0;
-        if (hi > out_size) hi = out_size;
-        return;
-    }
-    const float inv = (float)out_size / (float)in_size;
-    lo = (int)floorf(((float)i - 1.0f) * inv) - 1;
-    hi = (int)ceilf(((float)i + 2.0f) * inv) + 1;
-    if (lo < 0) lo = 0;
-    if (hi > out_size) hi = out_size;
-}
-
 template <bool ALONG_W>
 __global__ __launch_bounds__(256) void upsample_bwd_pass_kernel(const float* __restrict__ src, float* __restrict__ dst,
                                                                 long outer, int n_in, int n_out, long inner_q, int vec) {
@@ -599,11 +576,6 @@
     }
 }
 
-struct UpMulti {
-    const float* x[3]; float* d[3];
-    int Hi[3], Wi[3];
-    int n;
-};
 
 __global__ __launch_bounds__(256) void upsample_multi_fwd_kernel(UpMulti p, const float* base_, float* __restrict__ y, int B, int Ho, int Wo, int C) {
     const int QC = C >> 2;
@@ -650,7 +622,9 @@
 }
 
 constexpr int UT_H = 8, UT_W = 16, UT_C = 128, UT_POOL = 96;
-__global__ __launch_bounds__(256) void upsample_multi_tile_kernel(UpMulti p, const float* __restrict__ base_, float* __restrict__ y, int Ho, int Wo, int C) {
+template <bool STATS>
+__global__ __launch_bounds__(256) void upsample_multi_tile_kernel(UpMulti p, const float* __restrict__ base_, float* __restrict__ y, float* __restrict__ stat_part,
+                                                                  int Ho, int Wo, int C) {
     __shared__ __attribute__((aligned(16))) float s_src[UT_POOL * UT_C];
     const int tiles_w = Wo / UT_W;
     const int ty = blockIdx.x / tiles_w, tx = blockIdx.x - ty * tiles_w;
@@ -685,6 +659,7 @@
     }
     __syncthreads();
     const int cq = threadIdx.x & 31, colh = threadIdx.x >> 5;
+    float4 s1 = make_float4(0.f, 0.f, 0.f, 0.f), s2 = make_float4(0.f, 0.f, 0.f, 0.f);
 #pragma unroll 2
     for (int it = 0; it < UT_H * 2; ++it) {
         const int ho = ho0 + (it >> 1), wo = wo0 + (it & 1) * 8 + colh;
@@ -709,6 +684,24 @@
             o = (i == 0 && !base_) ? uu : f4_add(uu, o);
         }
         *reinterpret_cast<float4*>(y + oi) = o;
+        if (STATS) {
+            s1 = f4_add(s1, o);
+            s2.x = fmaf(o.x, o.x, s2.x); s2.y = fmaf(o.y, o.y, s2.y); s2.z = fmaf(o.z, o.z, s2.z); s2.w = fmaf(o.w, o.w, s2.w);
+        }
+    }
+    if (STATS) {
+        __syncthreads();
+        *reinterpret_cast<float4*>(s_src + threadIdx.x * 8) = s1;
+        *reinterpret_cast<float4*>(s_src + threadIdx.x * 8 + 4) = s2;
+        __syncthreads();
+        if (threadIdx.x < 64) {
+            const int which = threadIdx.x >> 5;
+            float4 a = make_float4(0.f, 0.f, 0.f, 0.f);
+#pragma unroll
+            for (int l = 0; l < 8; ++l) a = f4_add(a, *reinterpret_cast<const float4*>(s_src + (l * 32 + cq) * 8 + 4 * which));
+            const long row = (long)b * gridDim.x + blockIdx.x;
+            *reinterpret_cast<float4*>(stat_part + row * 2 * C + (long)which * C + c0 + 4 * cq) = a;
+        }
     }
 }
 
@@ -754,27 +747,7 @@
         *reinterpret_cast<float4*>(s_row + t * 32 + 4 * q) = *reinterpret_cast<const float4*>(src + (long)t * C + 4 * q);
     }
     __syncthreads();
-    const int Wsum = p.Wi[0] + (p.n > 1 ? p.Wi[1] : 0) + (p.n > 2 ? p.Wi[2] : 0);
-    float* dsts[3] = {p.d[0], p.d[1], p.d[2]};
-    for (int e = threadIdx.x; e < Wsum * 8; e += 256) {
-        const int q = e & 7;
-        int j = e >> 3, sidx = 0;
-        if (j >= p.Wi[0]) { j -= p.Wi[0]; sidx = 1; if (j >= p.Wi[1]) { j -= p.Wi[1]; sidx = 2; } }
-        const int Wi = p.Wi[sidx];
-        const float sc = (float)Wi / (float)Wo;
-        int lo, hi;
-        out_range(j, Wi, Wo, lo, hi);
-        float4 acc = make_float4(0.f, 0.f, 0.f, 0.f);
-#pragma unroll 4
-        for (int t = lo; t < hi; ++t) {
-            int i0, i1; float l;
-            bilin_src(t, Wi, sc, i0, i1, l);
-            const float wgt = (i0 == j ? 1.f - l : 0.f) + (i1 == j ? l : 0.f);
-            const float4 g = *reinterpret_cast<const float4*>(s_row + t * 32 + 4 * q);
-            acc.x = fmaf(wgt, g.x, acc.x); acc.y = fmaf(wgt, g.y, acc.y); acc.z = fmaf(wgt, g.z, acc.z); acc.w = fmaf(wgt, g.w, acc.w);
-        }
-        *reinterpret_cast<float4*>(dsts[sidx] + (o * Wi + j) * C + c0 + 4 * q) = acc;
-    }
+    upsample_fold_row_lds(p, s_row, o, c0, Wo, C);
 }
 
 __global__ __launch_bounds__(256) void dropout_kernel(const float* __restrict__ x, float* __restrict__ y, long n4, uint32_t k0, uint32_t k1,
@@ -987,8 +960,44 @@
     return MDVIT_OK;
 }
 
+static bool upsample_tile_ok(const int32_t* Hi, const int32_t* Wi, int n, int B, int Ho, int Wo, int C) {
+    bool ok = Ho % UT_H == 0 && Wo % UT_W == 0 && C % UT_C == 0 && (long)(Ho / UT_H) * (Wo / UT_W) < (1L << 30) && C / UT_C < 65536 && B < 65536;
+    int pool = 0;
+    for (int i = 0; i < n && ok; ++i) {
+        if (Hi[i] <= 0 || Wi[i] <= 0) return false;
+        const int fh = Ho / Hi[i], fw = Wo / Wi[i];
+        ok = Ho % Hi[i] == 0 && Wo % Wi[i] == 0 && fh >= 2 && fw >= 2 && fh <= 16 && fw <= 16 && (fh & (fh - 1)) == 0 && (fw & (fw - 1)) == 0;
+        if (ok) pool += (UT_H / fh + 2) * (UT_W / fw + 2);
+    }
+    return ok && pool <= UT_POOL;
+}
+
+static int upsample_multi_fwd_impl(const float* const* xs, const int32_t* Hi, const int32_t* Wi, int32_t n, const float* base, float* y, float* stat_part, int32_t B,
+                                   int32_t Ho, int32_t Wo, int32_t C, void* stream);
+
 extern "C" int mdvit_upsample_multi_fwd(const float* const* xs, const int32_t* Hi, const int32_t* Wi, int32_t n, const float* base, float* y, int32_t B, int32_t Ho,
                                         int32_t Wo, int32_t C, void* stream) {
+    return upsample_multi_fwd_impl(xs, Hi, Wi, n, base, y, nullptr, B, Ho, Wo, C, stream);
+}
+
+extern "C" size_t mdvit_upsample_multi_stats_ws_bytes(const int32_t* Hi, const int32_t* Wi, int32_t n, int32_t B, int32_t Ho, int32_t Wo, int32_t C) {
+    if (!Hi || !Wi || n < 1 || n > 3 || B <= 0 || Ho <= 0 || Wo <= 0 || C <= 0 || !upsample_tile_ok(Hi, Wi, n, B, Ho, Wo, C)) return 0;
+    const size_t nblk = (size_t)B * (Ho / UT_H) * (Wo / UT_W);
+    return sizeof(double) * 2 * (size_t)C + sizeof(float) * 2 * (size_t)C * nblk;
+}
+
+extern "C" int mdvit_upsample_multi_fwd_stats(const float* const* xs, const int32_t* Hi, const int32_t* Wi, int32_t n, const float* base, float* y, void* ws,
+                                              size_t ws_bytes, int32_t B, int32_t Ho, int32_t Wo, int32_t C, void* stream) {
+    MDVIT_CHECK_ARG(n >= 1 && n <= 3 && B > 0 && Ho > 0 && Wo > 0 && C > 0 && C % 4 == 0, MDVIT_E_SHAPE, "upsample_multi_fwd_stats: 1..3 sources, C %% 4 == 0 (n=%d C=%d)", n, C);
+    const size_t need = mdvit_upsample_multi_stats_ws_bytes(Hi, Wi, n, B, Ho, Wo, C);
+    MDVIT_CHECK_ARG(need > 0, MDVIT_E_SHAPE, "upsample_multi_fwd_stats: shape not built for the tile kernel (mdvit_upsample_multi_stats_ws_bytes is 0): use "
+                    "mdvit_upsample_multi_fwd + mdvit_bn_stats");
+    MDVIT_CHECK_ARG(ws && aligned16(ws) && ws_bytes >= need, MDVIT_E_WORKSPACE, "upsample_multi_fwd_stats: workspace too small (mdvit_upsample_multi_stats_ws_bytes)");
+    return upsample_multi_fwd_impl(xs, Hi, Wi, n, base, y, (float*)((double*)ws + 2 * (size_t)C), B, Ho, Wo, C, stream);
+}
+
+static int upsample_multi_fwd_impl(const float* const* xs, const int32_t* Hi, const int32_t* Wi, int32_t n, const float* base, float* y, float* stat_part, int32_t B,
+                                   int32_t Ho, int32_t Wo, int32_t C, void* stream) {
     MDVIT_CHECK_ARG(n >= 1 && n <= 3 && B > 0 && Ho > 0 && Wo > 0 && C > 0 && C % 4 == 0, MDVIT_E_SHAPE, "upsample_multi_fwd: 1..3 sources, C %% 4 == 0 (n=%d C=%d)", n, C);
     UpMulti p; memset(&p, 0, sizeof(p));
     p.n = n;
@@ -997,20 +1006,14 @@
         p.x[i] = xs[i]; p.Hi[i] = Hi[i]; p.Wi[i] = Wi[i];
     }
     MDVIT_CHECK_ARG(aligned16(y) && (!base || aligned16(base)), MDVIT_E_ALIGN, "upsample_multi_fwd: y / base must be 16-byte aligned");
-    {
-        bool ok = Ho % UT_H == 0 && Wo % UT_W == 0 && C % UT_C == 0 && (long)(Ho / UT_H) * (Wo / UT_W) < (1L << 30) && C / UT_C < 65536 && B < 65536;
-        int pool = 0;
-        for (int i = 0; i < n && ok; ++i) {
-            const int fh = Ho / Hi[i], fw = Wo / Wi[i];
-            ok = Ho % Hi[i] == 0 && Wo % Wi[i] == 0 && fh >= 2 && fw >= 2 && fh <= 16 && fw <= 16 && (fh & (fh - 1)) == 0 && (fw & (fw - 1)) == 0;
-            if (ok) pool += (UT_H / fh + 2) * (UT_W / fw + 2);
-        }
-        if (ok && pool <= UT_POOL) {
-            hipLaunchKernelGGL(upsample_multi_tile_kernel, dim3((Ho / UT_H) * (Wo / UT_W), C / UT_C, B), dim3(256), 0, (hipStream_t)stream, p, base, y, Ho, Wo, C);
-            MDVIT_LAUNCH_CHECK();
-            return MDVIT_OK;
-        }
-    }
+    if (upsample_tile_ok(Hi, Wi, n, B, Ho, Wo, C)) {
+        const dim3 grid((Ho / UT_H) * (Wo / UT_W), C / UT_C, B);
+        if (stat_part) hipLaunchKernelGGL((upsample_multi_tile_kernel<true>), grid, dim3(256), 0, (hipStream_t)stream, p, base, y, stat_part, Ho, Wo, C);
+        else hipLaunchKernelGGL((upsample_multi_tile_kernel<false>), grid, dim3(256), 0, (hipStream_t)stream, p, base, y, stat_part, Ho, Wo, C);
+        MDVIT_LAUNCH_CHECK();
+        return MDVIT_OK;
+    }
+    MDVIT_CHECK_ARG(!stat_part, MDVIT_E_SHAPE, "upsample_multi_fwd_stats: shape not built for the tile kernel");
     MDVIT_CHECK_ARG((long)Wo * (C / 4) < (1L << 30), MDVIT_E_SHAPE, "upsample_multi_fwd: output row too long");
     const long nunits = (long)B * Ho * (((long)Wo * (C / 4) + 1023) >> 10);
     hipLaunchKernelGGL(upsample_multi_fwd_kernel, dim3((unsigned)min(nunits, 16384L)), dim3(256), 0, (hipStream_t)stream, p, base, y, B, Ho, Wo, C);
@@ -1026,7 +1029,11 @@
 
 extern "C" int mdvit_upsample_multi_bwd(const float* dy, float* const* dxs, const int32_t* Hi, const int32_t* Wi, int32_t n, void* ws, size_t ws_bytes, int32_t B,
                                         int32_t Ho, int32_t Wo, int32_t C, void* stream) {
-    hipStream_t s = (hipStream_t)stream;
+    return mdvit_upsample_multi_bwd_run(dy, dxs, Hi, Wi, n, ws, ws_bytes, B, Ho, Wo, C, 1, (hipStream_t)stream);
+}
+
+int mdvit_upsample_multi_bwd_run(const float* dy, float* const* dxs, const int32_t* Hi, const int32_t* Wi, int n, void* ws, size_t ws_bytes, int B, int Ho, int Wo,
+                                 int C, int w_fold, hipStream_t s) {
     MDVIT_CHECK_ARG(n >= 1 && n <= 3 && B > 0 && Ho > 0 && Wo > 0 && C > 0 && C % 4 == 0, MDVIT_E_SHAPE, "upsample_multi_bwd: 1..3 sources, C %% 4 == 0 (n=%d C=%d)", n, C);
     MDVIT_CHECK_ARG(ws && ws_bytes >= mdvit_upsample_multi_bwd_ws_bytes(Wi, n, B, Ho, C) && aligned16(ws) && aligned16(dy), MDVIT_E_WORKSPACE,
                     "upsample_multi_bwd: workspace too small (mdvit_upsample_multi_bwd_ws_bytes)");
@@ -1043,9 +1050,9 @@
     const long cq = C / 4;
     const int bpr = (int)cdiv((long)wsum * cq, 256L);
     MDVIT_CHECK_ARG((long)B * Ho * bpr < (1L << 31), MDVIT_E_SHAPE, "upsample_multi_bwd: too many workgroups");
-    if (C % 32 == 0 && Wo <= 384 && (long)B * Ho < (1L << 31) && C / 32 <= 65535)
+    if (w_fold && upsample_fold_lds_ok(B, Ho, Wo, C))
         hipLaunchKernelGGL(upsample_multi_bwd_w_lds_kernel, dim3((unsigned)((long)B * Ho), C / 32), dim3(256), sizeof(float) * Wo * 32, s, p, dy, Wo, C);
-    else
+    else if (w_fold)
         hipLaunchKernelGGL(upsample_multi_bwd_w_kernel, dim3((unsigned)((long)B * Ho * bpr)), dim3(256), 0, s, p, dy, (long)B * Ho, Wo, C, bpr);
     for (int i = 0; i < n; ++i)
         hipLaunchKernelGGL((upsample_bwd_pass_kernel<false>), dim3(ew_grid((long)B * Hi[i] * Wi[i] * cq)), dim3(256), 0, s, p.d[i], dxs[i], (long)B, Hi[i], Ho,
diff --git a/mdvit_amd/csrc/norm.hip b/mdvit_amd/csrc/norm.hip
--- a/mdvit_amd/csrc/norm.hip
+++ b/mdvit_amd/csrc/norm.hip
@@ -1,4 +1,5 @@
 #include "common.h"
+#include "upsample_fold.h"
 
 namespace {
 
@@ -657,6 +658,37 @@
     }
 }
 
+struct RowdotConsts { float mu[4], rs[4], ga[4], be[4], wv[4], sg[4], sgx[4]; };
+__device__ __forceinline__ void bn_rowdot_consts(const ChanArgs& p, const float* __restrict__ w, int c, int training, RowdotConsts& k) {
+    const double invM = 1.0 / (double)p.M;
+#pragma unroll
+    for (int j = 0; j < 4; ++j) {
+        k.mu[j] = p.mean[c + j]; k.rs[j] = p.rstd[c + j]; k.ga[j] = p.gamma[c + j]; k.be[j] = p.beta[c + j]; k.wv[j] = w[c + j];
+        k.sg[j] = training ? (float)(p.ws[c + j] * invM) : 0.f;
+        k.sgx[j] = training ? (float)(p.ws[p.C + c + j] * invM) : 0.f;
+    }
+}
+__device__ __forceinline__ float4 bn_rowdot_dy4(const ChanArgs& p, const RowdotConsts& k, uint32_t k0e, uint32_t k1e, long row, int c, float gr, float4 yv) {
+    const float y4[4] = {yv.x, yv.y, yv.z, yv.w};
+    float ds[4] = {1.f, 1.f, 1.f, 1.f};
+    if (p.drop_p > 0.f) {
+        const float4 q4 = mdvit_drop_scale4(k0e, k1e, (uint32_t)((row / p.rows_per_sample) * p.C + c), p.thresh, p.inv_keep);
+        ds[0] = q4.x; ds[1] = q4.y; ds[2] = q4.z; ds[3] = q4.w;
+    }
+    float o[4];
+#pragma unroll
+    for (int j = 0; j < 4; ++j) {
+        const float xh = (y4[j] - k.mu[j]) * k.rs[j];
+        const float G = gr * k.wv[j] * act_grad(p.act, xh * k.ga[j] + k.be[j]) * ds[j];
+        o[j] = k.ga[j] * k.rs[j] * (G - k.sg[j] - xh * k.sgx[j]);
+    }
+    return make_float4(o[0], o[1], o[2], o[3]);
+}
+__device__ __forceinline__ void bn_rowdot_param_grads(const ChanArgs& p, float* dgamma, float* dbeta, float* dw, float* db) {
+    for (int cc = threadIdx.x; cc < p.C; cc += blockDim.x) { dbeta[cc] = (float)p.ws[cc]; dgamma[cc] = (float)p.ws[p.C + cc]; dw[cc] = (float)p.ws[2 * p.C + cc]; }
+    if (threadIdx.x == 0 && db) db[0] = (float)p.ws[3 * p.C];
+}
+
 __global__ __launch_bounds__(256) void bn_rowdot_bwd_apply_kernel(ChanArgs p, const float* __restrict__ g, const float* __restrict__ w, float* __restrict__ dy,
                                                                  float* dgamma, float* dbeta, float* dw, float* db, int training) {
     const uint32_t k0e = p.k0 ^ (p.seed ? p.seed[0] : 0u), k1e = p.k1 + (p.seed ? p.seed[1] : 0u);
@@ -664,36 +696,50 @@
     const long T = (long)gridDim.x * blockDim.x, t0 = (long)blockIdx.x * blockDim.x + threadIdx.x;
     const int c = (int)(t0 % QC) * 4;
     const long rstep = T / QC;
-    const double invM = 1.0 / (double)p.M;
-    float mu[4], rs[4], ga[4], be[4], wv[4], sg[4], sgx[4];
-#pragma unroll
-    for (int j = 0; j < 4; ++j) {
-        mu[j] = p.mean[c + j]; rs[j] = p.rstd[c + j]; ga[j] = p.gamma[c + j]; be[j] = p.beta[c + j]; wv[j] = w[c + j];
-        sg[j] = training ? (float)(p.ws[c + j] * invM) : 0.f;
-        sgx[j] = training ? (float)(p.ws[p.C + c + j] * invM) : 0.f;
-    }
+    RowdotConsts k;
+    bn_rowdot_consts(p, w, c, training, k);
     for (long row = t0 / QC; row < p.M; row += rstep) {
         const float gr = g[row];
         const float4 yv = *reinterpret_cast<const float4*>(p.a + row * p.C + c);
-        const float y4[4] = {yv.x, yv.y, yv.z, yv.w};
-        float ds[4] = {1.f, 1.f, 1.f, 1.f};
-        if (p.drop_p > 0.f) {
-            const float4 q4 = mdvit_drop_scale4(k0e, k1e, (uint32_t)((row / p.rows_per_sample) * p.C + c), p.thresh, p.inv_keep);
-            ds[0] = q4.x; ds[1] = q4.y; ds[2] = q4.z; ds[3] = q4.w;
-        }
-        float o[4];
-#pragma unroll
-        for (int j = 0; j < 4; ++j) {
-            const float xh = (y4[j] - mu[j]) * rs[j];
-            const float G = gr * wv[j] * act_grad(p.act, xh * ga[j] + be[j]) * ds[j];
-            o[j] = ga[j] * rs[j] * (G - sg[j] - xh * sgx[j]);
-        }
-        *reinterpret_cast<float4*>(dy + row * p.C + c) = make_float4(o[0], o[1], o[2], o[3]);
-    }
-    if (blockIdx.x == 0 && dgamma) {
-        for (int cc = threadIdx.x; cc < p.C; cc += blockDim.x) { dbeta[cc] = (float)p.ws[cc]; dgamma[cc] = (float)p.ws[p.C + cc]; dw[cc] = (float)p.ws[2 * p.C + cc]; }
-        if (threadIdx.x == 0 && db) db[0] = (float)p.ws[3 * p.C];
-    }
+        *reinterpret_cast<float4*>(dy + row * p.C + c) = bn_rowdot_dy4(p, k, k0e, k1e, row, c, gr, yv);
+    }
+    if (blockIdx.x == 0 && dgamma) bn_rowdot_param_grads(p, dgamma, dbeta, dw, db);
+}
+
+__global__ __launch_bounds__(256) void bn_rowdot_bwd_apply_fold_kernel(ChanArgs p, const float* __restrict__ g, const float* __restrict__ w, float* __restrict__ dy,
+                                                                      float* dgamma, float* dbeta, float* dw, float* db, int training, UpMulti u, int Wo) {
+    extern __shared__ __attribute__((aligned(16))) float s_row[];
+    const uint32_t k0e = p.k0 ^ (p.seed ? p.seed[0] : 0u), k1e = p.k1 + (p.seed ? p.seed[1] : 0u);
+    const long o = blockIdx.x;
+    const int c0 = blockIdx.y * 32, q = threadIdx.x & 7, c = c0 + 4 * q;
+    RowdotConsts k;
+    bn_rowdot_consts(p, w, c, training, k);
+    const float* __restrict__ yrow = p.a + o * Wo * p.C + c;
+    const float* __restrict__ grow = g + o * Wo;
+    float* drow = dy + o * Wo * p.C + c;
+    const int items = Wo * 8;
+    int e = threadIdx.x;
+    for (; e + 3 * 256 < items; e += 4 * 256) {
+        float gr[4]; float4 yv[4];
+#pragma unroll
+        for (int i = 0; i < 4; ++i) { const int t = (e >> 3) + 32 * i; gr[i] = grow[t]; yv[i] = *reinterpret_cast<const float4*>(yrow + (long)t * p.C); }
+#pragma unroll
+        for (int i = 0; i < 4; ++i) {
+            const int t = (e >> 3) + 32 * i;
+            const float4 d4 = bn_rowdot_dy4(p, k, k0e, k1e, o * Wo + t, c, gr[i], yv[i]);
+            *reinterpret_cast<float4*>(drow + (long)t * p.C) = d4;
+            *reinterpret_cast<float4*>(s_row + t * 32 + 4 * q) = d4;
+        }
+    }
+    for (; e < items; e += 256) {
+        const int t = e >> 3;
+        const float4 d4 = bn_rowdot_dy4(p, k, k0e, k1e, o * Wo + t, c, grow[t], *reinterpret_cast<const float4*>(yrow + (long)t * p.C));
+        *reinterpret_cast<float4*>(drow + (long)t * p.C) = d4;
+        *reinterpret_cast<float4*>(s_row + t * 32 + 4 * q) = d4;
+    }
+    __syncthreads();
+    upsample_fold_row_lds(u, s_row, o, c0, Wo, p.C);
+    if (blockIdx.x == 0 && blockIdx.y == 0 && dgamma) bn_rowdot_param_grads(p, dgamma, dbeta, dw, db);
 }
 
 int chan_grid(long M, int C, int max_blocks) {
@@ -862,6 +908,18 @@
     return MDVIT_OK;
 }
 
+extern "C" int mdvit_bn_stats_finalize(void* ws, size_t ws_bytes, int32_t nblk, float* mean, float* rstd, float* running_mean, float* running_var, int64_t* nbt,
+                                       int32_t M, int32_t C, float eps, float momentum, void* stream) {
+    MDVIT_CHECK_ARG(M > 0 && C > 0 && C % 4 == 0 && C <= 4096 && nblk > 0, MDVIT_E_SHAPE, "bn_stats_finalize: need C %% 4 == 0, C <= 4096, nblk > 0 (M=%d C=%d nblk=%d)", M, C, nblk);
+    MDVIT_CHECK_ARG(mean && rstd && (running_mean == nullptr) == (running_var == nullptr), MDVIT_E_SHAPE, "bn_stats_finalize: null mean / rstd, or one running statistic without the other");
+    MDVIT_CHECK_ARG(ws && ws_bytes >= sizeof(double) * 2 * (size_t)C + sizeof(float) * 2 * (size_t)C * (size_t)nblk, MDVIT_E_WORKSPACE, "bn_stats_finalize: workspace too small");
+    double* sums = (double*)ws;
+    hipLaunchKernelGGL(bn_stats_finalize_kernel, dim3(cdiv(C, 16)), dim3(1024), 0, (hipStream_t)stream, (const float*)(sums + 2 * (size_t)C), sums, nblk, mean, rstd, running_mean,
+                       running_var, nbt, M, C, eps, momentum, 1, 0);
+    MDVIT_LAUNCH_CHECK();
+    return MDVIT_OK;
+}
+
 extern "C" int mdvit_bn_eval_prep(const float* rm, const float* rv, float* mean, float* rstd, int32_t C, float eps, void* stream) {
     hipLaunchKernelGGL(bn_eval_prep_kernel, dim3(cdiv(C, 256)), dim3(256), 0, (hipStream_t)stream, rm, rv, mean, rstd, C, eps);
     MDVIT_LAUNCH_CHECK();
@@ -929,9 +987,10 @@
     return MDVIT_OK;
 }
 
-extern "C" int mdvit_bn_rowdot_bwd(const float* g, const float* y, const float* mean, const float* rstd, const float* gamma, const float* beta, const float* w,
-                                   float* dy, float* dgamma, float* dbeta, float* dw, float* db, void* ws, size_t ws_bytes, int32_t M, int32_t C, int32_t act,
-                                   int32_t training, float drop2d_p, uint32_t key0, uint32_t key1, const uint32_t* seed, int32_t rows_per_sample, void* stream) {
+static int bn_rowdot_bwd_impl(const float* g, const float* y, const float* mean, const float* rstd, const float* gamma, const float* beta, const float* w,
+                              float* dy, float* dgamma, float* dbeta, float* dw, float* db, void* ws, size_t ws_bytes, int32_t M, int32_t C, int32_t act,
+                              int32_t training, float drop2d_p, uint32_t key0, uint32_t key1, const uint32_t* seed, int32_t rows_per_sample, const UpMulti* fold,
+                              long fold_rows, int Wo, void* stream) {
     hipStream_t s = (hipStream_t)stream;
     MDVIT_CHECK_ARG(M > 0 && C > 0 && C % 4 == 0 && C <= 4096, MDVIT_E_SHAPE, "bn_rowdot_bwd: need C %% 4 == 0, C <= 4096 (M=%d C=%d)", M, C);
     MDVIT_CHECK_ARG(g && y && mean && rstd && gamma && beta && w && dy && aligned16(y) && aligned16(dy), MDVIT_E_SHAPE, "bn_rowdot_bwd: null or misaligned operand");
@@ -949,9 +1008,53 @@
         hipLaunchKernelGGL(bn_rowdot_reduce_kernel, dim3(grid), dim3(256), sizeof(float) * 256 * 13, s, a, g, w, dgamma != nullptr);
         hipLaunchKernelGGL(chan_finalize_kernel, dim3(cdiv(C2, 32), 1), dim3(256), 0, s, a.part, a.ws, grid, C2);
     }
-    hipLaunchKernelGGL(bn_rowdot_bwd_apply_kernel, dim3(chan_grid(M, C, 4096)), dim3(256), 0, s, a, g, w, dy, dgamma, dbeta, dw, db, training);
+    if (fold)
+        hipLaunchKernelGGL(bn_rowdot_bwd_apply_fold_kernel, dim3((unsigned)fold_rows, C / 32), dim3(256), sizeof(float) * Wo * 32, s, a, g, w, dy, dgamma, dbeta, dw, db, training,
+                           *fold, Wo);
+    else
+        hipLaunchKernelGGL(bn_rowdot_bwd_apply_kernel, dim3(chan_grid(M, C, 4096)), dim3(256), 0, s, a, g, w, dy, dgamma, dbeta, dw, db, training);
     MDVIT_LAUNCH_CHECK();
     return MDVIT_OK;
+}
+
+extern "C" int mdvit_bn_rowdot_bwd(const float* g, const float* y, const float* mean, const float* rstd, const float* gamma, const float* beta, const float* w,
+                                   float* dy, float* dgamma, float* dbeta, float* dw, float* db, void* ws, size_t ws_bytes, int32_t M, int32_t C, int32_t act,
+                                   int32_t training, float drop2d_p, uint32_t key0, uint32_t key1, const uint32_t* seed, int32_t rows_per_sample, void* stream) {
+    return bn_rowdot_bwd_impl(g, y, mean, rstd, gamma, beta, w, dy, dgamma, dbeta, dw, db, ws, ws_bytes, M, C, act, training, drop2d_p, key0, key1, seed, rows_per_sample,
+                              nullptr, 0, 0, stream);
+}
+
+extern "C" int mdvit_bn_rowdot_upsample_bwd(const float* g, const float* y, const float* mean, const float* rstd, const float* gamma, const float* beta, const float* w,
+                                            float* dy, float* dgamma, float* dbeta, float* dw, float* db, void* ws, size_t ws_bytes, float* const* dxs, const int32_t* Hi,
+                                            const int32_t* Wi, int32_t n, void* up_ws, size_t up_ws_bytes, int32_t B, int32_t Ho, int32_t Wo, int32_t C, int32_t act,
+                                            int32_t training, float drop2d_p, uint32_t key0, uint32_t key1, const uint32_t* seed, void* stream) {
+    MDVIT_CHECK_ARG(n >= 1 && n <= 3 && B > 0 && Ho > 0 && Wo > 0 && C > 0 && C % 4 == 0 && (long)B * Ho * Wo < (1L << 31), MDVIT_E_SHAPE,
+                    "bn_rowdot_upsample_bwd: 1..3 sources, C %% 4 == 0, B Ho Wo < 2^31 (n=%d C=%d)", n, C);
+    MDVIT_CHECK_ARG(dxs && Hi && Wi, MDVIT_E_SHAPE, "bn_rowdot_upsample_bwd: null source arrays");
+    const int M = B * Ho * Wo, rps = Ho * Wo;
+    if (!upsample_fold_lds_ok(B, Ho, Wo, C)) {
+        const int rc = bn_rowdot_bwd_impl(g, y, mean, rstd, gamma, beta, w, dy, dgamma, dbeta, dw, db, ws, ws_bytes, M, C, act, training, drop2d_p, key0, key1, seed, rps,
+                                          nullptr, 0, 0, stream);
+        if (rc != MDVIT_OK) return rc;
+        return mdvit_upsample_multi_bwd_run(dy, dxs, Hi, Wi, n, up_ws, up_ws_bytes, B, Ho, Wo, C, 1, (hipStream_t)stream);
+    }
+    size_t need = 0;
+    for (int i = 0; i < n; ++i) {
+        MDVIT_CHECK_ARG(dxs[i] && Hi[i] > 0 && Wi[i] > 0 && aligned16(dxs[i]), MDVIT_E_SHAPE, "bn_rowdot_upsample_bwd: bad source %d", i);
+        need += sizeof(float) * (size_t)B * Ho * Wi[i] * C;
+    }
+    MDVIT_CHECK_ARG(up_ws && aligned16(up_ws) && up_ws_bytes >= need, MDVIT_E_WORKSPACE, "bn_rowdot_upsample_bwd: fold workspace too small (mdvit_upsample_multi_bwd_ws_bytes)");
+    UpMulti u; memset(&u, 0, sizeof(u));
+    u.n = n;
+    float* t = (float*)up_ws;
+    for (int i = 0; i < n; ++i) {
+        u.Hi[i] = Hi[i]; u.Wi[i] = Wi[i]; u.d[i] = t;
+        t += (size_t)B * Ho * Wi[i] * C;
+    }
+    const int rc = bn_rowdot_bwd_impl(g, y, mean, rstd, gamma, beta, w, dy, dgamma, dbeta, dw, db, ws, ws_bytes, M, C, act, training, drop2d_p, key0, key1, seed, rps, &u,
+                                      (long)B * Ho, Wo, stream);
+    if (rc != MDVIT_OK) return rc;
+    return mdvit_upsample_multi_bwd_run(dy, dxs, Hi, Wi, n, up_ws, up_ws_bytes, B, Ho, Wo, C, 0, (hipStream_t)stream);
 }
 
 static int colsum_impl(const float* A, int64_t lda, float* out, float* masked, void* ws, size_t ws_bytes, int32_t M, int32_t N, float drop_p,
diff --git a/mdvit_amd/csrc/upsample_fold.h b/mdvit_amd/csrc/upsample_fold.h
--- /dev/null
+++ b/mdvit_amd/csrc/upsample_fold.h
@@ -0,0 +1,61 @@
+#pragma once
+
+#include "common.h"
+
+__device__ __forceinline__ void bilin_src(int o, int in_size, float scale, int& i0, int& i1, float& l1) {
+    float src = scale * ((float)o + 0.5f) - 0.5f;
+    if (src < 0.f) src = 0.f;
+    i0 = (int)src;
+    if (i0 > in_size - 1) i0 = in_size - 1;
+    i1 = i0 + (i0 < in_size - 1 ? 1 : 0);
+    l1 = src - (float)i0;
+}
+
+__device__ __forceinline__ void out_range(int i, int in_size, int out_size, int& lo, int& hi) {
+    if (out_size % in_size == 0 && ((out_size / in_size) & 1) == 0) {
+        const int s = out_size / in_size;
+        lo = s * i - s / 2; hi = s * i + 3 * s / 2;
+        if (lo < 0) lo = 0;
+        if (hi > out_size) hi = out_size;
+        return;
+    }
+    const float inv = (float)out_size / (float)in_size;
+    lo = (int)floorf(((float)i - 1.0f) * inv) - 1;
+    hi = (int)ceilf(((float)i + 2.0f) * inv) + 1;
+    if (lo < 0) lo = 0;
+    if (hi > out_size) hi = out_size;
+}
+
+struct UpMulti {
+    const float* x[3]; float* d[3];
+    int Hi[3], Wi[3];
+    int n;
+};
+
+__device__ __forceinline__ void upsample_fold_row_lds(const UpMulti& p, const float* s_row, long o, int c0, int Wo, int C) {
+    const int Wsum = p.Wi[0] + (p.n > 1 ? p.Wi[1] : 0) + (p.n > 2 ? p.Wi[2] : 0);
+    float* dsts[3] = {p.d[0], p.d[1], p.d[2]};
+    for (int e = threadIdx.x; e < Wsum * 8; e += 256) {
+        const int q = e & 7;
+        int j = e >> 3, sidx = 0;
+        if (j >= p.Wi[0]) { j -= p.Wi[0]; sidx = 1; if (j >= p.Wi[1]) { j -= p.Wi[1]; sidx = 2; } }
+        const int Wi = p.Wi[sidx];
+        const float sc = (float)Wi / (float)Wo;
+        int lo, hi;
+        out_range(j, Wi, Wo, lo, hi);
+        float4 acc = make_float4(0.f, 0.f, 0.f, 0.f);
+#pragma unroll 4
+        for (int t = lo; t < hi; ++t) {
+            int i0, i1; float l;
+            bilin_src(t, Wi, sc, i0, i1, l);
+            const float wgt = (i0 == j ? 1.f - l : 0.f) + (i1 == j ? l : 0.f);
+            const float4 g = *reinterpret_cast<const float4*>(s_row + t * 32 + 4 * q);
+            acc.x = fmaf(wgt, g.x, acc.x); acc.y = fmaf(wgt, g.y, acc.y); acc.z = fmaf(wgt, g.z, acc.z); acc.w = fmaf(wgt, g.w, acc.w);
+        }
+        *reinterpret_cast<float4*>(dsts[sidx] + (o * Wi + j) * C + c0 + 4 * q) = acc;
+    }
+}
+
+int mdvit_upsample_multi_bwd_run(const float* dy, float* const* dxs, const int32_t* Hi, const int32_t* Wi, int n, void* ws, size_t ws_bytes, int B, int Ho, int Wo,
+                                 int C, int w_fold, hipStream_t stream);
+static inline bool upsample_fold_lds_ok(int B, int Ho, int Wo, int C) { return C % 32 == 0 && Wo <= 384 && (long)B * Ho < (1L << 31) && C / 32 <= 65535; }
diff --git a/mdvit_amd/decode.py b/mdvit_amd/decode.py
--- a/mdvit_amd/decode.py
+++ b/mdvit_amd/decode.py
@@ -33,6 +33,9 @@
 _LOWS_GROUPED = os.environ.get("MDVIT_LOWS_GROUPED", "1") != "0"
 _WT_BATCH = os.environ.get("MDVIT_WT_BATCH", "1") != "0"
 _HEAD_CAT = os.environ.get("MDVIT_HEAD_CAT", "1") != "0"
+
+
+_HEAD_TAIL = os.environ.get("MDVIT_HEAD_TAIL", "1") != "0"
 
 
 class MLPDecoderFM(nn.Module):
@@ -120,10 +123,15 @@
                 lows.append(pre[q])
             else:
                 lows.append(ops.linear(fq, Wc, bc))
+        p = self.dropout.p if self.training else 0.0
+        bn = self.linear_fuse[1]
+        if lows and _HEAD_TAIL and bn.training and len(lows) <= 3:
+            low = ops.upsample_sum_bn_rowdot(acc, lows, h, w, bn.weight, bn.bias, bn.running_mean, bn.running_var, bn.num_batches_tracked, True, bn.act,
+                                             self.linear_out.weight, self.linear_out.bias, bn.eps, bn.momentum, p)
+            out = ops.upsample_bilinear(low.view(B, h, w, 1), int(img_size[0]), int(img_size[1]))
+            return out.view(B, 1, int(img_size[0]), int(img_size[1]))
         if lows:
             acc = ops.upsample_sum(acc, lows, h, w)
-        p = self.dropout.p if self.training else 0.0
-        bn = self.linear_fuse[1]
         low = ops.bn_act_rowdot(acc, bn.weight, bn.bias, bn.running_mean, bn.running_var, bn.num_batches_tracked, bn.training, bn.act,
                                 self.linear_out.weight, self.linear_out.bias, bn.eps, bn.momentum, p)
         out = ops.upsample_bilinear(low.view(B, h, w, 1), int(img_size[0]), int(img_size[1]))
diff --git a/mdvit_amd/ops.py b/mdvit_amd/ops.py
--- a/mdvit_amd/ops.py
+++ b/mdvit_amd/ops.py
@@ -2083,6 +2083,82 @@
     return out
 
 
+class _UpsampleSumBNRowDot(torch.autograd.Function):
+
+    @staticmethod
+    def forward(ctx, base, gamma, beta, running_mean, running_var, nbt, w, b, eps, momentum, act, drop2d_p, Ho, Wo, *xs):
+        ctx.set_materialize_grads(False)
+        _chk(base, gamma, beta, running_mean, running_var, w, b, *xs)
+        B, _, _, Cn = xs[0].shape
+        n = len(xs)
+        dev = xs[0].device
+        M = B * Ho * Wo
+        lib = _lib.load()
+        y = _empty((B, Ho, Wo, Cn), device=dev, dtype=torch.float32)
+        ptrs = (C.c_void_p * n)(*[x.data_ptr() for x in xs])
+        Hi = (C.c_int32 * n)(*[x.shape[1] for x in xs])
+        Wi = (C.c_int32 * n)(*[x.shape[2] for x in xs])
+        wsb = lib.mdvit_upsample_multi_stats_ws_bytes(Hi, Wi, n, B, Ho, Wo, Cn)
+        if wsb == 0:
+            raise _lib.MdvitHipError("upsample_sum_bn_rowdot: shape not built for the tile kernel (upsample_sum_bn_rowdot() checks before it builds this node)")
+        ws = _empty((wsb // 8 + 1,), device=dev, dtype=torch.float64)
+        mean = _empty((Cn,), device=dev, dtype=torch.float32)
+        rstd = _empty_like(mean)
+        call("mdvit_upsample_multi_fwd_stats", ptrs, Hi, Wi, n, _p(base), _p(y), _p(ws), wsb, B, Ho, Wo, Cn, _stream())
+        nblk = (wsb - 16 * Cn) // (8 * Cn)
+        call("mdvit_bn_stats_finalize", _p(ws), wsb, nblk, _p(mean), _p(rstd), _p(running_mean), _p(running_var),
+             C.c_void_p(nbt.data_ptr()) if nbt is not None else None, M, Cn, eps, momentum, _stream())
+        key = _next_key() if drop2d_p > 0 else (0, 0)
+        low = _empty((M,), device=dev, dtype=torch.float32)
+        call("mdvit_bn_rowdot_fwd", _p(y), _p(mean), _p(rstd), _p(gamma), _p(beta), _p(w), _p(b), _p(low), M, Cn, act, drop2d_p, key[0], key[1],
+             _seed_ptr() if drop2d_p > 0 else None, Ho * Wo, _stream())
+        ctx.save_for_backward(y, gamma, beta, mean, rstd, w)
+        ctx.meta = (act, drop2d_p, key, b is not None, base is not None, [(x.shape[1], x.shape[2]) for x in xs])
+        return low
+
+    @staticmethod
+    def backward(ctx, g):
+        act, drop2d_p, key, has_b, has_base, dims = ctx.meta
+        n = len(dims)
+        if g is None:
+            return (None,) * (14 + n)
+        y, gamma, beta, mean, rstd, w = ctx.saved_tensors
+        g = _c(g)
+        B, Ho, Wo, Cn = y.shape
+        M = B * Ho * Wo
+        dy = _empty_like(y)
+        dg = db_ = dw = dbias = None
+        if not _dgrad_only:
+            dg, db_, dw, dbias = _flat_like(gamma, gamma, w.reshape(-1), (1,) if has_b else None)
+        lib = _lib.load()
+        wsb = lib.mdvit_bn_rowdot_ws_bytes(M, Cn)
+        ws = _empty((wsb // 8 + 1,), device=y.device, dtype=torch.float64)
+        dxs = [_empty((B, h, w_, Cn), device=y.device, dtype=torch.float32) for h, w_ in dims]
+        ptrs = (C.c_void_p * n)(*[t.data_ptr() for t in dxs])
+        Hi = (C.c_int32 * n)(*[h for h, _ in dims])
+        Wi = (C.c_int32 * n)(*[w_ for _, w_ in dims])
+        uwsb = lib.mdvit_upsample_multi_bwd_ws_bytes(Wi, n, B, Ho, Cn)
+        uws = _empty((uwsb // 4,), device=y.device, dtype=torch.float32)
+        call("mdvit_bn_rowdot_upsample_bwd", _p(g), _p(y), _p(mean), _p(rstd), _p(gamma), _p(beta), _p(w), _p(dy), _p(dg), _p(db_), _p(dw), _p(dbias), _p(ws), wsb,
+             ptrs, Hi, Wi, n, _p(uws), uwsb, B, Ho, Wo, Cn, act, 1, drop2d_p, key[0], key[1], _seed_ptr() if drop2d_p > 0 else None, _stream())
+        return (dy if has_base else None, dg, db_, None, None, None, None if dw is None else dw.view_as(w), dbias, None, None, None, None, None, None, *dxs)
+
+
+def upsample_sum_bn_rowdot(base, xs, Ho, Wo, gamma, beta, running_mean, running_var, nbt, training, act, w, b, eps=1e-5, momentum=0.1, drop2d_p=0.0):
+    xs = [_c(x) for x in xs]
+    Cn = xs[0].shape[-1]
+    if (training and _bn_groups == 1 and gamma.dim() == 1 and Cn in (256, 512, 1024) and 1 <= len(xs) <= 3 and xs[0].is_cuda
+            and all(x.dim() == 4 and x.shape[0] == xs[0].shape[0] and x.shape[-1] == Cn for x in xs)):
+        n = len(xs)
+        Hi = (C.c_int32 * n)(*[x.shape[1] for x in xs])
+        Wi = (C.c_int32 * n)(*[x.shape[2] for x in xs])
+        if _lib.load().mdvit_upsample_multi_stats_ws_bytes(Hi, Wi, n, xs[0].shape[0], int(Ho), int(Wo), Cn) > 0:
+            low = _UpsampleSumBNRowDot.apply(None if base is None else _c(base), _c(gamma), _c(beta), running_mean, running_var, nbt, w, b, float(eps), float(momentum),
+                                             int(act), float(drop2d_p), int(Ho), int(Wo), *xs)
+            return low.view(xs[0].shape[0], int(Ho), int(Wo))
+    return bn_act_rowdot(upsample_sum(base, xs, Ho, Wo), gamma, beta, running_mean, running_var, nbt, training, act, w, b, eps, momentum, drop2d_p)
+
+
 class _RowDot(torch.autograd.Function):
     @staticmethod
     def forward(ctx, x, w, b):
```

Measured after the change: 516.0 images/s, median of 6. About the same (+0.7%).
